# viswavi/speech-anonymization

Hardware: AMD Instinct MI355X
Metric: audio frames/sec (node), ConvAE+gender-adv train step (higher is better)
Workload: dtype bf16x3; 1 GPU; ConvAE recon0.1+sex0.9 adversarial train step (L1 recon + NLL), shape M: 32 utt/GPU x 161120 samples (T=1008 frames), Fbank x2 + norm + fwd + bwd + clip + Adam + Noam; batch_per_gpu=32, frames_per_utt=1008, parallelism=dp1

## Files before the change

### include/sa_hip.h

```cpp
#ifndef SA_HIP_H
#define SA_HIP_H
#ifdef __cplusplus
extern "C" {
#endif

#define SA_F32 0
#define SA_BF16 1
#define SA_BF16X3 2
#define SA_BF16X1F 3
#define SA_FP8 4
#define SA_F64 5
#define SA_MAX_TAPS 5
#define SA_COMM_ID_BYTES 128

typedef struct SaTaps {
  int ntaps[2];
  int off[2][SA_MAX_TAPS];
  int widx[2][SA_MAX_TAPS];
} SaTaps;

typedef struct SaConvArgs {
  const void* x;
  const void* wp;
  const float* bias;
  void* y;
  const float* s1; const float* t1;
  const float* s2; const float* t2;
  int swish;
  int relu;
  float* stats;
  int B, Lin, Lout, ntiles;
  int rowmin, nrows, wlo_off;
  SaTaps taps;
  int ep_mode, ep_xp_is_act, ep_bstride;
  const void* ep_x; const void* ep_g2;
  const float* ep_s1; const float* ep_t1; const float* ep_mean; const float* ep_rstd;
  void* a_out;
  const void* nb_x; const float* nb_c1; const float* nb_c2; const float* nb_c3;
  int nb_bstride, nb_relu_mask; float* nb_colsum;
  const float* ep_g2k1; const float* ep_g2k2; const float* ep_g2k3;
  float* pro_stats;
  const float* wscale;
  int tile_rows; int pad2_;
} SaConvArgs;

int sa_conv_gemm(int dtype, int cin, int cout, int sa, int u, const SaConvArgs* a, void* stream);
int sa_abi_sizeof(int which);
int sa_conv_gemm_ntiles(int cin, int cout, int u, int Lout);
int sa_conv_gemm_ntiles_tm(int tile_rows, int u, int Lout);
int sa_conv_gemm_set_tile_rows(int rows);
int sa_conv_gemm_set_impl(int impl);
int sa_conv_gemm_route(int dtype, int cin, int cout, int sa, int u, const SaConvArgs* a);

int sa_pack_weights(int dtype, const float* src, void* dst, int ntaps, int K, int N, int sk, int sn,
                    int st, void* stream);

typedef struct SaPackDesc {
  const float* src; void* dst;
  int dtype, ntaps, K, N, sk, sn, st, pad_;
  float* scale;
} SaPackDesc;
int sa_pack_weights_multi(const SaPackDesc* descs, int n, int blocks_per_image, void* stream);
int sa_pack_scales_multi(const SaPackDesc* descs, int n, void* stream);

typedef struct SaWgradArgs {
  const void* x;
  const void* dy;
  float* slabs;
  const float* s1; const float* t1; const float* s2; const float* t2; int swish;
  int B, Lin, Ldy, Mrows, chunk, nchunk;
  int ntaps; int off[SA_MAX_TAPS]; int ph[SA_MAX_TAPS];
  int x_pre;
  int dy_pre;
} SaWgradArgs;

int sa_wgrad(int dtype, int cin, int cout, int sa, int u, const SaWgradArgs* a, void* stream);
int sa_wgrad_kw(int cin, int cout);
int sa_wgrad_reduce(const float* slabs, float* dst, int nslab, int ntaps, int cin, int cout, int sk,
                    int sn, int st, int accumulate, void* stream);
#define SA_WRED_MAX 8
typedef struct SaWredDesc {
  const float* slabs; float* dst;
  int nslab, ntaps, cin, cout, sk, sn, st, accumulate, vec, pad_;
} SaWredDesc;
typedef struct SaWredMulti { int n, pad_; SaWredDesc d[SA_WRED_MAX]; } SaWredMulti;
int sa_wgrad_reduce_multi(const SaWredMulti* m, void* stream);

int sa_conv1toC(int dtype, const float* x, const float* w, const float* bias, void* y, int B, int L,
                int flip, float* stats, const void* ep_x, const float* ep_s1, const float* ep_t1,
                const float* ep_mean, const float* ep_rstd, void* stream);
int sa_conv1toC_ntiles(int L);
int sa_convCto1(int dtype, const void* x, const float* w, const float* bias, float* y, int B, int L,
                const float* s1, const float* t1, int swish, int flip, void* stream);
int sa_wgrad1C(int dtype, const float* u, const void* v, float* slabs, int B, int L, int chunk,
               int flip, const float* s1, const float* t1, int swish, void* stream);
int sa_wgrad1C_nchunk(int L, int chunk);
int sa_bwd1C(int dtype, const float* u, const void* v, const float* w, void* g, float* stats, float* slabs,
             int B, int L, int chunk, int flip, const float* s1, const float* t1, const float* mean,
             const float* rstd, void* stream);
int sa_sum_slabs(const float* slabs, float* dst, int nslab, int n, int accumulate, void* stream);

typedef struct SaEwArgs {
  const void* g; const void* g2; const void* x; void* out;
  const float* s1; const float* t1;
  const float* mean; const float* rstd;
  const float* c1; const float* c2; const float* c3;
  int actbwd, xp_is_act, relu_mask, bstride;
  float* stats;
  int B, L, ntiles;
} SaEwArgs;

int sa_ew_stats(int dtype, int C, const SaEwArgs* a, void* stream);
int sa_ew_apply(int dtype, int C, const SaEwArgs* a, void* stream);
int sa_ew_ntiles(int L);
int sa_sum_partials(const float* slabs, double* dst, int nbatch, int nslab, int n, void* stream);
int sa_sum_rows_d(const double* src, double* dst, int R, int n, void* stream);
int sa_fin_in_fwd(const double* sums, int B, int C, int n, const float* gamma, const float* beta,
                  float eps, float* mean, float* rstd, float* scale, float* shift, void* stream);
int sa_fin_bn_fwd(const double* sums, int R, int C, double count, const float* gamma, const float* beta,
                  float eps, float momentum, float* run_mean, float* run_var, float* mean,
                  float* rstd, float* scale, float* shift, const double* count_dev, void* stream);
int sa_fin_bn_eval(int C, const float* gamma, const float* beta, float eps, const float* run_mean,
                   const float* run_var, float* mean, float* rstd, float* scale, float* shift,
                   void* stream);
int sa_fin_norm_bwd(const double* sums, const double* lsums, int R, int groups, int C, double n,
                    const float* gamma, const float* mean, const float* rstd, float sign, float* c1,
                    float* c2, float* c3, float* dgamma, float* dbeta, const double* n_dev,
                    void* stream);
int sa_fin_bias(const double* sums, int B, int C, int ncomp, float* db, void* stream);

#define SA_FLATS_MAX 4
typedef struct SaFlat { float* p; long long n; } SaFlat;
typedef struct SaFlats { int n, pad_; SaFlat f[SA_FLATS_MAX]; } SaFlats;
int sa_clip_grads(const SaFlats* f, float max_norm, float eps, double* partials, float* total_norm, void* stream);
#define SA_BIAS_MAX 8
typedef struct SaBiasDesc {
  const float* part; double* rows; float* db;
  int nbatch, nslab, C, ncomp;
} SaBiasDesc;
typedef struct SaBiasMulti { int n, pad_; SaBiasDesc d[SA_BIAS_MAX]; } SaBiasMulti;
int sa_bias_multi(const SaBiasMulti* m, void* stream);

int sa_pool_fwd(int dtype, const void* r, const float* scale, const float* shift, float* part, int B,
                int L, int nseg, void* stream);
int sa_pool_nseg(int B);
int sa_pool_gather(const float* part, int B, int nseg, int L, double* sums, void* stream);
int sa_pool_fin(const double* sums, int B, int n, const float* noise, float eps, float* pooled,
                float* mean, float* stdraw, void* stream);
int sa_pool_bwd(int dtype, const void* r, const float* scale, const float* shift,
                const float* dpooled, const float* mean, const float* stdraw, void* g, int B, int L,
                const float* bn_mean, const float* bn_rstd, float* stats, void* stream);
int sa_dense(const float* X, int lda, const float* ps, const float* pt, const float* W, int sbk,
             int sbn, const float* bias, float* Y, int ldy, int M, int N, int K, int relu,
             void* stream);
int sa_colsums(const float* X, const float* H, const float* hmean, const float* hrstd, int M, int N,
               double* sums, float* out0, float* out1, void* stream);
int sa_bn2d_bwd(const float* G, const float* H, const double* sums, double count, const float* gamma,
                const float* mean, const float* rstd, int relu_mask, int M, int N, float* dH,
                const double* count_dev, void* stream);
int sa_dense_wgrad(const float* dY, const float* X, const float* ps, const float* pt, int M, int N,
                   int K, float* dW, void* stream);
int sa_log_softmax(const float* X, float* Y, int M, int N, void* stream);
int sa_log_softmax_bwd(const float* dY, const float* Y, float* dX, int M, int N, void* stream);
int sa_loss_workspace_bytes(void);
int sa_recon_loss(const float* a, const float* b, long long n, int kind, float* grad, float* loss,
                  void* workspace, void* stream);
int sa_cls_losses(const float* logp, const long long* label, int B, int NC, float* out, float* dnll,
                  float* dconf, void* stream);
int sa_cosine_loss(const float* x1, const float* x2, int B, int S, int D, float* rowloss,
                   float* loss, float* dx1, void* stream);

int sa_head_fwd(const float* pooled, const float* w1, const float* b1, const float* g1, const float* be1,
                float* rm1, float* rv1, const float* w2, const float* b2, const float* g2, const float* be2,
                float* rm2, float* rv2, const float* w3, const float* b3, float* h1, float* f1, float* h2,
                float* f2, float* logp, int M, float eps, float momentum, void* stream);
int sa_head_bwd(const float* dlogp, const float* logp, const float* pooled, const float* h1, const float* f1,
                const float* h2, const float* f2, const float* w1, const float* g1, const float* w2,
                const float* g2, const float* w3, float* dw1, float* db1, float* dg1, float* dbe1, float* dw2,
                float* db2, float* dg2, float* dbe2, float* dw3, float* db3, float* dpooled, int M, void* stream);
int sa_head_max_rows(void);

int sa_tdnn_fwd(const float* x, const void* wp, const float* bias, const float* bn_s, const float* bn_t,
                float* y, int B, int T, int Cin, int Cout, int Npad, int K, int dil, float slope,
                unsigned char* mask, void* stream);
int sa_time_pool(const float* x, const float* lens, const float* noise, int B, int T, int C, float eps,
                 float* out, void* stream);
int sa_leaky_affine(const float* x, const float* s, const float* t, float slope, int M, int C, float* y,
                    void* stream);
int sa_tdnn_bwd_input(const float* dy, const unsigned char* mask, const float* bn_s, const void* wp,
                      float* dxe, int B, int T, int Cy, int Cred, int Cin, int Npad, int K, int dil,
                      float slope, void* stream);
int sa_tdnn_fold(const float* dxe, float* dx, int B, int T, int C, int pad, void* stream);
int sa_time_pool_bwd(const float* x, const float* lens, const float* g, const float* pooled, int B,
                     int T, int C, float eps, float* dx, void* stream);
int sa_leaky_affine_bwd(const float* dy, const float* x, const float* s, float slope, int M, int C,
                        float* dx, void* stream);
// ... 137 lines not shown
```

### speech-anonymization_amd/_lib.py

```python
import ctypes as C
import os

import torch

_HERE = os.path.dirname(os.path.abspath(__file__))
LIB_PATH = os.environ.get("SA_HIP_LIB") or os.path.join(_HERE, "libsa_hip.so")

F32, BF16, BF16X3, BF16X1F, FP8, F64 = 0, 1, 2, 3, 4, 5
MAX_TAPS = 5

c_fp = C.POINTER(C.c_float)
vp = C.c_void_p


class SaTaps(C.Structure):
    _fields_ = [("ntaps", C.c_int * 2), ("off", (C.c_int * MAX_TAPS) * 2),
                ("widx", (C.c_int * MAX_TAPS) * 2)]


class SaConvArgs(C.Structure):
    _fields_ = [("x", vp), ("wp", vp), ("bias", vp), ("y", vp),
                ("s1", vp), ("t1", vp), ("s2", vp), ("t2", vp),
                ("swish", C.c_int), ("relu", C.c_int), ("stats", vp),
                ("B", C.c_int), ("Lin", C.c_int), ("Lout", C.c_int), ("ntiles", C.c_int),
                ("rowmin", C.c_int), ("nrows", C.c_int), ("wlo_off", C.c_int), ("taps", SaTaps),
                ("ep_mode", C.c_int), ("ep_xp_is_act", C.c_int), ("ep_bstride", C.c_int),
                ("ep_x", vp), ("ep_g2", vp), ("ep_s1", vp), ("ep_t1", vp), ("ep_mean", vp), ("ep_rstd", vp),
                ("a_out", vp),
                ("nb_x", vp), ("nb_c1", vp), ("nb_c2", vp), ("nb_c3", vp),
                ("nb_bstride", C.c_int), ("nb_relu_mask", C.c_int), ("nb_colsum", vp),
                ("ep_g2k1", vp), ("ep_g2k2", vp), ("ep_g2k3", vp), ("pro_stats", vp), ("wscale", vp),
                ("tile_rows", C.c_int), ("pad2_", C.c_int)]


class SaPackDesc(C.Structure):
    _fields_ = [("src", vp), ("dst", vp), ("dtype", C.c_int), ("ntaps", C.c_int), ("K", C.c_int),
                ("N", C.c_int), ("sk", C.c_int), ("sn", C.c_int), ("st", C.c_int), ("pad_", C.c_int),
                ("scale", vp)]


class SaWgradArgs(C.Structure):
    _fields_ = [("x", vp), ("dy", vp), ("slabs", vp),
                ("s1", vp), ("t1", vp), ("s2", vp), ("t2", vp), ("swish", C.c_int),
                ("B", C.c_int), ("Lin", C.c_int), ("Ldy", C.c_int), ("Mrows", C.c_int),
                ("chunk", C.c_int), ("nchunk", C.c_int),
                ("ntaps", C.c_int), ("off", C.c_int * MAX_TAPS), ("ph", C.c_int * MAX_TAPS),
                ("x_pre", C.c_int), ("dy_pre", C.c_int)]


class SaEwArgs(C.Structure):
    _fields_ = [("g", vp), ("g2", vp), ("x", vp), ("out", vp),
                ("s1", vp), ("t1", vp), ("mean", vp), ("rstd", vp),
                ("c1", vp), ("c2", vp), ("c3", vp),
                ("actbwd", C.c_int), ("xp_is_act", C.c_int), ("relu_mask", C.c_int),
                ("bstride", C.c_int), ("stats", vp),
                ("B", C.c_int), ("L", C.c_int), ("ntiles", C.c_int)]


BIAS_MAX = 8


class SaBiasDesc(C.Structure):
    _fields_ = [("part", vp), ("rows", vp), ("db", vp),
                ("nbatch", C.c_int), ("nslab", C.c_int), ("C", C.c_int), ("ncomp", C.c_int)]


class SaBiasMulti(C.Structure):
    _fields_ = [("n", C.c_int), ("pad_", C.c_int), ("d", SaBiasDesc * BIAS_MAX)]


WRED_MAX = 8
FLATS_MAX = 4


class SaFlat(C.Structure):
    _fields_ = [("p", vp), ("n", C.c_longlong)]


class SaFlats(C.Structure):
    _fields_ = [("n", C.c_int), ("pad_", C.c_int), ("f", SaFlat * FLATS_MAX)]



class SaWredDesc(C.Structure):
    _fields_ = [("slabs", vp), ("dst", vp)] + [(k, C.c_int) for k in ("nslab", "ntaps", "cin", "cout", "sk", "sn", "st",
                                                                      "accumulate", "vec", "pad_")]


class SaWredMulti(C.Structure):
    _fields_ = [("n", C.c_int), ("pad_", C.c_int), ("d", SaWredDesc * WRED_MAX)]


SYMBOLS = [
    "sa_conv_gemm", "sa_abi_sizeof", "sa_conv_gemm_ntiles", "sa_conv_gemm_ntiles_tm", "sa_conv_gemm_set_tile_rows",
    "sa_conv_gemm_set_impl", "sa_conv_gemm_route", "sa_pack_weights", "sa_pack_weights_multi", "sa_pack_scales_multi", "sa_wgrad", "sa_wgrad_kw", "sa_wgrad_reduce",
    "sa_conv1toC", "sa_conv1toC_ntiles", "sa_convCto1", "sa_wgrad1C", "sa_wgrad1C_nchunk", "sa_bwd1C",
    "sa_sum_slabs", "sa_ew_stats", "sa_ew_apply", "sa_ew_ntiles",
    "sa_sum_partials", "sa_sum_rows_d", "sa_fin_in_fwd", "sa_fin_bn_fwd", "sa_fin_bn_eval", "sa_fin_norm_bwd", "sa_fin_bias",
    "sa_pool_fwd", "sa_pool_nseg", "sa_pool_gather", "sa_pool_fin", "sa_pool_bwd", "sa_dense", "sa_colsums",
    "sa_bn2d_bwd", "sa_dense_wgrad", "sa_log_softmax", "sa_log_softmax_bwd",
    "sa_loss_workspace_bytes", "sa_recon_loss", "sa_cls_losses", "sa_cosine_loss",
    "sa_tdnn_fwd", "sa_time_pool", "sa_leaky_affine", "sa_tdnn_bwd_input", "sa_tdnn_fold", "sa_time_pool_bwd",
    "sa_leaky_affine_bwd", "sa_cluster_mi", "sa_fbank", "sa_fbank_table_elems", "sa_fbank_ntiles", "sa_fbank_scratch_bytes", "sa_fbank_normalize", "sa_fbank_normalize_pair",
    "sa_comm_unique_id", "sa_comm_init", "sa_comm_world", "sa_comm_allreduce", "sa_comm_allreduce_inline", "sa_comm_join", "sa_comm_ncalls",
    "sa_comm_destroy", "sa_head_fwd", "sa_head_bwd", "sa_head_max_rows",
    "sa_add_layernorm_fwd", "sa_layernorm_bwd", "sa_reflect_pad_fwd", "sa_reflect_pad_bwd", "sa_ln_leaky_fwd", "sa_ln_leaky_bwd", "sa_bias_multi", "sa_asr_block0_fwd", "sa_asr_block0_bwd", "sa_wgrad_reduce_multi", "sa_clip_grads",
    "sa_xv_tdnn_fwd_train", "sa_xv_tdnn_ntiles", "sa_xv_colsums", "sa_xv_tdnn_wgrad", "sa_xv_wgrad_reduce",
    "sa_xv_tdnn_dgrad", "sa_xv_pool_affine", "sa_xv_pool_affine_bwd",
    "sa_fc_tiles", "sa_fc_groups", "sa_fc_nparam", "sa_fc_nhead", "sa_fc_max_rows", "sa_fc_enc_fwd", "sa_fc_bn_fin",
    "sa_fc_mid_fwd", "sa_fc_head_fwd", "sa_fc_head_bwd", "sa_fc_mid_bwd", "sa_fc_bn_bwd_fin", "sa_fc_enc_bwd",
    "sa_fc_wreduce", "sa_fc_recon_fwd",
    "sa_wav_augment_tile", "sa_wav_augment_max_chunks", "sa_wav_abs_sums", "sa_noise_scales", "sa_wav_augment",
    "sa_specaug_warp_sums", "sa_specaug_finalize", "sa_specaug_fill",
    "sa_gl_tile", "sa_mel_to_mag", "sa_gl_istft", "sa_gl_project",
    "sa_yin_dim", "sa_yin_f0", "sa_pitch_ratio", "sa_pitch_stretch_mag", "sa_pitch_resample",
    "sa_env_dim", "sa_env_warp",
    "sa_mcadams_dim", "sa_mcadams",
    "sa_stoi_dim", "sa_stoi",
    "sa_pv_dim", "sa_pv_synth",
]

_lib = None


class SaHipError(RuntimeError):
    pass


def load():
    global _lib
    if _lib is None:
        if not os.path.exists(LIB_PATH):
            raise SaHipError(
                f"{LIB_PATH} not found: build it with `python -c 'import __graft_entry__ as g; "
                "g.build()'` (hipcc --offload-arch=gfx950). There is no CPU fallback.")
        _lib = C.CDLL(LIB_PATH)
        for s in SYMBOLS:
            getattr(_lib, s).restype = C.c_int
        _lib.sa_pv_workspace_bytes.restype = C.c_longlong
        for i, rec in enumerate((SaConvArgs, SaWgradArgs, SaEwArgs, SaPackDesc, SaTaps, SaBiasMulti, SaWredMulti, SaFlats)):
            if _lib.sa_abi_sizeof(i) != C.sizeof(rec):
                raise SaHipError(f"{rec.__name__}: binding has {C.sizeof(rec)} bytes, {LIB_PATH} "
                                 f"{_lib.sa_abi_sizeof(i)} -- rebuild the library (stale build?)")
    return _lib


def stream():
    return C.c_void_p(torch._C._cuda_getCurrentRawStream(torch._C._cuda_getDevice()))


def ptr(t):
    if t is None:
        return None
    assert t.is_cuda and t.is_contiguous(), "HIP kernels take contiguous device tensors"
    return C.c_void_p(t.data_ptr())


def check(rc, what):
    if rc != 0:
        raise SaHipError(f"{what} failed with code {rc}")


def dt_code(dtype):
    if dtype == torch.float32:
        return F32
    if dtype == torch.bfloat16:
        return BF16
    raise SaHipError(f"unsupported activation dtype {dtype}")


_taps_cache = {}


def make_taps(phases):
    key = tuple(tuple(p) for p in phases)
    t = _taps_cache.get(key)
    if t is not None:
        return t
    t = _taps_cache[key] = SaTaps()
    for ph, lst in enumerate(phases):
        t.ntaps[ph] = len(lst)
        for i, (off, wi) in enumerate(lst):
            t.off[ph][i] = off
            t.widx[ph][i] = wi
    return t
# ... 1 lines not shown
```

### speech-anonymization_amd/convae.py

```python
import functools
import os

import torch
import torch.nn as nn

from . import distributed as sdist
from . import ops
from . import _lib as L
from ._lib import SaHipError


class _ParamOnly(nn.Module):

    def forward(self, x):
        raise SaHipError("parameter container only; use ConvAutoencoder.forward")


class GLU(_ParamOnly):
    pass


class StatisticsPooling(_ParamOnly):
    pass


class TDNNSexClassifier(nn.Module):
    def __init__(self, num_classes=2):
        super().__init__()
        self.tdnn = nn.Sequential(
            nn.Conv1d(128, 128, kernel_size=5, dilation=1), nn.ReLU(), nn.BatchNorm1d(128),
            nn.Conv1d(128, 128, kernel_size=3, dilation=2), nn.ReLU(), nn.BatchNorm1d(128),
            nn.Conv1d(128, 128, kernel_size=3, dilation=3), nn.ReLU(), nn.BatchNorm1d(128),
        )
        self.norm = nn.BatchNorm1d(128)
        self.stats_pooling = StatisticsPooling()
        self.classify = nn.Sequential(
            nn.Linear(256, 128), nn.ReLU(), nn.BatchNorm1d(128),
            nn.Linear(128, 64), nn.ReLU(), nn.BatchNorm1d(64),
            nn.Linear(64, num_classes),
        )

    def forward(self, x):
        raise SaHipError("parameter container only; use ConvAutoencoder.forward")


class ConvAutoencoder(nn.Module):
    def __init__(self, precision="bf16x3", pooling_noise=True, sync_bn=True, dtype=None,
                 cache_wgrad_operand=True):
        super().__init__()
        if dtype is not None:
            precision = {torch.float32: "f32", torch.bfloat16: "bf16"}[dtype]
        if precision not in ops.PRECISIONS:
            raise SaHipError(f"unknown precision {precision!r}")
        self.precision = precision
        self.encoder = nn.Sequential(
            nn.Conv1d(1, 32, 15, 1, 7), GLU(),
            nn.Conv1d(32, 64, 5, 2, 2), nn.InstanceNorm1d(64, affine=True), GLU(),
            nn.Conv1d(64, 64, 5, 1, 2), nn.InstanceNorm1d(64, affine=True), GLU(),
            nn.Conv1d(64, 128, 5, 2, 2), nn.InstanceNorm1d(128, affine=True), GLU(),
            nn.Conv1d(128, 128, 5, 1, 2), nn.InstanceNorm1d(128, affine=True), GLU(),
        )
        self.decoder = nn.Sequential(
            nn.Conv1d(128, 128, 5, 1, 2),
            nn.ConvTranspose1d(128, 64, 5, 2, 2, output_padding=1),
            nn.InstanceNorm1d(64, affine=True), GLU(),
            nn.Conv1d(64, 64, 5, 1, 2),
            nn.ConvTranspose1d(64, 32, 5, 2, 2, output_padding=1),
            nn.InstanceNorm1d(32, affine=True), GLU(),
            nn.Conv1d(32, 1, 15, 1, 7),
        )
        self.sex_classifier = TDNNSexClassifier(2)
        self.lay = ops.conv_layers(self, ("encoder", "sex_classifier.tdnn", "decoder"))
        self.pack_plan = [(ly.key, ly.kinds[i]) for i in (0, 1)
                          for ly in sorted(self.lay.values(), key=lambda ly: ly.transposed)]
        self.act_dtype, self.kcode = ops.PRECISIONS[precision]
        self.dgrad_kcode = ops.DGRAD_CODE[precision]
        self.cache_wgrad_operand = cache_wgrad_operand
        self.pooling_noise = pooling_noise
        self.sync_bn = sync_bn
        self.fused_head = os.environ.get("SA_FUSED_HEAD", "1") == "1"
        self.fused_bwd1c = os.environ.get("SA_FUSED_BWD1C", "1") == "1"
        self.dp_batch_sizes = None

    def forward(self, feats):
        names, params = self._named_params()
        return _ConvAEFn.apply(self, names, feats, *params)

    def _named_params(self):
        c = self.__dict__.get("_np_cache")
        if c is None or any(o[n] is not p for o, n, p in c[2]):
            names, params, owners = [], [], []
            for mname, mod in self.named_modules():
                for pname, p in mod._parameters.items():
                    if p is not None:
                        names.append(f"{mname}.{pname}" if mname else pname)
                        params.append(p)
                        owners.append((mod._parameters, pname, p))
            c = self.__dict__["_np_cache"] = (tuple(names), tuple(params), owners)
        return c[0], c[1]

    @torch.no_grad()
    def reconstruct(self, feats):
        if not torch.is_tensor(feats) or feats.dim() != 3:
            raise SaHipError("ConvAutoencoder expects feats [B, T, 80]")
        x0, B, T, Ltot = _input_rows(feats)
        P = dict(zip(*self._named_params()))
        cg, inorm = _launchers(self, P, _packed(self, P), B)
        y, _, _ = _encoder_launches(self, P, cg, inorm, x0, Ltot, False)
        return _decoder_launches(self, P, cg, inorm, y[5], Ltot)[-1].view(B, T, 80)

    def _side_stream(self, device):
        if getattr(self, "_side", None) is None and device.type == "cuda":
            self._side = torch.cuda.Stream(device=device)
        return getattr(self, "_side", None)

    def _bn_syncs(self):
        return self.sync_bn and sdist.dp_active()

    def _bn_allreduce(self, sums):
        if self._bn_syncs():
            sdist.all_reduce_now(sums)
            return sdist.world_size()
        return 1

    def _bn_global_counts(self, counts, device):
        if not self._bn_syncs():
            return None
        key = (tuple(counts), str(device))
        cache = self.__dict__.setdefault("_count_cache", {})
        local = cache.get(key)
        if local is None:
            if len(cache) > 64:
                cache.clear()
            local = cache[key] = torch.tensor(counts, dtype=torch.float64).to(device)
        g = local.clone()
        sdist.all_reduce_now(g)
        return g

    def _bn_rows(self):
        return not self._bn_syncs()

    def _bn_global(self, local_sums):
        if not self._bn_syncs():
            return local_sums, 1
        g = local_sums.clone()
        return g, self._bn_allreduce(g)

    def _head_plan(self, B):
        if not self._bn_syncs() or self.dp_batch_sizes is None:
            return None
        W, r = sdist.world_size(), sdist.rank()
        sizes = [B] * W if isinstance(self.dp_batch_sizes, str) else [int(b) for b in self.dp_batch_sizes]
        if self.dp_batch_sizes != "equal" and isinstance(self.dp_batch_sizes, str):
            raise SaHipError(f"dp_batch_sizes: 'equal', a list of per-rank batch sizes or None, not {self.dp_batch_sizes!r}")
        if len(sizes) != W or sizes[r] != B:
            raise SaHipError(f"dp_batch_sizes {sizes} does not describe rank {r} of {W} holding {B} utterances")
        return sum(sizes[:r]), sum(sizes), W

    @staticmethod
    def _gather_rows(x, plan):
        off, Bg, _ = plan
        g = torch.zeros(Bg, x.shape[1], device=x.device, dtype=x.dtype)
        g[off:off + x.shape[0]].copy_(x)
        sdist.all_reduce_now(g)
        return g


class _W:
    __slots__ = ("img", "code")

    def __init__(self, img, code):
        self.img, self.code = img, code


def _kcode(model, kind):
    return model.dgrad_kcode if kind.endswith("dgrad") else model.kcode


def _packed(model, P):
    items = [((k, kind), P[k], kind, _kcode(model, kind)) for k, kind in model.pack_plan]
    key = tuple(w.data_ptr() for _, w, _, _ in items) + tuple(c for _, _, _, c in items)
    pk = getattr(model, "_pack_cache", None)
    if pk is None or pk[0] != key:
        pk = (key, ops.PackedWeights(items, model.act_dtype))
        model._pack_cache = pk
    pk[1].refresh()
    return {tag: _W(img, code) for tag, (img, code) in pk[1].images.items()}


def _conv(x, w, *args, **kw):
    return ops.conv_gemm(x, w.img, *args, code=w.code, **kw)


class _PendingApply:
    __slots__ = ("g", "y", "c", "per_c", "relu", "bias_key", "wgrads")

    def __init__(self, g, y, c, per_c, relu, bias_key):
        self.g, self.y, self.c, self.per_c, self.relu, self.bias_key = g, y, c, per_c, relu, bias_key
        self.wgrads = []


def _noise(model, B, device):
    return ops.pooling_noise(model.pooling_noise, B, 128, device)


def _input_rows(feats):
    B, T, Fd = feats.shape
    Ltot = T * Fd
    if Fd != 80 or Ltot % 4:
        raise SaHipError("ConvAutoencoder expects feats [B, T, 80] with T*80 divisible by 4")
    if not feats.is_cuda:
        raise SaHipError("ConvAutoencoder runs on the GPU only (no CPU fallback)")
    return feats.detach().reshape(B, Ltot).contiguous().float(), B, T, Ltot


def _in_ep(y, nrm, g2=None):
    mean, rstd, scale, shift = nrm
    d = dict(mode=1, x=y, g2=g2, s1=scale, t1=shift, mean=mean, rstd=rstd)
    if isinstance(g2, _PendingApply):
        d.update(g2=g2.g, g2k=g2.c)
    return d


def _launchers(model, P, W, B, A=None):
    def cg(ly, x, **kw):
        if A is not None and P[ly.key].requires_grad:
            A[ly.key] = kw["a_out"] = torch.empty(x.shape, dtype=torch.bfloat16, device=x.device)
        return _conv(x, W[ly.key, ly.kinds[0]], P[ly.bias], *ly.fwd(x.shape[1]), **kw)

    def inorm(stats, n, prefix, C):
        sums = ops.sum_partials(stats, B)
        return ops.fin_in_fwd(sums, B, C, n, P[prefix + ".weight"], P[prefix + ".bias"])
    return cg, inorm


def _encoder_launches(model, P, cg, inorm, x0, Ltot, want_pro_stats):
    L2, L4, lay = Ltot // 2, Ltot // 4, model.lay
    y0 = ops.conv1toC(x0, P["encoder.0.weight"], P["encoder.0.bias"], model.act_dtype)
    y1, st = cg(lay["encoder.2"], y0, swish=True, want_stats=True)
    n1 = inorm(st, L2, "encoder.3", 64)
    y2, st = cg(lay["encoder.5"], y1, s1=n1[2], t1=n1[3], swish=True, want_stats=True)
    n2 = inorm(st, L2, "encoder.6", 64)
    y3, st = cg(lay["encoder.8"], y2, s1=n2[2], t1=n2[3], swish=True, want_stats=True)
    n3 = inorm(st, L4, "encoder.9", 128)
    y4, st = cg(lay["encoder.11"], y3, s1=n3[2], t1=n3[3], swish=True, want_stats=True)
    n4 = inorm(st, L4, "encoder.12", 128)
    y5 = cg(lay["decoder.0"], y4, s1=n4[2], t1=n4[3], swish=True, want_pro_stats=want_pro_stats)
    a4_stats = None
    if want_pro_stats:
        y5, a4_stats = y5
    return [y0, y1, y2, y3, y4, y5], [n1, n2, n3, n4], a4_stats


def _decoder_launches(model, P, cg, inorm, y5, Ltot):
    L2, lay = Ltot // 2, model.lay
    y6, st = cg(lay["decoder.1"], y5, want_stats=True)
    n6 = inorm(st, L2, "decoder.2", 64)
    y7 = cg(lay["decoder.4"], y6, s1=n6[2], t1=n6[3], swish=True)
    y8, st = cg(lay["decoder.5"], y7, want_stats=True)
    n8 = inorm(st, Ltot, "decoder.6", 32)
    recon = ops.convCto1(y8, P["decoder.8.weight"], P["decoder.8.bias"], n8[2], n8[3], True)
    return y6, n6, y7, y8, n8, recon


class _ConvAEFn(torch.autograd.Function):
    @staticmethod
    def forward(ctx, model, names, feats, *params):
        ctx.set_materialize_grads(False)
        P = dict(zip(names, params))
        train = model.training
        x0, B, T, Ltot = _input_rows(feats)
        L2, L4 = Ltot // 2, Ltot // 4
        S = {}
        W, lay = _packed(model, P), model.lay
        A = {}
        cache_a = (train and model.cache_wgrad_operand and any(ctx.needs_input_grad)
                   and ops.WGRAD_CODE[model.precision] in (L.BF16X1F, L.BF16) and model.kcode != L.FP8)

        cg, inorm = _launchers(model, P, W, B, A if cache_a else None)

        def bn_stats(stats, count, mod, prefix, C, ci):
            sums = ops.sum_partials(stats, 1, rows=model._bn_rows()) if train else None
            return bnorm(sums, count, mod, prefix, C, ci)

        def bnorm(sums, count, mod, prefix, C, ci, local=False):
            if not train:
                return ops.fin_bn_eval(C, P[prefix + ".weight"], P[prefix + ".bias"],
                                       mod.running_mean, mod.running_var)
            if not local:
                model._bn_allreduce(sums)
            out = ops.fin_bn_fwd(sums, C, count, P[prefix + ".weight"], P[prefix + ".bias"],
                                 mod.running_mean, mod.running_var, count_dev=None if local else cdev(ci))
            tracked.append(mod.num_batches_tracked)
            return out

        tracked = []
        enc, dec, cls = model.encoder, model.decoder, model.sex_classifier
        La, Lb, Lc = L4 - 4, L4 - 8, L4 - 14
        gc = model._bn_global_counts([B * L4, B * La, B * Lb, B * Lc, B, B], feats.device) if train else None
        cdev = lambda i: None if gc is None else gc[i:i + 1]
        (y0, y1, y2, y3, y4, y5), (n1, n2, n3, n4), a4_stats = _encoder_launches(model, P, cg, inorm, x0, Ltot, train)
        bn_n = bn_stats(a4_stats if train else None, B * L4, cls.norm, "sex_classifier.norm", 128, 0)
        r0, st = cg(lay["sex_classifier.tdnn.0"], y4, s1=n4[2], t1=n4[3], swish=True, s2=bn_n[2], t2=bn_n[3],
                    relu=True, want_stats=True)
        bn0 = bn_stats(st, B * La, cls.tdnn[2], "sex_classifier.tdnn.2", 128, 1)
        r1, st = cg(lay["sex_classifier.tdnn.3"], r0, s2=bn0[2], t2=bn0[3], relu=True, want_stats=True)
        bn1 = bn_stats(st, B * Lb, cls.tdnn[5], "sex_classifier.tdnn.5", 128, 2)
        r2, st = cg(lay["sex_classifier.tdnn.6"], r1, s2=bn1[2], t2=bn1[3], relu=True, want_stats=True)
        bn2 = bn_stats(st, B * Lc, cls.tdnn[8], "sex_classifier.tdnn.8", 128, 3)
        pooled, pmean, psd = ops.pool_fwd(r2, bn2[2], bn2[3], noise=_noise(model, B, feats.device))
        def head_fwd(X, n, local=False):
            H1 = ops.dense(X, P["sex_classifier.classify.0.weight"], P["sex_classifier.classify.0.bias"],
                           128, 256, relu=True)
            f1 = bnorm(ops.colsums(H1) if train else None, n, cls.classify[2], "sex_classifier.classify.2", 128, 4, local)
            H2 = ops.dense(H1, P["sex_classifier.classify.3.weight"], P["sex_classifier.classify.3.bias"],
                           64, 128, ps=f1[2], pt=f1[3], relu=True)
            f2 = bnorm(ops.colsums(H2) if train else None, n, cls.classify[5], "sex_classifier.classify.5", 64, 5, local)
            logits = ops.dense(H2, P["sex_classifier.classify.6.weight"], P["sex_classifier.classify.6.bias"],
                               2, 64, ps=f2[2], pt=f2[3])
            return H1, f1, H2, f2, ops.log_softmax(logits)

        plan = model._head_plan(B) if train else None
        head_in, Bh = (model._gather_rows(pooled, plan), plan[1]) if plan else (pooled, B)
        fused_head = (train and model.fused_head and (plan is not None or not model._bn_syncs())
                      and Bh <= ops.head_max_rows())
        clsP = {k[len("sex_classifier.classify."):]: v for k, v in P.items() if k.startswith("sex_classifier.classify.")}
        if fused_head:
            H1, f1, H2, f2, logp = ops.head_fwd(head_in, clsP, cls.classify[2], cls.classify[5])
            tracked += [cls.classify[2].num_batches_tracked, cls.classify[5].num_batches_tracked]
        else:
            H1, f1, H2, f2, logp = head_fwd(head_in, Bh, plan is not None)
        logp_all = logp
        if plan:
            logp = logp_all[plan[0]:plan[0] + B]
        y6, n6, y7, y8, n8, recon = _decoder_launches(model, P, cg, inorm, y5, Ltot)

        if tracked:
            torch._foreach_add_(tracked, 1)
        S.update(x0=x0, y=[y0, y1, y2, y3, y4, y5, y6, y7, y8], r=[r0, r1, r2],
                 n=[None, n1, n2, n3, n4, None, n6, None, n8], bn=[bn_n, bn0, bn1, bn2], f=[f1, f2],
                 pooled=head_in, pmean=pmean, psd=psd, H1=H1, H2=H2, logp=logp_all, head_plan=plan,
                 dims=(B, T, Ltot, L2, L4, La, Lb, Lc), train=train, W=W, A=A, gc=gc, fused_head=fused_head)
        ctx.S, ctx.model, ctx.names, ctx.params = S, model, names, params
        ctx.need_input_grad = feats.requires_grad
        return recon.view(B, T, 80), logp

    @staticmethod
    def backward(ctx, d_recon, d_logp):
        S, model, names = ctx.S, ctx.model, ctx.names
        if S is None:
            raise SaHipError("ConvAutoencoder backward called twice (saved tensors were released)")
        P = dict(zip(names, ctx.params))
        dt = model.act_dtype
        B, T, Ltot, L2, L4, La, Lb, Lc = S["dims"]
        if not S["train"]:
            raise SaHipError("backward through eval-mode BatchNorm is not implemented")
        y0, y1, y2, y3, y4, y5, y6, y7, y8 = S["y"]
        r0, r1, r2 = S["r"]
        n1, n2, n3, n4, n6, n8 = S["n"][1], S["n"][2], S["n"][3], S["n"][4], S["n"][6], S["n"][8]
        bn_n, bn0, bn1, bn2 = S["bn"]
        f1, f2 = S["f"]
        dev = y0.device
        G = {k: None for k in names}
        need = {k: p.requires_grad for k, p in P.items()}
        need_stage = {st: any(v for k, v in need.items() if k.startswith(st))
                      for st in sdist.StageBuckets.STAGES}
        run_encoder = need_stage["encoder"] or ctx.need_input_grad
        run_decoder = need_stage["decoder"] or run_encoder
        model._last_flats = None
        buckets = sdist.StageBuckets(list(P.items()), dev, model._side_stream(dev))
        newg = buckets.view

        def setg(key, val):
            G[key] = newg(key).copy_(val.reshape(P[key].shape))
        W, A, lay = S["W"], S["A"], model.lay
        gc = S["gc"]
        cdev = lambda i: None if gc is None else gc[i:i + 1]
        pending_wred = []
        wg = functools.partial(ops.wgrad, code=ops.WGRAD_CODE[model.precision], defer=pending_wred)
        fuse = bool(A) and model.dgrad_kcode in (L.BF16X3, L.BF16)

        def cg(ly, gin, **kw):
            p, dy = gin, gin.g if isinstance(gin, _PendingApply) else gin
            w, args = W[ly.key, ly.kinds[1]], (None,) + ly.dgrad(ly.lin(dy.shape[1]))
            if dy is gin:
                return _conv(dy, w, *args, **kw)
            dyc = torch.empty(p.g.shape, dtype=torch.bfloat16, device=p.g.device) if p.wgrads else None
            want_cs = p.bias_key is not None and need[p.bias_key]
            out = _conv(p.g, w, *args, a_out=dyc, nb=dict(x=p.y, c1=p.c[0], c2=p.c[1], c3=p.c[2],
                                                           per_c=p.per_c, relu_mask=p.relu,
                                                           want_colsum=want_cs), **kw)
            if want_cs:
                cs = out[-1]
                out = out[:-1] if len(out) > 2 else out[0]
                nb_, _, cc_ = cs.shape
                G[p.bias_key] = newg(p.bias_key)
                pending_bias.append((cs, nb_, cc_, 1, G[p.bias_key]))
            for f in p.wgrads:
                f(dyc)
            p.wgrads = []
            return out

        def bias_from(stats, key, C):
            if need[key]:
                G[key] = newg(key)
                pending_bias.append((stats, B, C, 2, G[key]))

        pending_bias = []

        def flush_pending():
            if pending_bias:
                ops.bias_multi(pending_bias)
                pending_bias.clear()
            if pending_wred:
                ops.wgrad_reduce_multi(pending_wred)
                pending_wred.clear()

        def in_finish(g, st, y, nrm, C, Ln, prefix, bias_key):
            mean, rstd = nrm[0], nrm[1]
            dg, db = newg(prefix + ".weight"), newg(prefix + ".bias")
            sums = ops.sum_partials(st, B)
            c1, c2, c3 = ops.fin_norm_bwd(sums, sums, B * C, C, Ln, P[prefix + ".weight"], mean, rstd,
                                          dgamma=dg, dbeta=db)
            G[prefix + ".weight"], G[prefix + ".bias"] = dg, db
            if fuse:
                return _PendingApply(g, y, (c1, c2, c3), False, False, bias_key)
            st2 = ops.ew("apply", g, y, C, out=g, c1=c1, c2=c2, c3=c3)
            bias_from(st2, bias_key, C)
            return g

        def bn_ep(r, bn, xp=None):
            d = dict(mode=2, x=r, mean=bn[0], rstd=bn[1], per_c=True)
            if xp:
                d.update(s1=xp[0], t1=xp[1], xp_is_act=True)
            return d

        def bn_finish(g, st, r, bn, Ln, prefix, bias_key, ci, xp=None):
            mean, rstd = bn[0], bn[1]
            kw = dict(s1=xp[0], t1=xp[1], xp_is_act=True) if xp else {}
            dg, db = newg(prefix + ".weight"), newg(prefix + ".bias")
            lsums = ops.sum_partials(st, 1, rows=model._bn_rows())
            gsums, _ = model._bn_global(lsums)
            c1, c2, c3 = ops.fin_norm_bwd(gsums, lsums, 128, 128, float(B * Ln), P[prefix + ".weight"],
                                          mean, rstd, sign=-1.0 if xp else 1.0, dgamma=dg, dbeta=db,
                                          n_dev=cdev(ci))
            G[prefix + ".weight"], G[prefix + ".bias"] = dg, db
            if fuse:
                return _PendingApply(g, r, (c1, c2, c3), True, not xp, bias_key)
            st2 = ops.ew("apply", g, r, 128, out=g, c1=c1, c2=c2, c3=c3, relu_mask=not xp, per_c=True,
                         want_stats=bias_key is not None, **kw)
            if bias_key:
                bias_from(st2, bias_key, 128)
            return g

        def conv_wgrad(ly, x, dy, **pro):
            key = ly.key
            if not need[key]:
                return
            if isinstance(dy, _PendingApply):
                dy.wgrads.append(lambda dyc: conv_wgrad(ly, x, dyc, dy_pre=True))
                return
            if key in A:
                x, pro = A[key], dict(x_pre=True, dy_pre=bool(pro.get("dy_pre")))
            *geo, strides = ly.wgrad(x.shape[1])
            G[key] = wg(x, dy, *geo, newg(key), strides, **pro)

        recon_unused = d_recon is None
        if recon_unused:
            for k in need:
                if k.startswith("decoder"):
                    need[k] = False
            need_stage["decoder"] = False
        if d_logp is None:
            d_logp = torch.zeros(B, 2, device=dev)

        def finish(d_feats=None):
            flush_pending()
            buckets.join()
            ctx.S = None
            model._last_flats = [buckets.flat[st] for st in sdist.StageBuckets.STAGES if need_stage[st]]
            grads = tuple(G[k] if need[k] else None for k in names)
            G.clear()
            buckets.views.clear()
            return (None, None, d_feats) + grads

        def head_bwd():
            c = "sex_classifier.classify."
            plan = S.get("head_plan")
            dlp, Bh = d_logp.contiguous().float(), B
            if plan:
                dlp, Bh = model._gather_rows(dlp, plan), plan[1]
            dP = head_bwd_rows(c, dlp, Bh, plan is not None)
            if plan:
                hg = [G[k] for k in names if k.startswith(c) and k in G]
                if plan[2] > 1 and hg:
                    torch._foreach_mul_(hg, 1.0 / plan[2])
                dP = dP[plan[0]:plan[0] + B]
            return dP

        def head_bwd_rows(c, dlp, n, local):
            if S.get("fused_head"):
                short = ("0.weight", "0.bias", "2.weight", "2.bias", "3.weight", "3.bias", "5.weight", "5.bias",
                         "6.weight", "6.bias")
                views = {}
                for k in short:
                    if need[c + k]:
                        views[k] = G[c + k] = newg(c + k)
                clsP = {k: P[c + k] for k in short}
                return ops.head_bwd(dlp, S["logp"], S["pooled"], S["H1"], f1, S["H2"], f2, clsP, views)
            glob = (lambda l: l) if local else (lambda l: model._bn_global(l)[0])
            cd = (lambda i: None) if local else cdev
            dLG = ops.log_softmax_bwd(dlp, S["logp"])
            H1, H2 = S["H1"], S["H2"]
            G[c + "6.weight"] = ops.dense_wgrad(dLG, H2, newg(c + "6.weight"), ps=f2[2], pt=f2[3])
            G[c + "6.bias"] = newg(c + "6.bias"); ops.colsums(dLG, out0=G[c + "6.bias"])
            dN2 = ops.dense(dLG, P[c + "6.weight"], None, 64, 2, transpose_w=True)
            G[c + "5.weight"], G[c + "5.bias"] = newg(c + "5.weight"), newg(c + "5.bias")
            l2 = ops.colsums(dN2, H2, f2[0], f2[1], out0=G[c + "5.bias"], out1=G[c + "5.weight"])
            dH2 = ops.bn2d_bwd(dN2, H2, glob(l2), n, P[c + "5.weight"], f2[0], f2[1], True, count_dev=cd(5))
            G[c + "3.weight"] = ops.dense_wgrad(dH2, H1, newg(c + "3.weight"), ps=f1[2], pt=f1[3])
            G[c + "3.bias"] = newg(c + "3.bias"); ops.colsums(dH2, out0=G[c + "3.bias"])
            dN1 = ops.dense(dH2, P[c + "3.weight"], None, 128, 64, transpose_w=True)
            G[c + "2.weight"], G[c + "2.bias"] = newg(c + "2.weight"), newg(c + "2.bias")
            l1 = ops.colsums(dN1, H1, f1[0], f1[1], out0=G[c + "2.bias"], out1=G[c + "2.weight"])
            dH1 = ops.bn2d_bwd(dN1, H1, glob(l1), n, P[c + "2.weight"], f1[0], f1[1], True, count_dev=cd(4))
            G[c + "0.weight"] = ops.dense_wgrad(dH1, S["pooled"], newg(c + "0.weight"))
            G[c + "0.bias"] = newg(c + "0.bias"); ops.colsums(dH1, out0=G[c + "0.bias"])
            return ops.dense(dH1, P[c + "0.weight"], None, 256, 128, transpose_w=True)

        def tdnn_bwd(dP):
            t = "sex_classifier.tdnn."
            g, st = ops.pool_bwd(r2, bn2[2], bn2[3], dP, S["pmean"], S["psd"], bn=(bn2[0], bn2[1]))
            g = bn_finish(g, st, r2, bn2, Lc, t + "8", t + "6.bias", 3)
            conv_wgrad(lay[t + "6"], r1, g, s2=bn1[2], t2=bn1[3])
            g, st = cg(lay[t + "6"], g, want_stats=True, ep=bn_ep(r1, bn1))
            g = bn_finish(g, st, r1, bn1, Lb, t + "5", t + "3.bias", 2)
            conv_wgrad(lay[t + "3"], r0, g, s2=bn0[2], t2=bn0[3])
            g, st = cg(lay[t + "3"], g, want_stats=True, ep=bn_ep(r0, bn0))
            g = bn_finish(g, st, r0, bn0, La, t + "2", t + "0.bias", 1)
            conv_wgrad(lay[t + "0"], y4, g, s1=n4[2], t1=n4[3], swish=True, s2=bn_n[2], t2=bn_n[3])
            xp4 = (n4[2], n4[3])
            g, st = cg(lay[t + "0"], g, want_stats=True, ep=bn_ep(y4, bn_n, xp4))
            da = bn_finish(g, st, y4, bn_n, L4, "sex_classifier.norm", None, 0, xp=xp4)
            flush_pending()
            if need_stage["sex_classifier"]:
                buckets.reduce_stage("sex_classifier")
            return da

        def decoder_bwd():
            d_rec = torch.zeros(B, T, 80, device=dev) if recon_unused else d_recon
            g_rec = d_rec.reshape(B, Ltot).contiguous().float()
            if need["decoder.8.bias"]:
                setg("decoder.8.bias", ops.sum_partials(g_rec.view(4 * B, Ltot // 4), 1, n=Ltot // 4).sum())
            if need["decoder.8.weight"] and model.fused_bwd1c:
                g, st, G["decoder.8.weight"] = ops.bwd1C(g_rec, y8, P["decoder.8.weight"], newg("decoder.8.weight"),
                                                         n8[2], n8[3], n8[0], n8[1])
            else:
                if need["decoder.8.weight"]:
                    G["decoder.8.weight"] = ops.wgrad1C(g_rec, y8, newg("decoder.8.weight"), flip=True,
                                                        s1=n8[2], t1=n8[3], swish=True)
                g, st = ops.conv1toC(g_rec, P["decoder.8.weight"], None, dt, flip=True, want_stats=True,
                                     ep=dict(x=y8, s1=n8[2], t1=n8[3], mean=n8[0], rstd=n8[1]))
            g = in_finish(g, st, y8, n8, 32, Ltot, "decoder.6", "decoder.5.bias")
            conv_wgrad(lay["decoder.5"], y7, g)
            g, st = cg(lay["decoder.5"], g, want_stats=True)
            bias_from(st, "decoder.4.bias", 64)
            conv_wgrad(lay["decoder.4"], y6, g, s1=n6[2], t1=n6[3], swish=True)
            g, st = cg(lay["decoder.4"], g, want_stats=True, ep=_in_ep(y6, n6))
            g = in_finish(g, st, y6, n6, 64, L2, "decoder.2", "decoder.1.bias")
            conv_wgrad(lay["decoder.1"], y5, g)
            g, st = cg(lay["decoder.1"], g, want_stats=True)
            bias_from(st, "decoder.0.bias", 128)
            conv_wgrad(lay["decoder.0"], y4, g, s1=n4[2], t1=n4[3], swish=True)
            flush_pending()
            if need_stage["decoder"]:
                buckets.reduce_stage("decoder")
            return g

        da4_cls = tdnn_bwd(head_bwd())
        if not run_decoder:
            return finish()
        g = decoder_bwd()
        if not run_encoder:
            return finish()

        g, st = cg(lay["decoder.0"], g, want_stats=True, ep=_in_ep(y4, n4, g2=da4_cls))
        for conv, norm, y, nrm, x, nx in (("encoder.11", "encoder.12", y4, n4, y3, n3),
                                          ("encoder.8", "encoder.9", y3, n3, y2, n2),
                                          ("encoder.5", "encoder.6", y2, n2, y1, n1),
                                          ("encoder.2", "encoder.3", y1, n1, y0, None)):
            ly = lay[conv]
            g = in_finish(g, st, y, nrm, ly.cout, y.shape[1], norm, ly.bias)
            conv_wgrad(ly, x, g, swish=True, **(dict(s1=nx[2], t1=nx[3]) if nx else {}))
            g, st = cg(ly, g, want_stats=True, ep=_in_ep(x, nx) if nx else dict(mode=1, x=x))
        bias_from(st, "encoder.0.bias", 32)
        if need["encoder.0.weight"]:
            G["encoder.0.weight"] = ops.wgrad1C(S["x0"], g, newg("encoder.0.weight"))
        d_feats = None
        if ctx.need_input_grad:
            d_feats = ops.convCto1(g, P["encoder.0.weight"], None, flip=True).view(B, T, 80)
        flush_pending()
        if need_stage["encoder"]:
            buckets.reduce_stage("encoder")
        return finish(d_feats)
```

### speech-anonymization_amd/csrc/sa_conv_gemm.hip

```cpp
#include <type_traits>
#include "sa_common.h"

#include "sa_conv_cfg.h"

template <typename T, int CIN, int COUT, int SA, int U, int TM, bool PRO2>
__global__ __launch_bounds__(256, 2) void sa_conv_gemm_kernel(SaConvArgs a, int red_off, int col_off) {
  typedef ConvCfg<T, CIN, COUT, SA, U, TM> C;
  typedef Pol<T> P;
  typedef typename P::store_t S;
  typedef typename P::lds_t LT;
  typedef typename P::Frag Frag;
  typedef Tr<S> tr;
  constexpr int VEC = C::VEC, OVEC = C::OVEC;
  extern __shared__ __attribute__((aligned(16))) unsigned char smem[];
  LT* As = reinterpret_cast<LT*>(smem);
  S* Os = reinterpret_cast<S*>(smem);
  float* red = reinterpret_cast<float*>(smem + red_off);
  const int plane = a.nrows * C::APITCH;

  const int tid = threadIdx.x, lane = tid & 63, wave = tid >> 6;
  const int tile = blockIdx.x, b = blockIdx.y;
  const int m0 = tile * C::BMB;

  {
    const int c = tid % C::CHI, r0 = tid / C::CHI;
    float s1[VEC], t1[VEC], s2[VEC], t2[VEC];
#pragma unroll
    for (int j = 0; j < VEC; ++j) {
      s1[j] = a.s1 ? a.s1[(size_t)b * CIN + c * VEC + j] : 1.0f;
      t1[j] = a.t1 ? a.t1[(size_t)b * CIN + c * VEC + j] : 0.0f;
      s2[j] = a.s2 ? a.s2[c * VEC + j] : 1.0f;
      t2[j] = a.t2 ? a.t2[c * VEC + j] : 0.0f;
    }
    const bool has1 = a.s1 != nullptr, has2 = a.s2 != nullptr, sw = a.swish != 0;
    const S* xb = reinterpret_cast<const S*>(a.x) + (size_t)b * a.Lin * CIN + c * VEC;
    const int gbase = m0 * SA + a.rowmin;
    const int own_lo = m0 * SA;
    int own_hi = tile == a.ntiles - 1 ? a.Lin : (m0 + C::BMB) * SA;
    if (own_hi > a.Lin) own_hi = a.Lin;
    constexpr int NIT = ((C::BMB - 1) * SA + 1 + SA_MAX_HALO + C::RPPI - 1) / C::RPPI;
    uint4 raw[NIT];
#pragma unroll
    for (int i = 0; i < NIT; ++i) {
      const int r = r0 + i * C::RPPI, g = gbase + r;
      raw[i] = make_uint4(0, 0, 0, 0);
      if (r < a.nrows && g >= 0 && g < a.Lin) raw[i] = *reinterpret_cast<const uint4*>(xb + (size_t)g * CIN);
    }
    uint4 raw2[PRO2 ? NIT : 1];
    float k1[VEC], k2[VEC], k3[VEC], csum[VEC];
    if constexpr (PRO2) {
      const S* x2 = reinterpret_cast<const S*>(a.nb_x) + (size_t)b * a.Lin * CIN + c * VEC;
#pragma unroll
      for (int i = 0; i < NIT; ++i) {
        const int r = r0 + i * C::RPPI, g = gbase + r;
        raw2[i] = make_uint4(0, 0, 0, 0);
        if (r < a.nrows && g >= 0 && g < a.Lin) raw2[i] = *reinterpret_cast<const uint4*>(x2 + (size_t)g * CIN);
      }
#pragma unroll
      for (int j = 0; j < VEC; ++j) {
        const size_t q = (size_t)b * a.nb_bstride + c * VEC + j;
        k1[j] = a.nb_c1[q]; k2[j] = a.nb_c2[q]; k3[j] = a.nb_c3[q]; csum[j] = 0.0f;
      }
    }
    auto stage_rows = [&](auto xform) {
#pragma unroll
      for (int i = 0; i < NIT; ++i) {
        const int r = r0 + i * C::RPPI, g = gbase + r;
        if (r < a.nrows) {
          float f[VEC];
          tr::unpack(raw[i], f);
          if (g >= 0 && g < a.Lin) xform(f, i, g);
          LT* dst = As + (size_t)r * C::APITCH + c * VEC;
          if constexpr (P::NPL == 2) {
            uint2 hi, lo;
            sa_split4(f, hi, lo);
            *reinterpret_cast<uint2*>(dst) = hi;
            *reinterpret_cast<uint2*>(dst + plane) = lo;
          } else if constexpr (sizeof(LT) == 1) {
            *reinterpret_cast<uint2*>(dst) = sa_pack_fp8x8(f);
          } else if constexpr (sizeof(LT) == 2 && sizeof(S) == 4) {
            *reinterpret_cast<uint2*>(dst) = sa_pack_bf16x4(f);
          } else if constexpr (sizeof(LT) == 2) {
            *reinterpret_cast<uint4*>(dst) = tr::pack(f);
          } else {
            float* d = reinterpret_cast<float*>(dst);
            d[0] = f[0]; d[1] = f[1]; d[2] = f[2]; d[3] = f[3];
          }
        }
      }
    };
    if constexpr (PRO2) {
      stage_rows([&](float* f, int i, int g) {
        float y[VEC];
        tr::unpack(raw2[i], y);
        const bool own = g >= own_lo && g < own_hi;
#pragma unroll
        for (int j = 0; j < VEC; ++j) {
          float v = fmaf(k1[j], f[j], fmaf(k2[j], y[j], k3[j]));
          if (a.nb_relu_mask && !(y[j] > 0.0f)) v = 0.0f;
          f[j] = v;
          if (own) csum[j] += v;
        }
      });
      if (a.nb_colsum) {
        float* colred = reinterpret_cast<float*>(smem + col_off);
#pragma unroll
        for (int j = 0; j < VEC; ++j) {
          float v = csum[j];
          for (int off = C::CHI; off < 64; off <<= 1) v += __shfl_xor(v, off, 64);
          if (lane < C::CHI) colred[wave * CIN + (lane % C::CHI) * VEC + j] = v;
        }
      }
    } else if (!has1 && !has2 && !sw) {
      stage_rows([](float*, int, int) {});
    } else if (has1 && sw && !has2 && a.pro_stats) {
      float ps[VEC], pq[VEC];
#pragma unroll
      for (int j = 0; j < VEC; ++j) { ps[j] = 0.0f; pq[j] = 0.0f; }
      stage_rows([&](float* f, int, int g) {
        const bool own = g >= own_lo && g < own_hi;
#pragma unroll
        for (int j = 0; j < VEC; ++j) {
          const float v = sa_swish(fmaf(f[j], s1[j], t1[j]));
          f[j] = v;
          if (own) { ps[j] += v; pq[j] = fmaf(v, v, pq[j]); }
        }
      });
      float* colred = reinterpret_cast<float*>(smem + col_off);
#pragma unroll
      for (int j = 0; j < VEC; ++j) {
        float v = ps[j], w = pq[j];
        for (int off = C::CHI; off < 64; off <<= 1) { v += __shfl_xor(v, off, 64); w += __shfl_xor(w, off, 64); }
        if (lane < C::CHI) {
          colred[(wave * CIN + (lane % C::CHI) * VEC + j) * 2 + 0] = v;
          colred[(wave * CIN + (lane % C::CHI) * VEC + j) * 2 + 1] = w;
        }
      }
    } else if (has1 && sw && !has2) {
      stage_rows([&](float* f, int, int) {
#pragma unroll
        for (int j = 0; j < VEC; ++j) f[j] = sa_swish(fmaf(f[j], s1[j], t1[j]));
      });
    } else {
      stage_rows([&](float* f, int, int) {
#pragma unroll
        for (int j = 0; j < VEC; ++j) {
          float v = f[j];
          if (has1) v = fmaf(v, s1[j], t1[j]);
          if (sw) v = sa_swish(v);
          if (has2) v = fmaf(v, s2[j], t2[j]);
          f[j] = v;
        }
      });
    }
  }
  __syncthreads();
  if (!PRO2 && a.pro_stats && tid < CIN) {
    const float* colred = reinterpret_cast<const float*>(smem + col_off);
    float* d = a.pro_stats + (((size_t)b * a.ntiles + tile) * CIN + tid) * 2;
#pragma unroll
    for (int q = 0; q < 2; ++q)
      d[q] = (colred[tid * 2 + q] + colred[(CIN + tid) * 2 + q]) +
             (colred[(2 * CIN + tid) * 2 + q] + colred[(3 * CIN + tid) * 2 + q]);
  }
  if constexpr (PRO2) {
    if (a.nb_colsum && tid < CIN) {
      const float* colred = reinterpret_cast<const float*>(smem + col_off);
      a.nb_colsum[((size_t)b * a.ntiles + tile) * CIN + tid] =
          (colred[tid] + colred[CIN + tid]) + (colred[2 * CIN + tid] + colred[3 * CIN + tid]);
    }
  }
  if constexpr (sizeof(LT) == 2) {
    if (a.a_out) {
      constexpr int CH16 = CIN / 8;
      const int own_lo = m0 * SA;
      int own_hi = tile == a.ntiles - 1 ? a.Lin : (m0 + C::BMB) * SA;
      if (own_hi > a.Lin) own_hi = a.Lin;
      const int rlo = own_lo - (m0 * SA + a.rowmin);
      bf16_t* ao = reinterpret_cast<bf16_t*>(a.a_out) + ((size_t)b * a.Lin + own_lo) * CIN;
      for (int e = tid; e < (own_hi - own_lo) * CH16; e += 256) {
        const int r = e / CH16, c = e % CH16;
        *reinterpret_cast<uint4*>(ao + (size_t)r * CIN + c * 8) =
            *reinterpret_cast<const uint4*>(As + (size_t)(rlo + r) * C::APITCH + c * 8);
      }
    }
  }

  const int wn = wave % C::WN, wm = wave / C::WN;
  f32x16 acc[C::VPW][C::MT];
#pragma unroll
  for (int v = 0; v < C::VPW; ++v)
#pragma unroll
    for (int mt = 0; mt < C::MT; ++mt)
#pragma unroll
      for (int i = 0; i < 16; ++i) acc[v][mt][i] = 0.0f;

  constexpr int KUP = P::NPL == 2 ? 2 : 8;
  constexpr int KU = C::KSTEPS < KUP ? C::KSTEPS : KUP;
  constexpr int GPT = C::KSTEPS / KU;
  static_assert(C::KSTEPS % KU == 0, "k-steps per tap must be a multiple of the prefetch group");
  const Frag* wp = reinterpret_cast<const Frag*>(a.wp);
#pragma unroll
  for (int v = 0; v < C::VPW; ++v) {
    const int vt = wn + v * C::WN;
    const int ph = vt / C::NT, nt = vt % C::NT;
    const int G = a.taps.ntaps[ph] * GPT;
    const LT* abase = As + (size_t)((wm * C::MT * 32 + (lane & 31)) * SA - a.rowmin) * C::APITCH
                      + (lane >> 5) * (C::KS / 2);
    auto load_group = [&](Frag (&dst)[P::NPL][KU], int g) {
      const int ti = g / GPT, kg = g % GPT;
      const Frag* wt = wp + (((size_t)a.taps.widx[ph][ti] * C::KSTEPS + kg * KU) * C::NT + nt) * 64 + lane;
#pragma unroll
      for (int ku = 0; ku < KU; ++ku) {
        dst[0][ku] = wt[(size_t)ku * C::NT * 64];
        if constexpr (P::NPL == 2) dst[1][ku] = wt[(size_t)a.wlo_off + (size_t)ku * C::NT * 64];
      }
    };
    auto compute_group = [&](const Frag (&bq)[P::NPL][KU], int g) {
      const int ti = g / GPT, kg = g % GPT;
      const LT* arow = abase + (size_t)a.taps.off[ph][ti] * C::APITCH + kg * KU * C::KS;
      Frag ah[2][C::MT], al[2][C::MT];
      auto load_a = [&](int slot, int ku) {
#pragma unroll
        for (int mt = 0; mt < C::MT; ++mt) {
          const LT* ap = arow + (size_t)mt * 32 * SA * C::APITCH + ku * C::KS;
          ah[slot][mt] = *reinterpret_cast<const Frag*>(ap);
          if constexpr (P::NPL == 2) al[slot][mt] = *reinterpret_cast<const Frag*>(ap + plane);
        }
      };
      load_a(0, 0);
#pragma unroll
      for (int ku = 0; ku < KU; ++ku) {
        if (ku + 1 < KU) load_a((ku + 1) & 1, ku + 1);
#pragma unroll
        for (int mt = 0; mt < C::MT; ++mt) {
          if constexpr (P::NPL == 2) {
            acc[v][mt] = __builtin_amdgcn_mfma_f32_32x32x16_bf16(al[ku & 1][mt], bq[0][ku], acc[v][mt], 0, 0, 0);
            acc[v][mt] = __builtin_amdgcn_mfma_f32_32x32x16_bf16(ah[ku & 1][mt], bq[1][ku], acc[v][mt], 0, 0, 0);
            acc[v][mt] = __builtin_amdgcn_mfma_f32_32x32x16_bf16(ah[ku & 1][mt], bq[0][ku], acc[v][mt], 0, 0, 0);
          } else {
            acc[v][mt] = Tr<LT>::mfma(ah[ku & 1][mt], bq[0][ku], acc[v][mt]);
          }
        }
      }
    };
    Frag b0[P::NPL][KU], b1[P::NPL][KU];
    load_group(b0, 0);
    for (int g = 0; g < G; g += 2) {
      if (g + 1 < G) load_group(b1, g + 1);
      compute_group(b0, g);
      if (g + 1 < G) {
        if (g + 2 < G) load_group(b0, g + 2);
        compute_group(b1, g + 1);
      }
    }
  }
  constexpr int NOT = TM / C::RPPO;
  const int ec = tid % C::CHO, er0 = tid / C::CHO;
  __syncthreads();

#pragma unroll
  for (int v = 0; v < C::VPW; ++v) {
    const int vt = wn + v * C::WN;
    const int ph = vt / C::NT, nt = vt % C::NT;
    const int col = nt * 32 + (lane & 31);
    const float bv = a.bias ? a.bias[col] : 0.0f;
    float winv = 1.0f;
    if constexpr (sizeof(LT) == 1) winv = a.wscale ? 1.0f / a.wscale[0] : 1.0f;
#pragma unroll
    for (int mt = 0; mt < C::MT; ++mt) {
#pragma unroll
      for (int i = 0; i < 16; ++i) {
        const int m = wm * C::MT * 32 + mt * 32 + sa_acc_row(i, lane);
        float val = sizeof(LT) == 1 ? fmaf(acc[v][mt][i], winv, bv) : acc[v][mt][i] + bv;
        if (a.relu) val = fmaxf(val, 0.0f);
        Os[(size_t)(m * U + ph) * C::OPITCH + col] = tr::from_f(val);
      }
    }
  }
  __syncthreads();
  {
    const int c = ec, r0 = er0;
    float ssum[OVEC], ssq[OVEC], es1[OVEC], et1[OVEC], emu[OVEC], ers[OVEC];
#pragma unroll
    for (int j = 0; j < OVEC; ++j) {
      ssum[j] = 0.0f; ssq[j] = 0.0f;
      es1[j] = (a.ep_mode && a.ep_s1) ? a.ep_s1[(size_t)b * COUT + c * OVEC + j] : 1.0f;
      et1[j] = (a.ep_mode && a.ep_t1) ? a.ep_t1[(size_t)b * COUT + c * OVEC + j] : 0.0f;
      emu[j] = (a.ep_mode && a.ep_mean) ? a.ep_mean[(size_t)b * a.ep_bstride + c * OVEC + j] : 0.0f;
      ers[j] = (a.ep_mode && a.ep_rstd) ? a.ep_rstd[(size_t)b * a.ep_bstride + c * OVEC + j] : 1.0f;
    }
    const bool g2k = a.ep_mode && a.ep_g2 && a.ep_g2k1;
    float gk1[OVEC], gk2[OVEC], gk3[OVEC];
#pragma unroll
    for (int j = 0; j < OVEC; ++j) {
      gk1[j] = g2k ? a.ep_g2k1[c * OVEC + j] : 1.0f;
      gk2[j] = g2k ? a.ep_g2k2[c * OVEC + j] : 0.0f;
      gk3[j] = g2k ? a.ep_g2k3[c * OVEC + j] : 0.0f;
    }
    S* yb = reinterpret_cast<S*>(a.y) + (size_t)b * a.Lout * COUT + c * OVEC;
    const S* xe = a.ep_mode ? reinterpret_cast<const S*>(a.ep_x) + (size_t)b * a.Lout * COUT + c * OVEC : nullptr;
    const S* ge = (a.ep_mode && a.ep_g2) ? reinterpret_cast<const S*>(a.ep_g2) + (size_t)b * a.Lout * COUT + c * OVEC : nullptr;
    const int o0 = m0 * U;
    auto ep_rows = [&](uint4 u, const uint4& epx, const uint4& epg, int o) {
      float g[OVEC], x[OVEC], g2[OVEC], xn[OVEC];
      tr::unpack(u, g); tr::unpack(epx, x); tr::unpack(epg, g2);
#pragma unroll
      for (int j = 0; j < OVEC; ++j) {
        const float z = fmaf(x[j], es1[j], et1[j]);
        if (g2k) g2[j] = fmaf(gk1[j], g2[j], fmaf(gk2[j], sa_swish(z), gk3[j]));
        float gg = g[j] + g2[j];
        if (a.ep_mode == 1) gg *= sa_swish_grad(z);
        const float xv = a.ep_xp_is_act ? sa_swish(z) : x[j];
        xn[j] = (xv - emu[j]) * ers[j];
        g[j] = gg;
      }
      u = tr::pack(g);
      *reinterpret_cast<uint4*>(yb + (size_t)o * COUT) = u;
      if (a.stats) {
        tr::unpack(u, g);
#pragma unroll
        for (int j = 0; j < OVEC; ++j) { ssum[j] += g[j]; ssq[j] = fmaf(g[j], xn[j], ssq[j]); }
      }
    };
    if (a.ep_mode && o0 + TM <= a.Lout) {
      auto run = [&](auto has_g2_c) {
        constexpr bool HG = decltype(has_g2_c)::value;
        constexpr int D = NOT < 2 ? NOT : 2;
        uint4 px[D], pg[D];
#pragma unroll
        for (int d = 0; d < D; ++d) {
          px[d] = *reinterpret_cast<const uint4*>(xe + (size_t)(o0 + r0 + d * C::RPPO) * COUT);
          pg[d] = make_uint4(0, 0, 0, 0);
          if constexpr (HG) pg[d] = *reinterpret_cast<const uint4*>(ge + (size_t)(o0 + r0 + d * C::RPPO) * COUT);
        }
#pragma unroll
        for (int i = 0; i < NOT; ++i) {
          const int r = r0 + i * C::RPPO, o = o0 + r;
          const uint4 epx = px[i % D], epg = pg[i % D];
          if (i + D < NOT) {
            px[i % D] = *reinterpret_cast<const uint4*>(xe + (size_t)(o + D * C::RPPO) * COUT);
            if constexpr (HG) pg[i % D] = *reinterpret_cast<const uint4*>(ge + (size_t)(o + D * C::RPPO) * COUT);
          }
          const uint4 u = *reinterpret_cast<const uint4*>(Os + (size_t)r * C::OPITCH + c * OVEC);
          ep_rows(u, epx, epg, o);
        }
      };
      if (ge) run(std::true_type{}); else run(std::false_type{});
    } else {
#pragma unroll
    for (int i = 0; i < NOT; ++i) {
      const int r = r0 + i * C::RPPO, o = o0 + r;
      if (o < a.Lout) {
        uint4 u = *reinterpret_cast<const uint4*>(Os + (size_t)r * C::OPITCH + c * OVEC);
        if (a.ep_mode) {
          const uint4 epx = *reinterpret_cast<const uint4*>(xe + (size_t)o * COUT);
          const uint4 epg = ge ? *reinterpret_cast<const uint4*>(ge + (size_t)o * COUT) : make_uint4(0, 0, 0, 0);
          ep_rows(u, epx, epg, o);
        } else {
          *reinterpret_cast<uint4*>(yb + (size_t)o * COUT) = u;
          if (a.stats) {
            float f[OVEC];
            tr::unpack(u, f);
#pragma unroll
            for (int j = 0; j < OVEC; ++j) { ssum[j] += f[j]; ssq[j] = fmaf(f[j], f[j], ssq[j]); }
          }
        }
      }
    }
    }
    if (a.stats) {
      __syncthreads();
#pragma unroll
      for (int j = 0; j < OVEC; ++j) {
        red[((size_t)r0 * COUT + c * OVEC + j) * 2 + 0] = ssum[j];
        red[((size_t)r0 * COUT + c * OVEC + j) * 2 + 1] = ssq[j];
      }
    }
  }
  if (a.stats) {
    __syncthreads();
    if (tid < COUT) {
      float s = 0.0f, q = 0.0f;
      for (int r = 0; r < C::RPPO; ++r) {
        s += red[((size_t)r * COUT + tid) * 2 + 0];
        q += red[((size_t)r * COUT + tid) * 2 + 1];
      }
      float* dst = a.stats + (((size_t)b * a.ntiles + tile) * COUT + tid) * 2;
      dst[0] = s; dst[1] = q;
    }
  }
}

template <typename T, int CIN, int COUT, int SA, int U, int TM, bool PRO2 = false>
static int launch_cfg(const SaConvArgs& a, hipStream_t st) {
  typedef ConvCfg<T, CIN, COUT, SA, U, TM> C;
  SaConvArgs args = a;
  args.ntiles = sa_div_up(sa_div_up(a.Lout, U), C::BMB);
  int omin = 1 << 30, omax = -(1 << 30);
  for (int ph = 0; ph < U; ++ph)
    for (int t = 0; t < a.taps.ntaps[ph]; ++t) {
      omin = a.taps.off[ph][t] < omin ? a.taps.off[ph][t] : omin;
      omax = a.taps.off[ph][t] > omax ? a.taps.off[ph][t] : omax;
    }
  if (omin > omax || omax - omin > SA_MAX_HALO) return -22;
  int wmax = 0;
  for (int ph = 0; ph < U; ++ph)
    for (int t = 0; t < a.taps.ntaps[ph]; ++t) wmax = a.taps.widx[ph][t] > wmax ? a.taps.widx[ph][t] : wmax;
  args.rowmin = omin;
  args.nrows = (C::BMB - 1) * SA + (omax - omin) + 1;
  args.wlo_off = (wmax + 1) * C::KSTEPS * C::NT * 64;
  if ((a.a_out || a.nb_colsum || a.pro_stats) &&
      (omin > 0 || (C::BMB - 1) * SA + omax < C::BMB * SA - 1 ||
       (args.ntiles - 1) * C::BMB * SA + omin + args.nrows < a.Lin))
    return -22;
  if (a.a_out && sizeof(typename C::LT) != 2) return -22;
  if (PRO2 && (!a.nb_c1 || !a.nb_c2 || !a.nb_c3)) return -22;
  if (a.pro_stats && (PRO2 || !a.s1 || !a.swish || a.s2)) return -22;
  const size_t tile_lds = C::lds_bytes(args.nrows);
  const size_t lds = tile_lds + (PRO2 ? 4 * CIN * sizeof(float) : a.pro_stats ? 8 * CIN * sizeof(float) : 0);
  if (lds > 160 * 1024) return -12;
  auto kern = sa_conv_gemm_kernel<T, CIN, COUT, SA, U, TM, PRO2>;
  static bool attr_set = false;
  if (!attr_set) {
    hipError_t e = hipFuncSetAttribute(reinterpret_cast<const void*>(kern),
                                       hipFuncAttributeMaxDynamicSharedMemorySize, 160 * 1024);
    if (e != hipSuccess) return -(int)e;
    attr_set = true;
  }
  dim3 grid(args.ntiles, a.B);
  hipLaunchKernelGGL(kern, grid, dim3(256), lds, st, args, 0, (int)tile_lds);
  hipError_t e = hipGetLastError();
  return e == hipSuccess ? 0 : -(int)e;
}

static int g_tile_rows = 0;
extern "C" int sa_conv_gemm_set_tile_rows(int rows) {
  if (rows != 0 && rows != 64 && rows != 128) return -22;
  g_tile_rows = rows;
  return 0;
}
static int tile_rows(int cin, int cout, int u) {
  if (cin == 64 && cout == 32 && u == 2) return 128;
  if (g_tile_rows) return g_tile_rows;
  if ((cin == 64 && cout == 64) || (cin == 128 && cout == 64 && u == 2)) return 128;
  return 64;
}

extern "C" int sa_conv_gemm_ntiles(int cin, int cout, int u, int Lout) {
  const int tm = tile_rows(cin, cout, u);
  return sa_div_up(sa_div_up(Lout, u), tm / u);
}

bool sa_conv_ws_covers(int dtype, int cin, int cout, int sa, int u, const SaConvArgs* a);
int sa_conv_ws_dispatch(int cin, int cout, const SaConvArgs* a, hipStream_t st);
int sa_conv_ws_tile_rows(int cout);
int sa_conv_ws_rows_per_tile(int cout);
bool sa_conv_wsd_covers(int dtype, int cin, int cout, int sa, int u, const SaConvArgs* a);
int sa_conv_wsd_dispatch(int cin, int cout, const SaConvArgs* a, hipStream_t st);
static int g_use_ws = 1;
extern "C" int sa_conv_gemm_set_impl(int impl) {
  if (impl != 0 && impl != 2) return -22;
  g_use_ws = impl == 2;
  return 0;
}

extern "C" int sa_conv_gemm_ntiles_tm(int tile_rows, int u, int Lout) {
  if ((tile_rows != 64 && tile_rows != 128) || u < 1 || Lout < 1) return -22;
  return sa_div_up(sa_div_up(Lout, u), tile_rows / u);
}

template <typename T, int CI, int CO, int S, int UU, bool PRO2 = false>
static int launch_tm(const SaConvArgs& a, hipStream_t st) {
  if constexpr (CI == 64 && CO == 32 && UU == 2) {
    return launch_cfg<T, CI, CO, S, UU, 128, PRO2>(a, st);
  } else {
    const int tm = (a.tile_rows == 64 || a.tile_rows == 128) ? a.tile_rows : tile_rows(CI, CO, UU);
    return tm == 64 ? launch_cfg<T, CI, CO, S, UU, 64, PRO2>(a, st)
                    : launch_cfg<T, CI, CO, S, UU, 128, PRO2>(a, st);
  }
}

#define SA_CONV_CASE(CI, CO, S, UU)                                              \
  if (cin == CI && cout == CO && sa == S && u == UU) {                           \
    if (a->nb_x)                                                                 \
      return dtype == SA_BF16X3 ? launch_tm<bf16x3_t, CI, CO, S, UU, true>(*a, st) \
             : dtype == SA_BF16 ? launch_tm<bf16_t, CI, CO, S, UU, true>(*a, st) : -22; \
    if (dtype == SA_FP8) return (a->wscale && !a->ep_mode) ? launch_tm<fp8_t, CI, CO, S, UU>(*a, st) : -22; \
    return dtype == SA_BF16 ? launch_tm<bf16_t, CI, CO, S, UU>(*a, st)           \
           : dtype == SA_BF16X3 ? launch_tm<bf16x3_t, CI, CO, S, UU>(*a, st)     \
           : dtype == SA_BF16X1F ? launch_tm<bf16x1f_t, CI, CO, S, UU>(*a, st)   \
                                : launch_tm<float, CI, CO, S, UU>(*a, st);       \
  }

extern "C" int sa_abi_sizeof(int which) {
  switch (which) {
    case 0: return (int)sizeof(SaConvArgs);
    case 1: return (int)sizeof(SaWgradArgs);
    case 2: return (int)sizeof(SaEwArgs);
    case 3: return (int)sizeof(SaPackDesc);
    case 4: return (int)sizeof(SaTaps);
    case 5: return (int)sizeof(SaBiasMulti);
    case 6: return (int)sizeof(SaWredMulti);
    case 7: return (int)sizeof(SaFlats);
    default: return -22;
  }
}

static int conv_route(int dtype, int cin, int cout, int sa, int u, const SaConvArgs* a) {
  if (g_use_ws && sa_conv_ws_covers(dtype, cin, cout, sa, u, a) &&
      tile_rows(cin, cout, u) == sa_conv_ws_tile_rows(cout) &&
      (long)a->B * sa_div_up(a->Lout, sa_conv_ws_rows_per_tile(cout)) >= 1536)
    return 2;
  if (g_use_ws && sa_conv_wsd_covers(dtype, cin, cout, sa, u, a) && tile_rows(cin, cout, u) == 64 &&
      (long)a->B * sa_div_up(a->Lout, 64) >= 1536)
    return 3;
  return 0;
}
extern "C" int sa_conv_gemm_route(int dtype, int cin, int cout, int sa, int u, const SaConvArgs* a) {
  if (!a || a->B <= 0 || a->Lout <= 0) return -22;
  return conv_route(dtype, cin, cout, sa, u, a);
}

extern "C" int sa_conv_gemm(int dtype, int cin, int cout, int sa, int u, const SaConvArgs* a,
                            void* stream) {
  hipStream_t st = reinterpret_cast<hipStream_t>(stream);
  if (!a || !a->x || !a->wp || !a->y || a->B <= 0 || a->Lin <= 0 || a->Lout <= 0) return -22;
  if (a->ep_mode < 0 || a->ep_mode > 2 || (a->ep_mode && !a->ep_x)) return -22;
  const int route = conv_route(dtype, cin, cout, sa, u, a);
  if (route == 2) return sa_conv_ws_dispatch(cin, cout, a, st);
  if (route == 3) return sa_conv_wsd_dispatch(cin, cout, a, st);
  SA_CONV_CASE(32, 64, 2, 1)
  SA_CONV_CASE(64, 64, 1, 1)
  SA_CONV_CASE(64, 128, 2, 1)
  SA_CONV_CASE(128, 128, 1, 1)
  SA_CONV_CASE(128, 64, 1, 2)
  SA_CONV_CASE(64, 32, 1, 2)
  return -38;
}
```

### speech-anonymization_amd/csrc/sa_conv_ws.hip

```cpp
#include <type_traits>
#include "sa_conv_cfg.h"

#ifdef SA_WS_STAMPS
__device__ unsigned long long sa_ws_dbg[64 * 8];
#define WS_STAMP(it, i) do { if (lane_ == 0 && wave_ == 0 && blockIdx.x == 7 && (it) < 64) { \
  unsigned long long t_; asm volatile("s_memtime %0\n\ts_waitcnt lgkmcnt(0)" : "=s"(t_) :: "memory"); \
  sa_ws_dbg[(it) * 8 + (i)] = t_; } } while (0)
extern "C" int sa_ws_dbg_read(unsigned long long* out) {
  return -(int)hipMemcpyFromSymbol(out, HIP_SYMBOL(sa_ws_dbg), sizeof(sa_ws_dbg));
}
#else
#define WS_STAMP(it, i)
#endif

#include "sa_conv_ws_common.h"

namespace {

template <int MODE, int NT, int HALO, int CC = 128, int CO = CC, int SA = 1, int UU = 1>
__global__ __launch_bounds__(256) __attribute__((amdgpu_waves_per_eu(1, 1)))
void sa_conv_ws_kernel(SaConvArgs a, int total_tiles) {
  typedef WsGeo<CC, NT, HALO, CO, SA, UU> G;
  constexpr int WS_CO = G::CO, WS_SA = G::SA, WS_BM = G::BM;
  static_assert(UU == 1 || MODE == 0, "transposed layers: plain rows");
// ... 479 lines not shown
          if constexpr (k >= 2 && k < 6) piece_split(j, k - 2);
          if constexpr (k == 9) piece_cache(Tn, false, j);
          if constexpr (k == 10) dma_piece(Tnn, false, j);
        }
      };
      ws_static_for<0, WS_NTAPS * WS_KSTEPS>([&](auto s_c) {
        constexpr int s = decltype(s_c)::value;
        constexpr int tp = s / WS_KSTEPS, k = s % WS_KSTEPS, sl = s & 1;
        constexpr bool more = s + 1 < WS_NTAPS * WS_KSTEPS;
        __builtin_amdgcn_sched_barrier(0);
#define WS_MFMA1(M, A, BC, B) \
        asm volatile("v_mfma_f32_32x32x16_bf16 %0, %1, %2, %0" : "+v"(acc[M]) : "v"(A), BC(B))
#define WS_AL(M) if constexpr (more) { __builtin_amdgcn_sched_barrier(0); load_al(s + 1, M); load_ah(s + 1, M); }
#define WS_AH(M)
#define WS_SLOT(I) __builtin_amdgcn_sched_barrier(0); filler(std::integral_constant<int, 6 * s + (I)>{}); __builtin_amdgcn_sched_barrier(0)
        if constexpr (s == 0) {
          asm volatile("v_mfma_f32_32x32x16_bf16 %0, %1, %2, 0" : "=&v"(acc[0]) : "v"(al[0]), "a"(Bh[0][0]));
          WS_AL(0); WS_SLOT(0);
          asm volatile("v_mfma_f32_32x32x16_bf16 %0, %1, %2, 0" : "=&v"(acc[1]) : "v"(al[1]), "a"(Bh[0][0]));
          WS_AL(1); WS_SLOT(1);
        } else if constexpr (s < WS_NAGPR_FRAGS) {
          WS_MFMA1(0, al[0], "a", Bh[tp][k]); WS_AL(0); WS_SLOT(0);
          WS_MFMA1(1, al[1], "a", Bh[tp][k]); WS_AL(1); WS_SLOT(1);
        } else {
          WS_MFMA1(0, al[0], "v", Bh[tp][k]); WS_AL(0); WS_SLOT(0);
          WS_MFMA1(1, al[1], "v", Bh[tp][k]); WS_AL(1); WS_SLOT(1);
        }
        if constexpr (s < WS_NAGPR_FRAGS) {
          WS_MFMA1(0, ah[sl][0], "a", Bl[tp][k]); WS_AH(0); WS_SLOT(2);
          WS_MFMA1(1, ah[sl][1], "a", Bl[tp][k]); WS_AH(1); WS_SLOT(3);
          WS_MFMA1(0, ah[sl][0], "a", Bh[tp][k]); WS_SLOT(4);
          WS_MFMA1(1, ah[sl][1], "a", Bh[tp][k]); WS_SLOT(5);
        } else {
          WS_MFMA1(0, ah[sl][0], "v", Bl[tp][k]); WS_AH(0); WS_SLOT(2);
          WS_MFMA1(1, ah[sl][1], "v", Bl[tp][k]); WS_AH(1); WS_SLOT(3);
          WS_MFMA1(0, ah[sl][0], "v", Bh[tp][k]); WS_SLOT(4);
          WS_MFMA1(1, ah[sl][1], "v", Bh[tp][k]); WS_SLOT(5);
        }
#undef WS_MFMA1
#undef WS_SLOT
#undef WS_AL
#undef WS_AH
      });
    };
    const bool fast = slotE && slotT && slotD;
    if (fast) {
      tile_body(std::true_type{});
      piece_write(WS_DPW - 1);
    } else {
      if (doE && !partialE) {
#pragma unroll
        for (int n = 0; n < 32; ++n) epi_value(Tp, false, n);
        epi_stats(Tp);
      }
      tile_body(std::false_type{});
    }
    WS_STAMP(it, 1);
    if (!fast) {
      asm volatile("s_waitcnt vmcnt(0)" ::: "memory");
#pragma unroll
      for (int j = 0; j < WS_DPW; ++j) {
        piece_read(j);
#pragma unroll
        for (int q = 0; q < 4; ++q) piece_elem(Tn, edgeT, j, q);
        piece_write(j);
        piece_cache(Tn, edgeT, j);
      }
      asm volatile("s_waitcnt lgkmcnt(0)" ::: "memory");
#pragma unroll
      for (int j = 0; j < WS_DPW; ++j) dma_piece(Tnn, edgeD, j);
    }
    colsum_put(it + 1);
    asm volatile("s_nop 15\n\ts_nop 15\n\ts_nop 15\n\ts_nop 15\n\ts_nop 15" : "+v"(acc[0]), "+v"(acc[1]));
#pragma unroll
    for (int m = 0; m < 2; ++m)
#pragma unroll
      for (int i = 0; i < 16; ++i) {
        float v;
        asm volatile("v_mov_b32 %0, %1" : "=v"(v) : "v"(acc[m][i]));
        accp[m][i] = v;
      }
    eval = epi_form(0);
    asm volatile("s_waitcnt lgkmcnt(0)" ::: "memory");
    __builtin_amdgcn_s_barrier();
    WS_STAMP(it, 2);
    stats_out();
    if (doT) colsum_out(t + 1, it + 1);
    Tp = Tc; Tc = Tn; Tn = Tnn;
  }
  {
    const bool partialE = Tp.tile > part_hi;
    ybase_e = const_cast<char*>(row_ptr(a.y, Tp.orow, WS_CO * 4));
    stbase_e = const_cast<char*>(row_ptr(a.stats, Tp.srow, WS_CO * 8));
    st_slab_ok = G::SLABS == 1 || Tp.tile * 2 + rh_ < a.ntiles * 2 - slab_short;
    if (!partialE) eval = epi_form(0);
#pragma unroll
    for (int n = 0; n < 32; ++n) epi_value(Tp, partialE, n);
    epi_stats(Tp);
    if constexpr (G::COMBINE == 2) {
      asm volatile("s_waitcnt lgkmcnt(0)" ::: "memory");
      __builtin_amdgcn_s_barrier();
      stats_out();
    }
  }
#undef WS_IDS
}

template <int MODE, int NT = 5, int HALO = 4, int CC = 128, int CO = CC, int SA = 1, int UU = 1>
int launch_ws(const SaConvArgs& a, hipStream_t st) {
  typedef WsGeo<CC, NT, HALO, CO, SA, UU> G;
  constexpr int WS_NTAPS = G::NTAPS, WS_HALO = G::HALO, WS_ROWS = G::ROWS, WS_RAW_BYTES = G::RAW_BYTES, WS_BUF_BYTES = G::BUF_BYTES,
                WS_C = G::C, WS_KSTEPS = G::KSTEPS;
  SaConvArgs args = a;
  args.ntiles = sa_div_up(sa_div_up(a.Lout, UU), G::BM);
  int omin = 1 << 30, omax = -(1 << 30), wmax = 0;
  for (int ph = 0; ph < UU; ++ph)
    for (int t = 0; t < (UU == 1 ? WS_NTAPS : a.taps.ntaps[ph]); ++t) {
      omin = a.taps.off[ph][t] < omin ? a.taps.off[ph][t] : omin;
      omax = a.taps.off[ph][t] > omax ? a.taps.off[ph][t] : omax;
      wmax = a.taps.widx[ph][t] > wmax ? a.taps.widx[ph][t] : wmax;
    }
  if (omax - omin != WS_HALO) return -22;
  args.rowmin = omin;
  args.nrows = WS_ROWS;
  args.wlo_off = (wmax + 1) * WS_KSTEPS * G::NWN * 64;
  if ((a.a_out || a.nb_colsum || a.pro_stats) &&
      (omin > 0 || omax < 0 || (args.ntiles - 1) * G::BM * SA + omin + WS_ROWS < a.Lin))
    return -22;
  if ((long)a.B * a.Lin >= (1L << 31) - 64 || (long)a.B * a.Lout >= (1L << 31) - 64) return -22;
  const size_t lds = 2 * WS_BUF_BYTES + WS_RAW_BYTES + (MODE == 3 ? 2 * 4 * WS_C * 8 : G::COMBINE == 2 ? 2 * 4 * 32 * 8 : 0);
  auto kern = sa_conv_ws_kernel<MODE, NT, HALO, CC, CO, SA, UU>;
  static bool attr_set = false;
  static int n_cu = 0;
  if (!attr_set) {
    hipError_t e = hipFuncSetAttribute(reinterpret_cast<const void*>(kern),
                                       hipFuncAttributeMaxDynamicSharedMemorySize, 160 * 1024);
    if (e != hipSuccess) return -(int)e;
    int dev = 0;
    hipDeviceProp_t prop;
    if (hipGetDevice(&dev) != hipSuccess || hipGetDeviceProperties(&prop, dev) != hipSuccess) return -19;
    n_cu = prop.multiProcessorCount;
    attr_set = true;
  }
  const int total = args.ntiles * a.B;
  const int nwg = total < n_cu ? total : n_cu;
  hipLaunchKernelGGL(kern, dim3(nwg), dim3(256), lds, st, args, total);
  hipError_t e = hipGetLastError();
  return e == hipSuccess ? 0 : -(int)e;
}

}

bool sa_conv_ws_covers(int dtype, int cin, int cout, int sa, int u, const SaConvArgs* a) {
  if (dtype == SA_BF16X3 && ((cin == 128 && cout == 64) || (cin == 64 && cout == 32)) && sa == 1 && u == 2) {
    if (a->taps.ntaps[0] > 3 || a->taps.ntaps[1] > 3 || a->taps.ntaps[0] < 1 || a->taps.ntaps[1] < 1) return false;
    int lo = 1 << 30, hi = -(1 << 30);
    for (int ph = 0; ph < 2; ++ph)
      for (int t = 0; t < a->taps.ntaps[ph]; ++t) {
        lo = a->taps.off[ph][t] < lo ? a->taps.off[ph][t] : lo;
        hi = a->taps.off[ph][t] > hi ? a->taps.off[ph][t] : hi;
      }
    if (hi - lo != 2 || lo > 0 || hi < 0) return false;
    if (a->tile_rows && a->tile_rows != 128) return false;
    return !a->s1 && !a->swish && !a->s2 && !a->t2 && !a->pro_stats && !a->nb_x && !a->ep_mode && !a->wscale && !a->relu;
  }
  const bool s2layer = cin == 64 && cout == 128 && sa == 2;
  if (dtype != SA_BF16X3 || u != 1 || !(s2layer || (cin == cout && sa == 1 && (cin == 128 || cin == 64)))) return false;
  const int nt = a->taps.ntaps[0];
  if (cin == 64 && (nt != 5 || a->s2 || a->t2 || a->pro_stats || a->nb_x)) return false;
  if ((nt != 5 && nt != 3) || a->wscale) return false;
  if (a->ep_mode) return false;
  int omin = 1 << 30, omax = -(1 << 30);
  for (int t = 0; t < nt; ++t) {
    omin = a->taps.off[0][t] < omin ? a->taps.off[0][t] : omin;
    omax = a->taps.off[0][t] > omax ? a->taps.off[0][t] : omax;
  }
  if (nt == 5 ? omax - omin != 4 : (omax - omin != 4 && omax - omin != 6)) return false;
  if ((a->a_out || a->nb_colsum || a->pro_stats) && (omin > 0 || (omin & 1))) return false;
  if (a->tile_rows && a->tile_rows != (cout == 64 ? 128 : 64)) return false;
  if (a->nb_x) return false;
  if (nt == 3)
    return !a->s1 && !a->swish && !a->pro_stats && (a->s2 || !a->t2);
  if ((a->s2 || a->t2) && (!a->s2 || !a->s1 || a->pro_stats)) return false;
  if (a->pro_stats && !a->s1) return false;
  if (a->s1) return a->t1 && a->swish;
  return !a->swish;
}

int sa_conv_ws_tile_rows(int cout) { return cout == 128 ? 64 : 128; }
int sa_conv_ws_rows_per_tile(int cout) { return cout == 128 ? 64 : cout == 64 ? 128 : 256; }

int sa_conv_ws_dispatch(int cin, int cout, const SaConvArgs* a, hipStream_t st) {
  if (cin == 128 && cout == 64) return launch_ws<0, 3, 2, 128, 64, 1, 2>(*a, st);
  if (cin == 64 && cout == 32) return launch_ws<0, 3, 2, 64, 32, 1, 2>(*a, st);
  if (cin == 64 && cout == 128) return a->s1 ? launch_ws<1, 5, 4, 64, 128, 2>(*a, st) : launch_ws<0, 5, 4, 64, 128, 2>(*a, st);
  if (cin == 64) return a->s1 ? launch_ws<1, 5, 4, 64>(*a, st) : launch_ws<0, 5, 4, 64>(*a, st);
  if (a->taps.ntaps[0] == 3) {
    int omin = 1 << 30, omax = -(1 << 30);
    for (int t = 0; t < 3; ++t) {
      omin = a->taps.off[0][t] < omin ? a->taps.off[0][t] : omin;
      omax = a->taps.off[0][t] > omax ? a->taps.off[0][t] : omax;
    }
    if (omax - omin == 4) return a->s2 ? launch_ws<5, 3, 4>(*a, st) : launch_ws<0, 3, 4>(*a, st);
    return a->s2 ? launch_ws<5, 3, 6>(*a, st) : launch_ws<0, 3, 6>(*a, st);
  }
  if (a->s1 && a->pro_stats) return launch_ws<3>(*a, st);
  if (a->s1 && a->s2) return launch_ws<4>(*a, st);
  if (a->s1) return launch_ws<1>(*a, st);
  return launch_ws<0>(*a, st);
}
```

### speech-anonymization_amd/csrc/sa_conv_wsd.hip

```cpp
#include "sa_conv_ws_common.h"

#ifdef SA_WSD_STAMPS
__device__ unsigned long long sa_wsd_dbg[64 * 16];
__device__ unsigned long long sa_wsd_wg[512 * 2];
#define WSD_WG_STAMP(i) do { if (lane_ == 0 && wave_ == 0 && blockIdx.x < 512) { \
  unsigned long long t_; asm volatile("s_memrealtime %0\n\ts_waitcnt lgkmcnt(0)" : "=s"(t_) :: "memory"); \
  sa_wsd_wg[blockIdx.x * 2 + (i)] = t_; } } while (0)
#define WSD_STAMP(it, i) do { if (lane_ == 0 && wave_ == 0 && blockIdx.x == 7 && (it) < 64) { \
  unsigned long long t_; asm volatile("s_memtime %0\n\ts_waitcnt lgkmcnt(0)" : "=s"(t_) :: "memory"); \
  sa_wsd_dbg[(it) * 16 + (i)] = t_; } } while (0)
#define WSD_STAMP_RT(it, i) do { if (lane_ == 0 && wave_ == 0 && blockIdx.x == 7 && (it) < 64) { \
  unsigned long long t_; asm volatile("s_memrealtime %0\n\ts_waitcnt lgkmcnt(0)" : "=s"(t_) :: "memory"); \
  sa_wsd_dbg[(it) * 16 + (i)] = t_; } } while (0)
extern "C" int sa_wsd_dbg_read(unsigned long long* out) {
  return -(int)hipMemcpyFromSymbol(out, HIP_SYMBOL(sa_wsd_dbg), sizeof(sa_wsd_dbg));
}
extern "C" int sa_wsd_wg_read(unsigned long long* out) {
  return -(int)hipMemcpyFromSymbol(out, HIP_SYMBOL(sa_wsd_wg), sizeof(sa_wsd_wg));
}
#else
#define WSD_STAMP(it, i)
#define WSD_STAMP_RT(it, i)
#define WSD_WG_STAMP(i)
#endif
// ... 612 lines not shown
            if constexpr (k < 3) piece_level(Tn, j, k);
            if constexpr (k == 3) piece_split(j, 0);
            if constexpr (k == 4) { piece_split(j, 1); piece_level(Tn, j, 3); }
            if constexpr (k == 5) piece_split(j, 2);
            if constexpr (k == Sch::KWH) { piece_write(j, 0); piece_split(j, 3); }
          } else {
            if constexpr (k == 0) { piece_level(Tn, j, 0); piece_split(j, 0); }
            if constexpr (k == 1) piece_split(j, 1);
            if constexpr (k == 2) piece_split(j, 2);
            if constexpr (k == Sch::KWH) { piece_write(j, 0); piece_split(j, 3); }
          }
          if constexpr (k == Sch::KR && p + 1 < np) piece_read(j + 1);
          if constexpr (k == Sch::KWL) piece_write(j, 1);
          if constexpr (k == Sch::KC) piece_cache(Tn, false, j);
          if constexpr (k == Sch::KD0) dma_piece(Tnn, false, j, 0);
          if constexpr (PRO2 && k == Sch::KD1) dma_piece(Tnn, false, j, 1);
        }
        if constexpr (PRO2 && sec == 1 && fs == Sch::T0 + Sch::NP1 * Sch::SUBS) colsum_put(it + 1);
        if constexpr (fs >= Sch::LB && fs < Sch::LB + 16) {
          epi_load(std::integral_constant<int, fs - Sch::LB>{}, xcur, gcur);
          if constexpr (fs - Sch::LB == 7) { WSD_STEP16(xcur); if constexpr (EP == 4) WSD_STEP16(gcur); }
        }
      };
      ws_static_for<0, 2 * Sch::NS>([&](auto S_c) {
        constexpr int S = decltype(S_c)::value, sec = S / Sch::NS, s = S % Sch::NS;
        constexpr int tp = s / WS_KSTEPS, k = s % WS_KSTEPS, sl = S & 1;
        constexpr bool more = S + 1 < 2 * Sch::NS;
        __builtin_amdgcn_sched_barrier(0);
#define WSD_MFMA(A, BC, B) asm volatile("v_mfma_f32_32x32x16_bf16 %0, %1, %2, %0" : "+v"(acc[sec]) : "v"(A), BC(B))
#define WSD_SLOT(I) __builtin_amdgcn_sched_barrier(0); \
        filler(std::integral_constant<int, sec>{}, std::integral_constant<int, 3 * s + (I)>{}); __builtin_amdgcn_sched_barrier(0)
#define WSD_MFMA_LIT(A, R) asm volatile("v_mfma_f32_32x32x16_bf16 %0, %1, a[" R "], %0" : "+v"(acc[sec]) : "v"(A))
        constexpr bool hand = s >= WS_NAGPR_FRAGS && s < WS_NAGPR_FRAGS + WS_NHAND;
        if constexpr (s == 0) {
          asm volatile("v_mfma_f32_32x32x16_bf16 %0, %1, %2, 0" : "=&v"(acc[sec]) : "v"(al), "a"(Bh[0][0]));
        } else if constexpr (s < WS_NAGPR_FRAGS) {
          WSD_MFMA(al, "a", Bh[tp][k]);
        } else if constexpr (hand) {
          if constexpr (s == 30) WSD_MFMA_LIT(al, "240:243"); else WSD_MFMA_LIT(al, "248:251");
        } else {
          WSD_MFMA(al, "v", Bh[tp][k]);
        }
        if constexpr (more) { __builtin_amdgcn_sched_barrier(0); load_a(S + 1); }
        WSD_SLOT(0);
        if constexpr (s < WS_NAGPR_FRAGS) {
          WSD_MFMA(ah[sl], "a", Bl[tp][k]); WSD_SLOT(1);
          WSD_MFMA(ah[sl], "a", Bh[tp][k]); WSD_SLOT(2);
        } else if constexpr (hand) {
          if constexpr (s == 30) { WSD_MFMA_LIT(ah[sl], "244:247"); WSD_SLOT(1); WSD_MFMA_LIT(ah[sl], "240:243"); WSD_SLOT(2); }
          else { WSD_MFMA_LIT(ah[sl], "252:255"); WSD_SLOT(1); WSD_MFMA_LIT(ah[sl], "248:251"); WSD_SLOT(2); }
        } else {
          WSD_MFMA(ah[sl], "v", Bl[tp][k]); WSD_SLOT(1);
          WSD_MFMA(ah[sl], "v", Bh[tp][k]); WSD_SLOT(2);
        }
#undef WSD_MFMA_LIT
#undef WSD_MFMA
#undef WSD_SLOT
      });
    };
    if (fast) {
      tile_body(std::true_type{});
      pend_issued = true;
      WSD_STAMP(it, 2);
    } else {
      tile_body(std::false_type{});
      asm volatile("s_nop 15\n\ts_nop 15\n\ts_nop 15\n\ts_nop 15" : "+v"(acc[0]), "+v"(acc[1]));
      epi_plain(std::integral_constant<int, 0>{}, Tc, yb_c, xb_c, gb_c);
      asm volatile("s_waitcnt vmcnt(0)" ::: "memory");
#pragma unroll
      for (int j = 0; j < WS_DPW; ++j) {
        piece_read(j);
#pragma unroll
        for (int q = 0; q < 4; ++q) piece_elem(Tn, edgeT, j, q);
        piece_write(j);
        piece_cache(Tn, edgeT, j);
      }
      asm volatile("s_waitcnt lgkmcnt(0)" ::: "memory");
#pragma unroll
      for (int j = 0; j < WS_DPW; ++j) dma_piece(Tnn, edgeD, j);
      pend_issued = false;
    }
    if (!fast) colsum_put(it + 1);
    WSD_STAMP(it, 3);
    asm volatile("s_waitcnt lgkmcnt(0)" ::: "memory");
    __builtin_amdgcn_s_barrier();
    WSD_STAMP(it, 4);
    cs_pending = t + 1 < last;
    Tp = Tc; Tc = Tn; Tn = Tnn;
  }
  {
    drain_vmem();
    asm volatile("s_nop 15\n\ts_nop 15\n\ts_nop 15\n\ts_nop 15" : "+v"(acc[0]), "+v"(acc[1]));
    stbase_p = const_cast<char*>(row_ptr(a.stats, last - 1, WS_C * 8));
    epi_plain(std::integral_constant<int, 1>{}, Tp, block8(a.y, Tp), block8(a.ep_x, Tp), EP == 4 ? block8(a.ep_g2, Tp) : nullptr);
    epi_stats();
  }
  WSD_STAMP(63, 3); WSD_STAMP_RT(63, 9); WSD_WG_STAMP(1);
#undef WS_IDS
#undef WSD_IMM
#undef WSD_Q
#undef WSD_STEP16
#undef WSD_XR0
}

template <int NT, int HALO, int PRO, int EP>
__global__ __launch_bounds__(256) __attribute__((amdgpu_waves_per_eu(1, 1))) __attribute__((amdgpu_num_vgpr(240)))
void sa_conv_wsd_kernel(SaConvArgs a, int total_tiles) {
  wsd_body<NT, HALO, PRO, EP>(a, total_tiles);
}

template <int NT, int HALO, int PRO, int EP>
int launch_wsd(const SaConvArgs& a, hipStream_t st) {
  typedef WsGeo<128, NT, HALO> G;
  SaConvArgs args = a;
  args.ntiles = sa_div_up(a.Lout, G::BM);
  int omin = 1 << 30, omax = -(1 << 30), wmax = 0;
  for (int t = 0; t < NT; ++t) {
    omin = a.taps.off[0][t] < omin ? a.taps.off[0][t] : omin;
    omax = a.taps.off[0][t] > omax ? a.taps.off[0][t] : omax;
    wmax = a.taps.widx[0][t] > wmax ? a.taps.widx[0][t] : wmax;
  }
  if (omax - omin != HALO) return -22;
  args.rowmin = omin;
  args.nrows = G::ROWS;
  args.wlo_off = (wmax + 1) * G::KSTEPS * 4 * 64;
  if ((a.a_out || a.nb_colsum) && (omin > 0 || omax < 0 || (args.ntiles - 1) * G::BM + omin + G::ROWS < a.Lin))
    return -22;
  if ((long)a.B * a.Lin >= (1L << 31) - 64 || (long)a.B * a.Lout >= (1L << 31) - 64) return -22;
  const size_t lds = 2 * G::BUF_BYTES + (PRO == 2 ? 2 : 1) * G::RAW_BYTES + (PRO == 2 ? 2 * 4 * 128 * 4 : 0);
  if (lds > 160 * 1024) return -12;
  auto kern = sa_conv_wsd_kernel<NT, HALO, PRO, EP>;
  static bool attr_set = false;
  static int n_cu = 0;
  if (!attr_set) {
    hipError_t e = hipFuncSetAttribute(reinterpret_cast<const void*>(kern),
                                       hipFuncAttributeMaxDynamicSharedMemorySize, 160 * 1024);
    if (e != hipSuccess) return -(int)e;
    int dev = 0;
    hipDeviceProp_t prop;
    if (hipGetDevice(&dev) != hipSuccess || hipGetDeviceProperties(&prop, dev) != hipSuccess) return -19;
    n_cu = prop.multiProcessorCount;
    attr_set = true;
  }
  const int total = args.ntiles * a.B;
  const int nwg = total < n_cu ? total : n_cu;
  hipLaunchKernelGGL(kern, dim3(nwg), dim3(256), lds, st, args, total);
  hipError_t e = hipGetLastError();
  return e == hipSuccess ? 0 : -(int)e;
}

int wsd_variant(int dtype, int cin, int cout, int sa, int u, const SaConvArgs* a) {
  if (dtype != SA_BF16X3 || cin != 128 || cout != 128 || sa != 1 || u != 1) return 0;
  if (a->ep_mode != 1 && a->ep_mode != 2) return 0;
  if (!a->ep_x || !a->ep_mean || !a->ep_rstd || !a->stats) return 0;
  if (a->s1 || a->t1 || a->s2 || a->t2 || a->swish || a->relu || a->pro_stats || a->wscale || a->bias) return 0;
  if (a->tile_rows && a->tile_rows != 64) return 0;
  const int nt = a->taps.ntaps[0];
  if (nt != 5 && nt != 3) return 0;
  int omin = 1 << 30, omax = -(1 << 30);
  for (int t = 0; t < nt; ++t) {
    omin = a->taps.off[0][t] < omin ? a->taps.off[0][t] : omin;
    omax = a->taps.off[0][t] > omax ? a->taps.off[0][t] : omax;
  }
  const int halo = omax - omin;
  if (nt == 5 ? halo != 4 : (halo != 4 && halo != 6)) return 0;
  if (omin > 0 || (omin & 1) || omax < 0) return 0;
  int pro, ep;
  if (a->nb_x) {
    if (!a->nb_c1 || !a->nb_c2 || !a->nb_c3) return 0;
    pro = 2;
  } else {
    if (a->a_out || a->nb_colsum) return 0;
    pro = 0;
  }
  if (a->ep_mode == 1) {
    if (!a->ep_s1 || !a->ep_t1 || a->ep_xp_is_act || a->ep_bstride != 128) return 0;
    if (a->ep_g2) { if (!a->ep_g2k1 || !a->ep_g2k2 || !a->ep_g2k3) return 0; ep = 4; } else ep = 1;
  } else {
    if (a->ep_g2 || a->ep_bstride != 0) return 0;
    if (a->ep_xp_is_act) { if (!a->ep_s1 || !a->ep_t1) return 0; ep = 3; } else { if (a->ep_s1 || a->ep_t1) return 0; ep = 2; }
  }
  if (pro == 2 && (a->nb_relu_mask != 0) != (ep != 1)) return 0;
  if (nt == 5 && pro == 2 && ep == 1) return 1;
  if (nt == 5 && pro == 2 && ep == 3) return 2;
  if (nt == 5 && pro == 0 && ep == 4) return 3;
  if (nt == 3 && halo == 4 && pro == 2 && ep == 2) return 4;
  if (nt == 3 && halo == 6 && pro == 2 && ep == 2) return 5;
  return 0;
}

}

bool sa_conv_wsd_covers(int dtype, int cin, int cout, int sa, int u, const SaConvArgs* a) {
  return wsd_variant(dtype, cin, cout, sa, u, a) != 0;
}

int sa_conv_wsd_dispatch(int cin, int cout, const SaConvArgs* a, hipStream_t st) {
  switch (wsd_variant(SA_BF16X3, cin, cout, 1, 1, a)) {
    case 1: return launch_wsd<5, 4, 2, 1>(*a, st);
    case 2: return launch_wsd<5, 4, 2, 3>(*a, st);
    case 3: return launch_wsd<5, 4, 0, 4>(*a, st);
    case 4: return launch_wsd<3, 4, 2, 2>(*a, st);
    case 5: return launch_wsd<3, 6, 2, 2>(*a, st);
    default: return -38;
  }
}
```

### speech-anonymization_amd/csrc/sa_small.hip

```cpp
#include "sa_common.h"

#define SA_K15 15
#define SA_C32 32

template <typename T>
__global__ __launch_bounds__(256) void sa_conv1toC_kernel(const float* __restrict__ x,
                                                          const float* __restrict__ w,
                                                          const float* __restrict__ bias,
                                                          T* __restrict__ y, int L, int flip,
                                                          float* __restrict__ stats, int ntiles,
                                                          const T* __restrict__ ep_x,
                                                          const float* __restrict__ ep_s1,
                                                          const float* __restrict__ ep_t1,
                                                          const float* __restrict__ ep_mean,
                                                          const float* __restrict__ ep_rstd) {
  constexpr int VEC = Tr<T>::VEC, CH = SA_C32 / VEC, PPP = 256 / CH, TILE = 512;
  __shared__ float xs[TILE + SA_K15 - 1];
  __shared__ __attribute__((aligned(16))) float ws[SA_K15][SA_C32];
  __shared__ float red[PPP][SA_C32][2];
  const int tid = threadIdx.x, b = blockIdx.y, l0 = blockIdx.x * TILE;
  for (int i = tid; i < TILE + SA_K15 - 1; i += 256) {
    const int g = l0 + i - 7;
    xs[i] = (g >= 0 && g < L) ? x[(size_t)b * L + g] : 0.0f;
  }
  for (int i = tid; i < SA_K15 * SA_C32; i += 256) {
    const int k = i / SA_C32, c = i % SA_C32;
    ws[k][c] = w[c * SA_K15 + (flip ? SA_K15 - 1 - k : k)];
  }
  __syncthreads();
  const int c = tid % CH, p0 = tid / CH;
  float bv[VEC], ssum[VEC], ssq[VEC];
#pragma unroll
  for (int j = 0; j < VEC; ++j) { bv[j] = bias ? bias[c * VEC + j] : 0.0f; ssum[j] = 0.f; ssq[j] = 0.f; }
  float es[VEC], et[VEC], em[VEC], er[VEC];
#pragma unroll
  for (int j = 0; j < VEC; ++j) {
    const size_t bc = (size_t)b * SA_C32 + c * VEC + j;
    es[j] = ep_x ? ep_s1[bc] : 1.0f; et[j] = ep_x ? ep_t1[bc] : 0.0f;
    em[j] = ep_x ? ep_mean[bc] : 0.0f; er[j] = ep_x ? ep_rstd[bc] : 0.0f;
  }
  for (int p = p0; p < TILE; p += PPP) {
    const int l = l0 + p;
    if (l >= L) break;
    float acc[VEC];
#pragma unroll
    for (int j = 0; j < VEC; ++j) acc[j] = bv[j];
#pragma unroll
    for (int k = 0; k < SA_K15; ++k) {
      const float xv = xs[p + k];
#pragma unroll
      for (int j = 0; j < VEC; ++j) acc[j] = fmaf(xv, ws[k][c * VEC + j], acc[j]);
    }
    float xn[VEC];
    if (ep_x) {
      float xv[VEC];
      Tr<T>::unpack(*reinterpret_cast<const uint4*>(ep_x + ((size_t)b * L + l) * SA_C32 + c * VEC), xv);
#pragma unroll
      for (int j = 0; j < VEC; ++j) {
        acc[j] *= sa_swish_grad(fmaf(xv[j], es[j], et[j]));
        xn[j] = (xv[j] - em[j]) * er[j];
      }
    }
    const uint4 u = Tr<T>::pack(acc);
    *reinterpret_cast<uint4*>(y + ((size_t)b * L + l) * SA_C32 + c * VEC) = u;
    if (stats) {
      float f[VEC];
      Tr<T>::unpack(u, f);
#pragma unroll
      for (int j = 0; j < VEC; ++j) { ssum[j] += f[j]; ssq[j] = fmaf(f[j], ep_x ? xn[j] : f[j], ssq[j]); }
    }
  }
  if (stats) {
#pragma unroll
    for (int j = 0; j < VEC; ++j) { red[p0][c * VEC + j][0] = ssum[j]; red[p0][c * VEC + j][1] = ssq[j]; }
    __syncthreads();
    if (tid < SA_C32) {
      float s = 0.f, q = 0.f;
      for (int r = 0; r < PPP; ++r) { s += red[r][tid][0]; q += red[r][tid][1]; }
      float* d = stats + (((size_t)b * ntiles + blockIdx.x) * SA_C32 + tid) * 2;
      d[0] = s; d[1] = q;
    }
  }
}

extern "C" int sa_conv1toC_ntiles(int L) { return sa_div_up(L, 512); }

extern "C" int sa_conv1toC(int dtype, const float* x, const float* w, const float* bias, void* y,
                           int B, int L, int flip, float* stats, const void* ep_x, const float* ep_s1,
                           const float* ep_t1, const float* ep_mean, const float* ep_rstd,
                           void* stream) {
  if (!x || !w || !y || B <= 0 || L <= 0) return -22;
  if (ep_x && (!ep_s1 || !ep_t1 || !ep_mean || !ep_rstd)) return -22;
  hipStream_t st = reinterpret_cast<hipStream_t>(stream);
  const int nt = sa_div_up(L, 512);
  dim3 grid(nt, B);
  if (dtype == SA_BF16)
    hipLaunchKernelGGL(sa_conv1toC_kernel<bf16_t>, grid, dim3(256), 0, st, x, w, bias,
                       reinterpret_cast<bf16_t*>(y), L, flip, stats, nt,
                       reinterpret_cast<const bf16_t*>(ep_x), ep_s1, ep_t1, ep_mean, ep_rstd);
  else
    hipLaunchKernelGGL(sa_conv1toC_kernel<float>, grid, dim3(256), 0, st, x, w, bias,
                       reinterpret_cast<float*>(y), L, flip, stats, nt,
                       reinterpret_cast<const float*>(ep_x), ep_s1, ep_t1, ep_mean, ep_rstd);
  hipError_t e = hipGetLastError();
  return e == hipSuccess ? 0 : -(int)e;
}

template <typename T>
__global__ __launch_bounds__(256) void sa_convCto1_kernel(const T* __restrict__ x,
                                                          const float* __restrict__ w,
                                                          const float* __restrict__ bias,
                                                          float* __restrict__ y, int L,
                                                          const float* __restrict__ s1,
                                                          const float* __restrict__ t1, int swish,
                                                          int flip) {
  constexpr int VEC = Tr<T>::VEC, CH = SA_C32 / VEC, RPP = 256 / CH, TILE = 128, PITCH = 36;
  constexpr int NPOS = TILE + SA_K15 - 1, NBLK = (NPOS + 15) / 16, TP = 17;
  constexpr int NIT = (NBLK * 16 + RPP - 1) / RPP;
  __shared__ __attribute__((aligned(16))) float xs[NBLK * 16 * PITCH];
  __shared__ float tp[NBLK * 16 * TP];
  const int tid = threadIdx.x, lane = tid & 63, wave = tid >> 6, b = blockIdx.y, l0 = blockIdx.x * TILE;
  {
    const int c = tid % CH, r0 = tid / CH;
    float sc[VEC], sh[VEC];
#pragma unroll
    for (int j = 0; j < VEC; ++j) {
      sc[j] = s1 ? s1[(size_t)b * SA_C32 + c * VEC + j] : 1.0f;
      sh[j] = t1 ? t1[(size_t)b * SA_C32 + c * VEC + j] : 0.0f;
    }
    uint4 raw[NIT];
#pragma unroll
    for (int i = 0; i < NIT; ++i) {
      const int r = r0 + i * RPP, g = l0 + r - 7;
      raw[i] = make_uint4(0, 0, 0, 0);
      if (r < NPOS && g >= 0 && g < L)
        raw[i] = *reinterpret_cast<const uint4*>(x + ((size_t)b * L + g) * SA_C32 + c * VEC);
    }
#pragma unroll
    for (int i = 0; i < NIT; ++i) {
      const int r = r0 + i * RPP, g = l0 + r - 7;
      if (r < NBLK * 16) {
        float f[VEC];
        Tr<T>::unpack(raw[i], f);
        const bool valid = r < NPOS && g >= 0 && g < L;
#pragma unroll
        for (int j = 0; j < VEC; ++j) {
          float v = fmaf(f[j], sc[j], sh[j]);
          v = swish ? sa_swish(v) : v;
          xs[r * PITCH + c * VEC + j] = valid ? v : 0.0f;
        }
      }
    }
  }
  const int n = lane & 15, kq = lane >> 4;
  float wb[8];
#pragma unroll
  for (int ks = 0; ks < 8; ++ks)
    wb[ks] = n < SA_K15 ? w[(ks * 4 + kq) * SA_K15 + (flip ? SA_K15 - 1 - n : n)] : 0.0f;
  __syncthreads();
  for (int blk = wave; blk < NBLK; blk += 4) {
    f32x4 acc = {0.f, 0.f, 0.f, 0.f};
    const float* ap = xs + (blk * 16 + n) * PITCH + kq;
#pragma unroll
    for (int ks = 0; ks < 8; ++ks) acc = __builtin_amdgcn_mfma_f32_16x16x4f32(ap[ks * 4], wb[ks], acc, 0, 0, 0);
#pragma unroll
    for (int i = 0; i < 4; ++i) tp[(blk * 16 + 4 * kq + i) * TP + n] = acc[i];
  }
  __syncthreads();
  const int l = l0 + tid;
  if (tid < TILE && l < L) {
    float acc = bias ? bias[0] : 0.0f;
#pragma unroll
    for (int k = 0; k < SA_K15; ++k) acc += tp[(tid + k) * TP + k];
    y[(size_t)b * L + l] = acc;
  }
}

extern "C" int sa_convCto1(int dtype, const void* x, const float* w, const float* bias, float* y,
                           int B, int L, const float* s1, const float* t1, int swish, int flip,
                           void* stream) {
  if (!x || !w || !y || B <= 0 || L <= 0) return -22;
  hipStream_t st = reinterpret_cast<hipStream_t>(stream);
  dim3 grid(sa_div_up(L, 128), B);
  if (dtype == SA_BF16)
    hipLaunchKernelGGL(sa_convCto1_kernel<bf16_t>, grid, dim3(256), 0, st,
                       reinterpret_cast<const bf16_t*>(x), w, bias, y, L, s1, t1, swish, flip);
  else
    hipLaunchKernelGGL(sa_convCto1_kernel<float>, grid, dim3(256), 0, st,
                       reinterpret_cast<const float*>(x), w, bias, y, L, s1, t1, swish, flip);
  hipError_t e = hipGetLastError();
  return e == hipSuccess ? 0 : -(int)e;
}

template <typename T>
__global__ __launch_bounds__(256) void sa_wgrad1C_kernel(const float* __restrict__ u,
                                                         const T* __restrict__ v,
                                                         float* __restrict__ slabs, int L,
                                                         int chunk, int flip,
                                                         const float* __restrict__ s1,
                                                         const float* __restrict__ t1, int swish) {
  constexpr int VEC = Tr<T>::VEC, CH = SA_C32 / VEC, RPP = 256 / CH, TILE = 256, PITCH = 33;
  __shared__ float us[TILE + SA_K15 - 1 + 1];
  __shared__ float vs[TILE * PITCH];
  const int tid = threadIdx.x, lane = tid & 63, wave = tid >> 6, b = blockIdx.y;
  const int lbeg = blockIdx.x * chunk;
// ... 289 lines not shown
```

### speech-anonymization_amd/ops.py

```python
import collections
import ctypes as C
import functools

import torch

from . import _lib as L

UP2 = [[(1, 0), (0, 2), (-1, 4)], [(1, 1), (0, 3)]]


def taps_conv(K, dil, pad):
    return [[(k * dil - pad, k) for k in range(K)]]


def taps_conv_dgrad_s1(K, dil, pad):
    return [[(pad - k * dil, k) for k in range(K)]]


def taps_convT_dgrad(K=5, pad=2):
    return [[(k - pad, k) for k in range(K)]]


CONVT_WG_TAPS = [(1, 0), (1, 1), (0, 0), (0, 1), (-1, 0)]

# ... 22 lines not shown
        return 2 * Lout if self.stride == 2 else Lout - 2 * self.pad + self.dil * (self.K - 1)

    @functools.lru_cache(maxsize=256)
    def fwd(self, Lin):
        if self.transposed:
            return self.cin, self.cout, 1, 2, UP2, 2 * Lin
        return self.cin, self.cout, self.stride, 1, taps_conv(self.K, self.dil, self.pad), self.lout(Lin)

    @functools.lru_cache(maxsize=256)
    def dgrad(self, Lin):
        if self.transposed:
            return self.cout, self.cin, 2, 1, taps_convT_dgrad(), Lin
        if self.stride == 2:
            return self.cout, self.cin, 1, 2, UP2, Lin
        return self.cout, self.cin, 1, 1, taps_conv_dgrad_s1(self.K, self.dil, self.pad), Lin

    @functools.lru_cache(maxsize=256)
    def wgrad(self, Lin):
        if self.transposed:
            return self.cin, self.cout, 1, 2, CONVT_WG_TAPS, Lin, (self.cout * self.K, self.K, 1)
        return (self.cin, self.cout, self.stride, 1, [(k * self.dil - self.pad, 0) for k in range(self.K)],
                self.lout(Lin), (self.K, self.cin * self.K, 1))


def conv_layers(model, roots):
    return {f"{r}.{n}": ConvGeom.of(f"{r}.{n}", m) for r in roots for n, m in model.get_submodule(r).named_children()
            if isinstance(m, (torch.nn.Conv1d, torch.nn.ConvTranspose1d)) and min(m.in_channels, m.out_channels) > 1}


def _f(t):
    return L.ptr(t)


class _Profile:

    def __init__(self):
        self.key, self.kinds = None, {}

    def enable(self, key):
        self.key, self.kinds = key, {}

    def start(self, key):
        if key != self.key:
            return None
        e = torch.cuda.Event(enable_timing=True)
        e.record()
        return e

    def stop(self, e0, nbytes, flops, alg_bytes=None, kind=""):
        e1 = torch.cuda.Event(enable_timing=True)
        e1.record()
        k = self.kinds.setdefault(kind, {"ev": [], "bytes": 0, "alg_bytes": 0, "flops": 0})
        k["ev"].append((e0, e1))
        k["bytes"] += nbytes
        k["alg_bytes"] += nbytes if alg_bytes is None else alg_bytes
        k["flops"] += flops

    def collect(self):
        torch.cuda.synchronize()
        out = []
        for kind, k in self.kinds.items():
            out.append({"kernel": kind or self.key, "family": self.key, "launches": len(k["ev"]),
                        "ms": sum(a.elapsed_time(b) for a, b in k["ev"]), "bytes": k["bytes"],
                        "alg_bytes": k["alg_bytes"], "flops": k["flops"]})
        out.sort(key=lambda r: -r["ms"])
        self.key, self.kinds = None, {}
        return out


PROFILE = _Profile()


PRECISIONS = {"f32": (torch.float32, L.F32), "bf16": (torch.bfloat16, L.BF16),
              "bf16x3": (torch.float32, L.BF16X3), "bf16x1f": (torch.float32, L.BF16X1F),
              "fp8": (torch.bfloat16, L.FP8)}
WGRAD_CODE = {"f32": L.F32, "bf16": L.BF16, "bf16x3": L.BF16X1F, "bf16x1f": L.BF16X1F, "fp8": L.BF16}
DGRAD_CODE = {"f32": L.F32, "bf16": L.BF16, "bf16x3": L.BF16X3, "bf16x1f": L.BF16X1F, "fp8": L.BF16}


def _pack_geometry(shape, kind):
    if kind in ("conv_fwd", "conv_dgrad"):
        Cout, Cin, Kw = shape
        if kind == "conv_fwd":
            return Kw, Cin, Cout, Kw, Cin * Kw
        return Kw, Cout, Cin, Cin * Kw, Kw
    Cin, Cout, Kw = shape
    if kind == "convT_fwd":
        return Kw, Cin, Cout, Cout * Kw, Kw
    return Kw, Cout, Cin, Kw, Cout * Kw


def _image_buffer(code, dtype, n, device):
    if code == L.FP8:
        return torch.empty(n + 4, dtype=torch.uint8, device=device)
    if code == L.BF16X3:
        return torch.empty(2 * n, dtype=torch.bfloat16, device=device)
    if code in (L.BF16X1F, L.BF16):
        return torch.empty(n, dtype=torch.bfloat16, device=device)
    return torch.empty(n, dtype=torch.float32, device=device)


def pack_weights(w, kind, dtype, code=None):
    lib = L.load()
    code = L.dt_code(dtype) if code is None else code
    Kw, K, N, sk, sn = _pack_geometry(w.shape, kind)
    out = _image_buffer(code, dtype, Kw * K * N, w.device)
    L.check(lib.sa_pack_weights(code, _f(w), _f(out), Kw, K, N, sk, sn, 1, L.stream()),
            "sa_pack_weights")
    return out


class PackedWeights:

    def __init__(self, items, dtype):
        self.images, descs = {}, (L.SaPackDesc * len(items))()
        dev = items[0][1].device
        for d, (tag, w, kind, code) in zip(descs, items):
            Kw, K, N, sk, sn = _pack_geometry(w.shape, kind)
            img = _image_buffer(code, dtype, Kw * K * N, dev)
            self.images[tag] = (img, code)
            d.src, d.dst, d.dtype = w.data_ptr(), img.data_ptr(), code
            d.ntaps, d.K, d.N, d.sk, d.sn, d.st = Kw, K, N, sk, sn, 1
            d.scale = img.data_ptr() + Kw * K * N if code == L.FP8 else None
            self.fp8 = getattr(self, "fp8", False) or code == L.FP8
        raw = torch.frombuffer(bytearray(bytes(descs)), dtype=torch.uint8)
        self.table = raw.to(dev)
        self.n = len(items)
        self.key = tuple(w.data_ptr() for _, w, _, _ in items)

    def refresh(self):
        if getattr(self, "fp8", False):
            L.check(L.load().sa_pack_scales_multi(_f(self.table), self.n, L.stream()), "sa_pack_scales_multi")
        L.check(L.load().sa_pack_weights_multi(_f(self.table), self.n, 64, L.stream()),
                "sa_pack_weights_multi")


@functools.lru_cache(maxsize=None)
def _conv_geometry(cin, cout, u, Lout):
    return L.load().sa_conv_gemm_ntiles(cin, cout, u, Lout)


def conv_impl(pingpong=False, tile_rows=0, ws=True):
    if pingpong:
        raise L.SaHipError("the ping-pong conv kernel was removed (it tied the one-tile kernel forward and lost "
                           "on the fused data gradients: DESIGN.md section 4); use ws=True or ws=False")
    lib = L.load()
    L.check(lib.sa_conv_gemm_set_impl(2 if ws else 0), "sa_conv_gemm_set_impl")
    L.check(lib.sa_conv_gemm_set_tile_rows(int(tile_rows)), "sa_conv_gemm_set_tile_rows")
    _conv_geometry.cache_clear()


def conv_gemm(x, wp, bias, cin, cout, sa, u, phases, Lout, s1=None, t1=None, s2=None, t2=None,
              swish=False, relu=False, want_stats=False, out=None, code=None, ep=None, a_out=None,
              nb=None, want_pro_stats=False):
    lib = L.load()
    B, Lin, _ = x.shape
    assert x.shape[2] == cin
    y = out if out is not None else torch.empty(B, Lout, cout, dtype=x.dtype, device=x.device)
    kc = L.dt_code(x.dtype) if code is None else code
    nt = _conv_geometry(cin, cout, u, Lout)
    stats = torch.empty(B, nt, cout, 2, dtype=torch.float32, device=x.device) if want_stats else None
    a = L.SaConvArgs()
    a.x, a.wp, a.bias, a.y = _f(x), _f(wp), _f(bias), _f(y)
    a.s1, a.t1, a.s2, a.t2 = _f(s1), _f(t1), _f(s2), _f(t2)
    a.swish, a.relu, a.stats = int(swish), int(relu), _f(stats)
    a.B, a.Lin, a.Lout = B, Lin, Lout
    a.taps = L.make_taps(phases)
    if kc == L.FP8:
        a.wscale = C.c_void_p(wp.data_ptr() + wp.numel() - 4)
    if a_out is not None:
        assert a_out.dtype == torch.bfloat16 and a_out.shape == x.shape
        a.a_out = _f(a_out)
    pro_stats = None
    if want_pro_stats:
        pro_stats = torch.empty(B, nt, cin, 2, dtype=torch.float32, device=x.device)
        a.pro_stats = _f(pro_stats)
    colsum = None
    if nb:
        assert nb["x"].shape == x.shape and nb["x"].dtype == x.dtype
        a.nb_x, a.nb_c1, a.nb_c2, a.nb_c3 = _f(nb["x"]), _f(nb["c1"]), _f(nb["c2"]), _f(nb["c3"])
        a.nb_bstride, a.nb_relu_mask = (0 if nb.get("per_c") else cin), int(bool(nb.get("relu_mask")))
        if nb.get("want_colsum"):
            colsum = torch.empty(B, nt, cin, dtype=torch.float32, device=x.device)
            a.nb_colsum = _f(colsum)
    if ep:
        a.ep_mode, a.ep_xp_is_act = int(ep["mode"]), int(bool(ep.get("xp_is_act")))
        a.ep_bstride = 0 if ep.get("per_c") else cout
        a.ep_x, a.ep_g2 = _f(ep["x"]), _f(ep.get("g2"))
        a.ep_s1, a.ep_t1 = _f(ep.get("s1")), _f(ep.get("t1"))
        a.ep_mean, a.ep_rstd = _f(ep.get("mean")), _f(ep.get("rstd"))
        if ep.get("g2k") is not None:
            a.ep_g2k1, a.ep_g2k2, a.ep_g2k3 = (_f(t) for t in ep["g2k"])
    e0 = PROFILE.start(f"conv_gemm({cin},{cout},{sa},{u})") if PROFILE.key else None
    L.check(lib.sa_conv_gemm(kc, cin, cout, sa, u, C.byref(a), L.stream()),
            f"sa_conv_gemm({cin},{cout},{sa},{u})")
    if e0 is not None:
        ntap = sum(len(p) for p in phases)
        esz = x.element_size()
        extra = (a_out.numel() * 2 if a_out is not None else 0)
        if ep:
            extra += y.numel() * esz * (2 if ep.get("g2") is not None else 1)
        if nb:
            extra += x.numel() * esz
        io = (x.numel() + y.numel()) * esz
        route = lib.sa_conv_gemm_route(kc, cin, cout, sa, u, C.byref(a))
        tname = {L.F32: "float", L.BF16: "bf16_t", L.BF16X3: "bf16x3_t", L.BF16X1F: "bf16x1f_t", L.FP8: "fp8_t"}[kc]
        ws_mode = (5 if s2 is not None else 0) if s1 is None else 3 if want_pro_stats else 4 if s2 is not None else 1
        kind = (f"sa_conv_wsd_kernel ({tname}, {cin}->{cout}; 5 instances)" if route == 3 else
                f"sa_conv_ws_kernel<{ws_mode},{ntap}> ({tname}, {cin}->{cout})" if route == 2 else
                f"sa_conv_gemm_kernel<{tname},{cin},{cout},{sa},{u}{',nb prologue' if nb else ''}>")
        PROFILE.stop(e0, io + ntap * cin * cout * esz + extra,
                     2 * B * (-(-Lout // u)) * ntap * cin * cout,
                     alg_bytes=io + (y.numel() * esz if ep else 0), kind=kind)
    out_t = (y, stats) if want_stats else (y,)
    if nb and nb.get("want_colsum"):
        out_t = out_t + (colsum,)
    if want_pro_stats:
        out_t = out_t + (pro_stats,)
    return out_t if len(out_t) > 1 else y


WGRAD_TARGET_WGS = {True: 256, False: 512}


def wgrad(x, dy, cin, cout, sa, u, taps, Mrows, dst, dst_strides, s1=None, t1=None, s2=None,
          t2=None, swish=False, accumulate=False, target_wgs=None, code=None, x_pre=False,
          dy_pre=False, defer=None):
    lib = L.load()
    B, Lin, _ = x.shape
    Ldy = dy.shape[1]
    if x_pre:
        assert x.dtype == torch.bfloat16 and code in (L.BF16X1F, L.BF16)
    nt = len(taps)
    kw = lib.sa_wgrad_kw(cin, cout)
    if target_wgs is None:
        target_wgs = WGRAD_TARGET_WGS[(cin // 32) * (cout // 32) >= 8]
    chunk = max(64, -(-Mrows * B // target_wgs))
    chunk = -(-chunk // 64) * 64
    nchunk = -(-Mrows // chunk)
    slabs = torch.empty(B * nchunk * kw * nt * cin * cout, dtype=torch.float32, device=x.device)
    a = L.SaWgradArgs()
    a.x, a.dy, a.slabs = _f(x), _f(dy), _f(slabs)
    a.s1, a.t1, a.s2, a.t2, a.swish = _f(s1), _f(t1), _f(s2), _f(t2), int(swish)
    a.B, a.Lin, a.Ldy, a.Mrows, a.chunk, a.nchunk, a.ntaps = B, Lin, Ldy, Mrows, chunk, nchunk, nt
    for i, (off, ph) in enumerate(taps):
        a.off[i], a.ph[i] = off, ph
    a.x_pre, a.dy_pre = int(x_pre), int(dy_pre)
    if dy_pre:
        assert x_pre and dy.dtype == torch.bfloat16
    L.check(lib.sa_wgrad((L.BF16X1F if dy_pre else L.dt_code(dy.dtype)) if code is None else code, cin, cout, sa, u,
                         C.byref(a), L.stream()),
            f"sa_wgrad({cin},{cout},{sa},{u})")
    sk, sn, st = dst_strides
    if defer is not None:
        defer.append((slabs, dst, B * nchunk * kw, nt, cin, cout, sk, sn, st, int(accumulate)))
        return dst
    L.check(lib.sa_wgrad_reduce(_f(slabs), _f(dst), B * nchunk * kw, nt, cin, cout, sk, sn, st,
                                int(accumulate), L.stream()), "sa_wgrad_reduce")
    return dst


def wgrad_reduce_multi(items):
    lib = L.load()
    for i0 in range(0, len(items), L.WRED_MAX):
        m = L.SaWredMulti()
        chunk = items[i0:i0 + L.WRED_MAX]
        m.n = len(chunk)
        for d, (slabs, dst, nslab, nt, cin, cout, sk, sn, st, acc) in zip(m.d, chunk):
            d.slabs, d.dst = slabs.data_ptr(), dst.data_ptr()
            d.nslab, d.ntaps, d.cin, d.cout, d.sk, d.sn, d.st, d.accumulate = nslab, nt, cin, cout, sk, sn, st, acc
        L.check(lib.sa_wgrad_reduce_multi(C.byref(m), L.stream()), "sa_wgrad_reduce_multi")


def conv1toC(x, w, bias, dtype, flip=False, want_stats=False, ep=None):
    lib = L.load()
    B, Ln = x.shape
    y = torch.empty(B, Ln, 32, dtype=dtype, device=x.device)
    nt = lib.sa_conv1toC_ntiles(Ln)
    stats = torch.empty(B, nt, 32, 2, dtype=torch.float32, device=x.device) if want_stats else None
    e = ep or {}
    L.check(lib.sa_conv1toC(L.dt_code(dtype), _f(x), _f(w), _f(bias), _f(y), B, Ln, int(flip),
                            _f(stats), _f(e.get("x")), _f(e.get("s1")), _f(e.get("t1")),
                            _f(e.get("mean")), _f(e.get("rstd")), L.stream()), "sa_conv1toC")
    return (y, stats) if want_stats else y


def convCto1(x, w, bias, s1=None, t1=None, swish=False, flip=False):
    lib = L.load()
    B, Ln, _ = x.shape
    y = torch.empty(B, Ln, dtype=torch.float32, device=x.device)
    L.check(lib.sa_convCto1(L.dt_code(x.dtype), _f(x), _f(w), _f(bias), _f(y), B, Ln, _f(s1), _f(t1),
                            int(swish), int(flip), L.stream()), "sa_convCto1")
    return y


def wgrad1C(u, v, dst, flip=False, s1=None, t1=None, swish=False, accumulate=False, chunk=2048):
    lib = L.load()
    B, Ln = u.shape
    nch = lib.sa_wgrad1C_nchunk(Ln, chunk)
    slabs = torch.empty(B * nch, 32 * 15, dtype=torch.float32, device=u.device)
    L.check(lib.sa_wgrad1C(L.dt_code(v.dtype), _f(u), _f(v), _f(slabs), B, Ln, chunk, int(flip),
                           _f(s1), _f(t1), int(swish), L.stream()), "sa_wgrad1C")
    L.check(lib.sa_sum_slabs(_f(slabs), _f(dst), B * nch, 32 * 15, int(accumulate), L.stream()),
            "sa_sum_slabs")
    return dst


def bwd1C(u, v, w, dst, s1, t1, mean, rstd, flip=True, accumulate=False, chunk=2048):
    lib = L.load()
    B, Ln = u.shape
    nch = lib.sa_wgrad1C_nchunk(Ln, chunk)
    g = torch.empty(B, Ln, 32, dtype=v.dtype, device=u.device)
    stats = torch.empty(B, lib.sa_conv1toC_ntiles(Ln), 32, 2, dtype=torch.float32, device=u.device)
    slabs = torch.empty(B * nch, 32 * 15, dtype=torch.float32, device=u.device)
    L.check(lib.sa_bwd1C(L.dt_code(v.dtype), _f(u), _f(v), _f(w), _f(g), _f(stats), _f(slabs), B, Ln, chunk,
                         int(flip), _f(s1), _f(t1), _f(mean), _f(rstd), L.stream()), "sa_bwd1C")
    L.check(lib.sa_sum_slabs(_f(slabs), _f(dst), B * nch, 32 * 15, int(accumulate), L.stream()),
            "sa_sum_slabs")
    return g, stats, dst


def sum_partials(part, nbatch, n=None, rows=False):
    lib = L.load()
    if n is None:
        n = part.shape[-2] * part.shape[-1]
    total = part.numel()
    nslab = total // (nbatch * n)
    if nbatch == 1 and nslab >= 512 and part.dim() == 4 and part.shape[0] > 1:
        R = part.shape[0]
        mid = torch.empty(R, n, dtype=torch.float64, device=part.device)
        L.check(lib.sa_sum_partials(_f(part), _f(mid), R, nslab // R, n, L.stream()), "sa_sum_partials")
        if rows:
            return mid
        out = torch.empty(1, n, dtype=torch.float64, device=part.device)
        L.check(lib.sa_sum_rows_d(_f(mid), _f(out), R, n, L.stream()), "sa_sum_rows_d")
        return out
    out = torch.empty(nbatch, n, dtype=torch.float64, device=part.device)
    L.check(lib.sa_sum_partials(_f(part), _f(out), nbatch, nslab, n, L.stream()), "sa_sum_partials")
    return out


def fin_in_fwd(sums, B, Cc, n, gamma, beta, eps=1e-5):
    lib = L.load()
    o = torch.empty(4, B, Cc, dtype=torch.float32, device=sums.device)
    L.check(lib.sa_fin_in_fwd(_f(sums), B, Cc, n, _f(gamma), _f(beta), C.c_float(eps), _f(o[0]),
                              _f(o[1]), _f(o[2]), _f(o[3]), L.stream()), "sa_fin_in_fwd")
    return o[0], o[1], o[2], o[3]


def fin_bn_fwd(sums, Cc, count, gamma, beta, run_mean=None, run_var=None, eps=1e-5, momentum=0.1,
               count_dev=None):
    lib = L.load()
    o = torch.empty(4, Cc, dtype=torch.float32, device=sums.device)
    L.check(lib.sa_fin_bn_fwd(_f(sums), sums.numel() // (2 * Cc), Cc, C.c_double(count), _f(gamma), _f(beta), C.c_float(eps),
                              C.c_float(momentum), _f(run_mean), _f(run_var), _f(o[0]), _f(o[1]),
                              _f(o[2]), _f(o[3]), _f(count_dev), L.stream()), "sa_fin_bn_fwd")
    return o[0], o[1], o[2], o[3]


def fin_bn_eval(Cc, gamma, beta, run_mean, run_var, eps=1e-5):
    lib = L.load()
    o = torch.empty(4, Cc, dtype=torch.float32, device=gamma.device)
# ... 671 lines not shown
```

Measured before the change: 3.956 million frames/s.

## Recompute encoder.0 conv inside the next conv GEMM instead of materialising it

```diff
diff --git a/include/sa_hip.h b/include/sa_hip.h
--- a/include/sa_hip.h
+++ b/include/sa_hip.h
@@ -42,6 +42,8 @@
   float* pro_stats;
   const float* wscale;
   int tile_rows; int pad2_;
+  const float* gen_x; const float* gen_w; const float* gen_b;
+  int gen_in; int gen_ep;
 } SaConvArgs;
 
 int sa_conv_gemm(int dtype, int cin, int cout, int sa, int u, const SaConvArgs* a, void* stream);
diff --git a/speech-anonymization_amd/_lib.py b/speech-anonymization_amd/_lib.py
--- a/speech-anonymization_amd/_lib.py
+++ b/speech-anonymization_amd/_lib.py
@@ -30,7 +30,8 @@
                 ("nb_x", vp), ("nb_c1", vp), ("nb_c2", vp), ("nb_c3", vp),
                 ("nb_bstride", C.c_int), ("nb_relu_mask", C.c_int), ("nb_colsum", vp),
                 ("ep_g2k1", vp), ("ep_g2k2", vp), ("ep_g2k3", vp), ("pro_stats", vp), ("wscale", vp),
-                ("tile_rows", C.c_int), ("pad2_", C.c_int)]
+                ("tile_rows", C.c_int), ("pad2_", C.c_int),
+                ("gen_x", vp), ("gen_w", vp), ("gen_b", vp), ("gen_in", C.c_int), ("gen_ep", C.c_int)]
 
 
 class SaPackDesc(C.Structure):
diff --git a/speech-anonymization_amd/convae.py b/speech-anonymization_amd/convae.py
--- a/speech-anonymization_amd/convae.py
+++ b/speech-anonymization_amd/convae.py
@@ -80,6 +80,7 @@
         self.sync_bn = sync_bn
         self.fused_head = os.environ.get("SA_FUSED_HEAD", "1") == "1"
         self.fused_bwd1c = os.environ.get("SA_FUSED_BWD1C", "1") == "1"
+        self.recompute_enc0 = os.environ.get("SA_RECOMPUTE_ENC0", "1") == "1"
         self.dp_batch_sizes = None
 
     def forward(self, feats):
@@ -106,7 +107,7 @@
         x0, B, T, Ltot = _input_rows(feats)
         P = dict(zip(*self._named_params()))
         cg, inorm = _launchers(self, P, _packed(self, P), B)
-        y, _, _ = _encoder_launches(self, P, cg, inorm, x0, Ltot, False)
+        y, _, _ = _encoder_launches(self, P, cg, inorm, x0, Ltot, False, _recompute_enc0(self, False, False))
         return _decoder_launches(self, P, cg, inorm, y[5], Ltot)[-1].view(B, T, 80)
 
     def _side_stream(self, device):
@@ -222,11 +223,17 @@
     return d
 
 
+def _recompute_enc0(model, needs_grad, cache_a):
+    return (model.recompute_enc0 and model.kcode in (L.BF16X3, L.F32) and
+            (not needs_grad or (cache_a and model.dgrad_kcode in (L.BF16X3, L.F32))))
+
+
 def _launchers(model, P, W, B, A=None):
     def cg(ly, x, **kw):
+        shape = x.shape if x is not None else kw["gen"]["x"].shape + (ly.cin,)
         if A is not None and P[ly.key].requires_grad:
-            A[ly.key] = kw["a_out"] = torch.empty(x.shape, dtype=torch.bfloat16, device=x.device)
-        return _conv(x, W[ly.key, ly.kinds[0]], P[ly.bias], *ly.fwd(x.shape[1]), **kw)
+            A[ly.key] = kw["a_out"] = torch.empty(shape, dtype=torch.bfloat16, device=P[ly.key].device)
+        return _conv(x, W[ly.key, ly.kinds[0]], P[ly.bias], *ly.fwd(shape[1]), **kw)
 
     def inorm(stats, n, prefix, C):
         sums = ops.sum_partials(stats, B)
@@ -234,10 +241,18 @@
     return cg, inorm
 
 
-def _encoder_launches(model, P, cg, inorm, x0, Ltot, want_pro_stats):
+def _enc0_gen(P, x0):
+    return dict(x=x0, w=P["encoder.0.weight"], b=P["encoder.0.bias"])
+
+
+def _encoder_launches(model, P, cg, inorm, x0, Ltot, want_pro_stats, gen0=False):
     L2, L4, lay = Ltot // 2, Ltot // 4, model.lay
-    y0 = ops.conv1toC(x0, P["encoder.0.weight"], P["encoder.0.bias"], model.act_dtype)
-    y1, st = cg(lay["encoder.2"], y0, swish=True, want_stats=True)
+    if gen0:
+        y0 = None
+        y1, st = cg(lay["encoder.2"], None, swish=True, want_stats=True, gen=_enc0_gen(P, x0))
+    else:
+        y0 = ops.conv1toC(x0, P["encoder.0.weight"], P["encoder.0.bias"], model.act_dtype)
+        y1, st = cg(lay["encoder.2"], y0, swish=True, want_stats=True)
     n1 = inorm(st, L2, "encoder.3", 64)
     y2, st = cg(lay["encoder.5"], y1, s1=n1[2], t1=n1[3], swish=True, want_stats=True)
     n2 = inorm(st, L2, "encoder.6", 64)
@@ -299,7 +314,9 @@
         La, Lb, Lc = L4 - 4, L4 - 8, L4 - 14
         gc = model._bn_global_counts([B * L4, B * La, B * Lb, B * Lc, B, B], feats.device) if train else None
         cdev = lambda i: None if gc is None else gc[i:i + 1]
-        (y0, y1, y2, y3, y4, y5), (n1, n2, n3, n4), a4_stats = _encoder_launches(model, P, cg, inorm, x0, Ltot, train)
+        gen0 = _recompute_enc0(model, train and any(ctx.needs_input_grad), cache_a)
+        (y0, y1, y2, y3, y4, y5), (n1, n2, n3, n4), a4_stats = _encoder_launches(model, P, cg, inorm, x0, Ltot, train,
+                                                                                 gen0)
         bn_n = bn_stats(a4_stats if train else None, B * L4, cls.norm, "sex_classifier.norm", 128, 0)
         r0, st = cg(lay["sex_classifier.tdnn.0"], y4, s1=n4[2], t1=n4[3], swish=True, s2=bn_n[2], t2=bn_n[3],
                     relu=True, want_stats=True)
@@ -360,7 +377,7 @@
         n1, n2, n3, n4, n6, n8 = S["n"][1], S["n"][2], S["n"][3], S["n"][4], S["n"][6], S["n"][8]
         bn_n, bn0, bn1, bn2 = S["bn"]
         f1, f2 = S["f"]
-        dev = y0.device
+        dev = y1.device
         G = {k: None for k in names}
         need = {k: p.requires_grad for k, p in P.items()}
         need_stage = {st: any(v for k, v in need.items() if k.startswith(st))
@@ -592,7 +609,8 @@
             ly = lay[conv]
             g = in_finish(g, st, y, nrm, ly.cout, y.shape[1], norm, ly.bias)
             conv_wgrad(ly, x, g, swish=True, **(dict(s1=nx[2], t1=nx[3]) if nx else {}))
-            g, st = cg(ly, g, want_stats=True, ep=_in_ep(x, nx) if nx else dict(mode=1, x=x))
+            g, st = cg(ly, g, want_stats=True, ep=_in_ep(x, nx) if nx else
+                       dict(mode=1, x=x) if x is not None else dict(mode=1, gen=_enc0_gen(P, S["x0"])))
         bias_from(st, "encoder.0.bias", 32)
         if need["encoder.0.weight"]:
             G["encoder.0.weight"] = ops.wgrad1C(S["x0"], g, newg("encoder.0.weight"))
diff --git a/speech-anonymization_amd/csrc/sa_conv_gemm.hip b/speech-anonymization_amd/csrc/sa_conv_gemm.hip
--- a/speech-anonymization_amd/csrc/sa_conv_gemm.hip
+++ b/speech-anonymization_amd/csrc/sa_conv_gemm.hip
@@ -2,397 +2,19 @@
 #include "sa_common.h"
 
 #include "sa_conv_cfg.h"
+#include "sa_enc0.h"
 
 template <typename T, int CIN, int COUT, int SA, int U, int TM, bool PRO2>
 __global__ __launch_bounds__(256, 2) void sa_conv_gemm_kernel(SaConvArgs a, int red_off, int col_off) {
-  typedef ConvCfg<T, CIN, COUT, SA, U, TM> C;
-  typedef Pol<T> P;
-  typedef typename P::store_t S;
-  typedef typename P::lds_t LT;
-  typedef typename P::Frag Frag;
-  typedef Tr<S> tr;
-  constexpr int VEC = C::VEC, OVEC = C::OVEC;
-  extern __shared__ __attribute__((aligned(16))) unsigned char smem[];
-  LT* As = reinterpret_cast<LT*>(smem);
-  S* Os = reinterpret_cast<S*>(smem);
-  float* red = reinterpret_cast<float*>(smem + red_off);
-  const int plane = a.nrows * C::APITCH;
-
-  const int tid = threadIdx.x, lane = tid & 63, wave = tid >> 6;
-  const int tile = blockIdx.x, b = blockIdx.y;
-  const int m0 = tile * C::BMB;
-
-  {
-    const int c = tid % C::CHI, r0 = tid / C::CHI;
-    float s1[VEC], t1[VEC], s2[VEC], t2[VEC];
-#pragma unroll
-    for (int j = 0; j < VEC; ++j) {
-      s1[j] = a.s1 ? a.s1[(size_t)b * CIN + c * VEC + j] : 1.0f;
-      t1[j] = a.t1 ? a.t1[(size_t)b * CIN + c * VEC + j] : 0.0f;
-      s2[j] = a.s2 ? a.s2[c * VEC + j] : 1.0f;
-      t2[j] = a.t2 ? a.t2[c * VEC + j] : 0.0f;
-    }
-    const bool has1 = a.s1 != nullptr, has2 = a.s2 != nullptr, sw = a.swish != 0;
-    const S* xb = reinterpret_cast<const S*>(a.x) + (size_t)b * a.Lin * CIN + c * VEC;
-    const int gbase = m0 * SA + a.rowmin;
-    const int own_lo = m0 * SA;
-    int own_hi = tile == a.ntiles - 1 ? a.Lin : (m0 + C::BMB) * SA;
-    if (own_hi > a.Lin) own_hi = a.Lin;
-    constexpr int NIT = ((C::BMB - 1) * SA + 1 + SA_MAX_HALO + C::RPPI - 1) / C::RPPI;
-    uint4 raw[NIT];
-#pragma unroll
-    for (int i = 0; i < NIT; ++i) {
-      const int r = r0 + i * C::RPPI, g = gbase + r;
-      raw[i] = make_uint4(0, 0, 0, 0);
-      if (r < a.nrows && g >= 0 && g < a.Lin) raw[i] = *reinterpret_cast<const uint4*>(xb + (size_t)g * CIN);
-    }
-    uint4 raw2[PRO2 ? NIT : 1];
-    float k1[VEC], k2[VEC], k3[VEC], csum[VEC];
-    if constexpr (PRO2) {
-      const S* x2 = reinterpret_cast<const S*>(a.nb_x) + (size_t)b * a.Lin * CIN + c * VEC;
-#pragma unroll
-      for (int i = 0; i < NIT; ++i) {
-        const int r = r0 + i * C::RPPI, g = gbase + r;
-        raw2[i] = make_uint4(0, 0, 0, 0);
-        if (r < a.nrows && g >= 0 && g < a.Lin) raw2[i] = *reinterpret_cast<const uint4*>(x2 + (size_t)g * CIN);
-      }
-#pragma unroll
-      for (int j = 0; j < VEC; ++j) {
-        const size_t q = (size_t)b * a.nb_bstride + c * VEC + j;
-        k1[j] = a.nb_c1[q]; k2[j] = a.nb_c2[q]; k3[j] = a.nb_c3[q]; csum[j] = 0.0f;
-      }
-    }
-    auto stage_rows = [&](auto xform) {
-#pragma unroll
-      for (int i = 0; i < NIT; ++i) {
-        const int r = r0 + i * C::RPPI, g = gbase + r;
-        if (r < a.nrows) {
-          float f[VEC];
-          tr::unpack(raw[i], f);
-          if (g >= 0 && g < a.Lin) xform(f, i, g);
-          LT* dst = As + (size_t)r * C::APITCH + c * VEC;
-          if constexpr (P::NPL == 2) {
-            uint2 hi, lo;
-            sa_split4(f, hi, lo);
-            *reinterpret_cast<uint2*>(dst) = hi;
-            *reinterpret_cast<uint2*>(dst + plane) = lo;
-          } else if constexpr (sizeof(LT) == 1) {
-            *reinterpret_cast<uint2*>(dst) = sa_pack_fp8x8(f);
-          } else if constexpr (sizeof(LT) == 2 && sizeof(S) == 4) {
-            *reinterpret_cast<uint2*>(dst) = sa_pack_bf16x4(f);
-          } else if constexpr (sizeof(LT) == 2) {
-            *reinterpret_cast<uint4*>(dst) = tr::pack(f);
-          } else {
-            float* d = reinterpret_cast<float*>(dst);
-            d[0] = f[0]; d[1] = f[1]; d[2] = f[2]; d[3] = f[3];
-          }
-        }
-      }
-    };
-    if constexpr (PRO2) {
-      stage_rows([&](float* f, int i, int g) {
-        float y[VEC];
-        tr::unpack(raw2[i], y);
-        const bool own = g >= own_lo && g < own_hi;
-#pragma unroll
-        for (int j = 0; j < VEC; ++j) {
-          float v = fmaf(k1[j], f[j], fmaf(k2[j], y[j], k3[j]));
-          if (a.nb_relu_mask && !(y[j] > 0.0f)) v = 0.0f;
-          f[j] = v;
-          if (own) csum[j] += v;
-        }
-      });
-      if (a.nb_colsum) {
-        float* colred = reinterpret_cast<float*>(smem + col_off);
-#pragma unroll
-        for (int j = 0; j < VEC; ++j) {
-          float v = csum[j];
-          for (int off = C::CHI; off < 64; off <<= 1) v += __shfl_xor(v, off, 64);
-          if (lane < C::CHI) colred[wave * CIN + (lane % C::CHI) * VEC + j] = v;
-        }
-      }
-    } else if (!has1 && !has2 && !sw) {
-      stage_rows([](float*, int, int) {});
-    } else if (has1 && sw && !has2 && a.pro_stats) {
-      float ps[VEC], pq[VEC];
-#pragma unroll
-      for (int j = 0; j < VEC; ++j) { ps[j] = 0.0f; pq[j] = 0.0f; }
-      stage_rows([&](float* f, int, int g) {
-        const bool own = g >= own_lo && g < own_hi;
-#pragma unroll
-        for (int j = 0; j < VEC; ++j) {
-          const float v = sa_swish(fmaf(f[j], s1[j], t1[j]));
-          f[j] = v;
-          if (own) { ps[j] += v; pq[j] = fmaf(v, v, pq[j]); }
-        }
-      });
-      float* colred = reinterpret_cast<float*>(smem + col_off);
-#pragma unroll
-      for (int j = 0; j < VEC; ++j) {
-        float v = ps[j], w = pq[j];
-        for (int off = C::CHI; off < 64; off <<= 1) { v += __shfl_xor(v, off, 64); w += __shfl_xor(w, off, 64); }
-        if (lane < C::CHI) {
-          colred[(wave * CIN + (lane % C::CHI) * VEC + j) * 2 + 0] = v;
-          colred[(wave * CIN + (lane % C::CHI) * VEC + j) * 2 + 1] = w;
-        }
-      }
-    } else if (has1 && sw && !has2) {
-      stage_rows([&](float* f, int, int) {
-#pragma unroll
-        for (int j = 0; j < VEC; ++j) f[j] = sa_swish(fmaf(f[j], s1[j], t1[j]));
-      });
-    } else {
-      stage_rows([&](float* f, int, int) {
-#pragma unroll
-        for (int j = 0; j < VEC; ++j) {
-          float v = f[j];
-          if (has1) v = fmaf(v, s1[j], t1[j]);
-          if (sw) v = sa_swish(v);
-          if (has2) v = fmaf(v, s2[j], t2[j]);
-          f[j] = v;
-        }
-      });
-    }
-  }
-  __syncthreads();
-  if (!PRO2 && a.pro_stats && tid < CIN) {
-    const float* colred = reinterpret_cast<const float*>(smem + col_off);
-    float* d = a.pro_stats + (((size_t)b * a.ntiles + tile) * CIN + tid) * 2;
-#pragma unroll
-    for (int q = 0; q < 2; ++q)
-      d[q] = (colred[tid * 2 + q] + colred[(CIN + tid) * 2 + q]) +
-             (colred[(2 * CIN + tid) * 2 + q] + colred[(3 * CIN + tid) * 2 + q]);
-  }
-  if constexpr (PRO2) {
-    if (a.nb_colsum && tid < CIN) {
-      const float* colred = reinterpret_cast<const float*>(smem + col_off);
-      a.nb_colsum[((size_t)b * a.ntiles + tile) * CIN + tid] =
-          (colred[tid] + colred[CIN + tid]) + (colred[2 * CIN + tid] + colred[3 * CIN + tid]);
-    }
-  }
-  if constexpr (sizeof(LT) == 2) {
-    if (a.a_out) {
-      constexpr int CH16 = CIN / 8;
-      const int own_lo = m0 * SA;
-      int own_hi = tile == a.ntiles - 1 ? a.Lin : (m0 + C::BMB) * SA;
-      if (own_hi > a.Lin) own_hi = a.Lin;
-      const int rlo = own_lo - (m0 * SA + a.rowmin);
-      bf16_t* ao = reinterpret_cast<bf16_t*>(a.a_out) + ((size_t)b * a.Lin + own_lo) * CIN;
-      for (int e = tid; e < (own_hi - own_lo) * CH16; e += 256) {
-        const int r = e / CH16, c = e % CH16;
-        *reinterpret_cast<uint4*>(ao + (size_t)r * CIN + c * 8) =
-            *reinterpret_cast<const uint4*>(As + (size_t)(rlo + r) * C::APITCH + c * 8);
-      }
-    }
-  }
-
-  const int wn = wave % C::WN, wm = wave / C::WN;
-  f32x16 acc[C::VPW][C::MT];
-#pragma unroll
-  for (int v = 0; v < C::VPW; ++v)
-#pragma unroll
-    for (int mt = 0; mt < C::MT; ++mt)
-#pragma unroll
-      for (int i = 0; i < 16; ++i) acc[v][mt][i] = 0.0f;
-
-  constexpr int KUP = P::NPL == 2 ? 2 : 8;
-  constexpr int KU = C::KSTEPS < KUP ? C::KSTEPS : KUP;
-  constexpr int GPT = C::KSTEPS / KU;
-  static_assert(C::KSTEPS % KU == 0, "k-steps per tap must be a multiple of the prefetch group");
-  const Frag* wp = reinterpret_cast<const Frag*>(a.wp);
-#pragma unroll
-  for (int v = 0; v < C::VPW; ++v) {
-    const int vt = wn + v * C::WN;
-    const int ph = vt / C::NT, nt = vt % C::NT;
-    const int G = a.taps.ntaps[ph] * GPT;
-    const LT* abase = As + (size_t)((wm * C::MT * 32 + (lane & 31)) * SA - a.rowmin) * C::APITCH
-                      + (lane >> 5) * (C::KS / 2);
-    auto load_group = [&](Frag (&dst)[P::NPL][KU], int g) {
-      const int ti = g / GPT, kg = g % GPT;
-      const Frag* wt = wp + (((size_t)a.taps.widx[ph][ti] * C::KSTEPS + kg * KU) * C::NT + nt) * 64 + lane;
-#pragma unroll
-      for (int ku = 0; ku < KU; ++ku) {
-        dst[0][ku] = wt[(size_t)ku * C::NT * 64];
-        if constexpr (P::NPL == 2) dst[1][ku] = wt[(size_t)a.wlo_off + (size_t)ku * C::NT * 64];
-      }
-    };
-    auto compute_group = [&](const Frag (&bq)[P::NPL][KU], int g) {
-      const int ti = g / GPT, kg = g % GPT;
-      const LT* arow = abase + (size_t)a.taps.off[ph][ti] * C::APITCH + kg * KU * C::KS;
-      Frag ah[2][C::MT], al[2][C::MT];
-      auto load_a = [&](int slot, int ku) {
-#pragma unroll
-        for (int mt = 0; mt < C::MT; ++mt) {
-          const LT* ap = arow + (size_t)mt * 32 * SA * C::APITCH + ku * C::KS;
-          ah[slot][mt] = *reinterpret_cast<const Frag*>(ap);
-          if constexpr (P::NPL == 2) al[slot][mt] = *reinterpret_cast<const Frag*>(ap + plane);
-        }
-      };
-      load_a(0, 0);
-#pragma unroll
-      for (int ku = 0; ku < KU; ++ku) {
-        if (ku + 1 < KU) load_a((ku + 1) & 1, ku + 1);
-#pragma unroll
-        for (int mt = 0; mt < C::MT; ++mt) {
-          if constexpr (P::NPL == 2) {
-            acc[v][mt] = __builtin_amdgcn_mfma_f32_32x32x16_bf16(al[ku & 1][mt], bq[0][ku], acc[v][mt], 0, 0, 0);
-            acc[v][mt] = __builtin_amdgcn_mfma_f32_32x32x16_bf16(ah[ku & 1][mt], bq[1][ku], acc[v][mt], 0, 0, 0);
-            acc[v][mt] = __builtin_amdgcn_mfma_f32_32x32x16_bf16(ah[ku & 1][mt], bq[0][ku], acc[v][mt], 0, 0, 0);
-          } else {
-            acc[v][mt] = Tr<LT>::mfma(ah[ku & 1][mt], bq[0][ku], acc[v][mt]);
-          }
-        }
-      }
-    };
-    Frag b0[P::NPL][KU], b1[P::NPL][KU];
-    load_group(b0, 0);
-    for (int g = 0; g < G; g += 2) {
-      if (g + 1 < G) load_group(b1, g + 1);
-      compute_group(b0, g);
-      if (g + 1 < G) {
-        if (g + 2 < G) load_group(b0, g + 2);
-        compute_group(b1, g + 1);
-      }
-    }
-  }
-  constexpr int NOT = TM / C::RPPO;
-  const int ec = tid % C::CHO, er0 = tid / C::CHO;
-  __syncthreads();
-
-#pragma unroll
-  for (int v = 0; v < C::VPW; ++v) {
-    const int vt = wn + v * C::WN;
-    const int ph = vt / C::NT, nt = vt % C::NT;
-    const int col = nt * 32 + (lane & 31);
-    const float bv = a.bias ? a.bias[col] : 0.0f;
-    float winv = 1.0f;
-    if constexpr (sizeof(LT) == 1) winv = a.wscale ? 1.0f / a.wscale[0] : 1.0f;
-#pragma unroll
-    for (int mt = 0; mt < C::MT; ++mt) {
-#pragma unroll
-      for (int i = 0; i < 16; ++i) {
-        const int m = wm * C::MT * 32 + mt * 32 + sa_acc_row(i, lane);
-        float val = sizeof(LT) == 1 ? fmaf(acc[v][mt][i], winv, bv) : acc[v][mt][i] + bv;
-        if (a.relu) val = fmaxf(val, 0.0f);
-        Os[(size_t)(m * U + ph) * C::OPITCH + col] = tr::from_f(val);
-      }
-    }
-  }
-  __syncthreads();
-  {
-    const int c = ec, r0 = er0;
-    float ssum[OVEC], ssq[OVEC], es1[OVEC], et1[OVEC], emu[OVEC], ers[OVEC];
-#pragma unroll
-    for (int j = 0; j < OVEC; ++j) {
-      ssum[j] = 0.0f; ssq[j] = 0.0f;
-      es1[j] = (a.ep_mode && a.ep_s1) ? a.ep_s1[(size_t)b * COUT + c * OVEC + j] : 1.0f;
-      et1[j] = (a.ep_mode && a.ep_t1) ? a.ep_t1[(size_t)b * COUT + c * OVEC + j] : 0.0f;
-      emu[j] = (a.ep_mode && a.ep_mean) ? a.ep_mean[(size_t)b * a.ep_bstride + c * OVEC + j] : 0.0f;
-      ers[j] = (a.ep_mode && a.ep_rstd) ? a.ep_rstd[(size_t)b * a.ep_bstride + c * OVEC + j] : 1.0f;
-    }
-    const bool g2k = a.ep_mode && a.ep_g2 && a.ep_g2k1;
-    float gk1[OVEC], gk2[OVEC], gk3[OVEC];
-#pragma unroll
-    for (int j = 0; j < OVEC; ++j) {
-      gk1[j] = g2k ? a.ep_g2k1[c * OVEC + j] : 1.0f;
-      gk2[j] = g2k ? a.ep_g2k2[c * OVEC + j] : 0.0f;
-      gk3[j] = g2k ? a.ep_g2k3[c * OVEC + j] : 0.0f;
-    }
-    S* yb = reinterpret_cast<S*>(a.y) + (size_t)b * a.Lout * COUT + c * OVEC;
-    const S* xe = a.ep_mode ? reinterpret_cast<const S*>(a.ep_x) + (size_t)b * a.Lout * COUT + c * OVEC : nullptr;
-    const S* ge = (a.ep_mode && a.ep_g2) ? reinterpret_cast<const S*>(a.ep_g2) + (size_t)b * a.Lout * COUT + c * OVEC : nullptr;
-    const int o0 = m0 * U;
-    auto ep_rows = [&](uint4 u, const uint4& epx, const uint4& epg, int o) {
-      float g[OVEC], x[OVEC], g2[OVEC], xn[OVEC];
-      tr::unpack(u, g); tr::unpack(epx, x); tr::unpack(epg, g2);
-#pragma unroll
-      for (int j = 0; j < OVEC; ++j) {
-        const float z = fmaf(x[j], es1[j], et1[j]);
-        if (g2k) g2[j] = fmaf(gk1[j], g2[j], fmaf(gk2[j], sa_swish(z), gk3[j]));
-        float gg = g[j] + g2[j];
-        if (a.ep_mode == 1) gg *= sa_swish_grad(z);
-        const float xv = a.ep_xp_is_act ? sa_swish(z) : x[j];
-        xn[j] = (xv - emu[j]) * ers[j];
-        g[j] = gg;
-      }
-      u = tr::pack(g);
-      *reinterpret_cast<uint4*>(yb + (size_t)o * COUT) = u;
-      if (a.stats) {
-        tr::unpack(u, g);
-#pragma unroll
-        for (int j = 0; j < OVEC; ++j) { ssum[j] += g[j]; ssq[j] = fmaf(g[j], xn[j], ssq[j]); }
-      }
-    };
-    if (a.ep_mode && o0 + TM <= a.Lout) {
-      auto run = [&](auto has_g2_c) {
-        constexpr bool HG = decltype(has_g2_c)::value;
-        constexpr int D = NOT < 2 ? NOT : 2;
-        uint4 px[D], pg[D];
-#pragma unroll
-        for (int d = 0; d < D; ++d) {
-          px[d] = *reinterpret_cast<const uint4*>(xe + (size_t)(o0 + r0 + d * C::RPPO) * COUT);
-          pg[d] = make_uint4(0, 0, 0, 0);
-          if constexpr (HG) pg[d] = *reinterpret_cast<const uint4*>(ge + (size_t)(o0 + r0 + d * C::RPPO) * COUT);
-        }
-#pragma unroll
-        for (int i = 0; i < NOT; ++i) {
-          const int r = r0 + i * C::RPPO, o = o0 + r;
-          const uint4 epx = px[i % D], epg = pg[i % D];
-          if (i + D < NOT) {
-            px[i % D] = *reinterpret_cast<const uint4*>(xe + (size_t)(o + D * C::RPPO) * COUT);
-            if constexpr (HG) pg[i % D] = *reinterpret_cast<const uint4*>(ge + (size_t)(o + D * C::RPPO) * COUT);
-          }
-          const uint4 u = *reinterpret_cast<const uint4*>(Os + (size_t)r * C::OPITCH + c * OVEC);
-          ep_rows(u, epx, epg, o);
-        }
-      };
-      if (ge) run(std::true_type{}); else run(std::false_type{});
-    } else {
-#pragma unroll
-    for (int i = 0; i < NOT; ++i) {
-      const int r = r0 + i * C::RPPO, o = o0 + r;
-      if (o < a.Lout) {
-        uint4 u = *reinterpret_cast<const uint4*>(Os + (size_t)r * C::OPITCH + c * OVEC);
-        if (a.ep_mode) {
-          const uint4 epx = *reinterpret_cast<const uint4*>(xe + (size_t)o * COUT);
-          const uint4 epg = ge ? *reinterpret_cast<const uint4*>(ge + (size_t)o * COUT) : make_uint4(0, 0, 0, 0);
-          ep_rows(u, epx, epg, o);
-        } else {
-          *reinterpret_cast<uint4*>(yb + (size_t)o * COUT) = u;
-          if (a.stats) {
-            float f[OVEC];
-            tr::unpack(u, f);
-#pragma unroll
-            for (int j = 0; j < OVEC; ++j) { ssum[j] += f[j]; ssq[j] = fmaf(f[j], f[j], ssq[j]); }
-          }
-        }
-      }
-    }
-    }
-    if (a.stats) {
-      __syncthreads();
-#pragma unroll
-      for (int j = 0; j < OVEC; ++j) {
-        red[((size_t)r0 * COUT + c * OVEC + j) * 2 + 0] = ssum[j];
-        red[((size_t)r0 * COUT + c * OVEC + j) * 2 + 1] = ssq[j];
-      }
-    }
-  }
-  if (a.stats) {
-    __syncthreads();
-    if (tid < COUT) {
-      float s = 0.0f, q = 0.0f;
-      for (int r = 0; r < C::RPPO; ++r) {
-        s += red[((size_t)r * COUT + tid) * 2 + 0];
-        q += red[((size_t)r * COUT + tid) * 2 + 1];
-      }
-      float* dst = a.stats + (((size_t)b * a.ntiles + tile) * COUT + tid) * 2;
-      dst[0] = s; dst[1] = q;
-    }
-  }
+  constexpr int GEN = 0;
+#include "sa_conv_gemm_body.inc"
+}
+template <typename T, int CIN, int COUT, int SA, int U, int TM, bool PRO2, int GEN>
+__global__ __launch_bounds__(256, 2) void sa_conv_gemm_gen_kernel(SaConvArgs a, int red_off, int col_off) {
+#include "sa_conv_gemm_body.inc"
 }
 
-template <typename T, int CIN, int COUT, int SA, int U, int TM, bool PRO2 = false>
+template <typename T, int CIN, int COUT, int SA, int U, int TM, bool PRO2 = false, int GEN = 0>
 static int launch_cfg(const SaConvArgs& a, hipStream_t st) {
   typedef ConvCfg<T, CIN, COUT, SA, U, TM> C;
   SaConvArgs args = a;
@@ -418,9 +40,16 @@
   if (PRO2 && (!a.nb_c1 || !a.nb_c2 || !a.nb_c3)) return -22;
   if (a.pro_stats && (PRO2 || !a.s1 || !a.swish || a.s2)) return -22;
   const size_t tile_lds = C::lds_bytes(args.nrows);
-  const size_t lds = tile_lds + (PRO2 ? 4 * CIN * sizeof(float) : a.pro_stats ? 8 * CIN * sizeof(float) : 0);
+  size_t lds = tile_lds + (PRO2 ? 4 * CIN * sizeof(float) : a.pro_stats ? 8 * CIN * sizeof(float) : 0);
+  if (GEN) {
+    constexpr int NIT = ((C::BMB - 1) * SA + 1 + SA_MAX_HALO + C::RPPI - 1) / C::RPPI;
+    const int nx = (GEN == 1 ? NIT * C::RPPI : TM) + SA_ENC0_K - 1;
+    lds = tile_lds + (PRO2 ? 4 : 8) * CIN * sizeof(float) + SA_ENC0_LDS_FLOATS(nx) * sizeof(float);
+  }
   if (lds > 160 * 1024) return -12;
-  auto kern = sa_conv_gemm_kernel<T, CIN, COUT, SA, U, TM, PRO2>;
+  void (*kern)(SaConvArgs, int, int);
+  if constexpr (GEN != 0) kern = sa_conv_gemm_gen_kernel<T, CIN, COUT, SA, U, TM, PRO2, GEN>;
+  else kern = sa_conv_gemm_kernel<T, CIN, COUT, SA, U, TM, PRO2>;
   static bool attr_set = false;
   if (!attr_set) {
     hipError_t e = hipFuncSetAttribute(reinterpret_cast<const void*>(kern),
@@ -525,11 +154,31 @@
 extern "C" int sa_conv_gemm(int dtype, int cin, int cout, int sa, int u, const SaConvArgs* a,
                             void* stream) {
   hipStream_t st = reinterpret_cast<hipStream_t>(stream);
-  if (!a || !a->x || !a->wp || !a->y || a->B <= 0 || a->Lin <= 0 || a->Lout <= 0) return -22;
-  if (a->ep_mode < 0 || a->ep_mode > 2 || (a->ep_mode && !a->ep_x)) return -22;
+  if (!a || (!a->x && !a->gen_in) || !a->wp || !a->y || a->B <= 0 || a->Lin <= 0 || a->Lout <= 0) return -22;
+  if (a->ep_mode < 0 || a->ep_mode > 2 || (a->ep_mode && !a->ep_x && !a->gen_ep)) return -22;
   const int route = conv_route(dtype, cin, cout, sa, u, a);
   if (route == 2) return sa_conv_ws_dispatch(cin, cout, a, st);
   if (route == 3) return sa_conv_wsd_dispatch(cin, cout, a, st);
+  if (a->gen_in || a->gen_ep) {
+    if (!a->gen_x || !a->gen_w || (a->gen_in && a->gen_ep)) return -22;
+    if (dtype != SA_BF16X3 && dtype != SA_F32) return -22;
+    if (a->gen_in && (cin != 32 || a->nb_x)) return -22;
+    if (a->gen_ep && (cout != 32 || a->ep_mode != 1)) return -22;
+    if (a->gen_in && cout == 64 && sa == 2 && u == 1) {
+      const int tm = (a->tile_rows == 64 || a->tile_rows == 128) ? a->tile_rows : tile_rows(cin, cout, u);
+      if (dtype == SA_BF16X3)
+        return tm == 64 ? launch_cfg<bf16x3_t, 32, 64, 2, 1, 64, false, 1>(*a, st)
+                        : launch_cfg<bf16x3_t, 32, 64, 2, 1, 128, false, 1>(*a, st);
+      return tm == 64 ? launch_cfg<float, 32, 64, 2, 1, 64, false, 1>(*a, st)
+                      : launch_cfg<float, 32, 64, 2, 1, 128, false, 1>(*a, st);
+    }
+    if (a->gen_ep && cin == 64 && sa == 1 && u == 2) {
+      if (a->nb_x) return dtype == SA_BF16X3 ? launch_cfg<bf16x3_t, 64, 32, 1, 2, 128, true, 2>(*a, st) : -22;
+      return dtype == SA_BF16X3 ? launch_cfg<bf16x3_t, 64, 32, 1, 2, 128, false, 2>(*a, st)
+                                : launch_cfg<float, 64, 32, 1, 2, 128, false, 2>(*a, st);
+    }
+    return -38;
+  }
   SA_CONV_CASE(32, 64, 2, 1)
   SA_CONV_CASE(64, 64, 1, 1)
   SA_CONV_CASE(64, 128, 2, 1)
diff --git a/speech-anonymization_amd/csrc/sa_conv_gemm_body.inc b/speech-anonymization_amd/csrc/sa_conv_gemm_body.inc
--- /dev/null
+++ b/speech-anonymization_amd/csrc/sa_conv_gemm_body.inc
@@ -0,0 +1,419 @@
+  typedef ConvCfg<T, CIN, COUT, SA, U, TM> C;
+  typedef Pol<T> P;
+  typedef typename P::store_t S;
+  typedef typename P::lds_t LT;
+  typedef typename P::Frag Frag;
+  typedef Tr<S> tr;
+  constexpr int VEC = C::VEC, OVEC = C::OVEC;
+  extern __shared__ __attribute__((aligned(16))) unsigned char smem[];
+  LT* As = reinterpret_cast<LT*>(smem);
+  S* Os = reinterpret_cast<S*>(smem);
+  float* red = reinterpret_cast<float*>(smem + red_off);
+  const int plane = a.nrows * C::APITCH;
+
+  const int tid = threadIdx.x, lane = tid & 63, wave = tid >> 6;
+  const int tile = blockIdx.x, b = blockIdx.y;
+  const int m0 = tile * C::BMB;
+  static_assert(GEN == 0 || (sizeof(S) == 4 && (GEN == 1 ? CIN : COUT) == SA_ENC0_C && !(GEN == 1 && PRO2)),
+                "generated rows: fp32 storage, 32 channels");
+  float* gens = reinterpret_cast<float*>(smem + col_off + (PRO2 ? 4 : 8) * CIN * sizeof(float));
+  SaEnc0Regs genr;
+  if constexpr (GEN == 2)
+    genr = sa_enc0_load(a.gen_x, a.gen_w, a.gen_b, b, a.Lout, m0 * U - SA_ENC0_PAD, TM + SA_ENC0_K - 1, tid);
+
+  {
+    const int c = tid % C::CHI, r0 = tid / C::CHI;
+    float s1[VEC], t1[VEC], s2[VEC], t2[VEC];
+#pragma unroll
+    for (int j = 0; j < VEC; ++j) {
+      s1[j] = a.s1 ? a.s1[(size_t)b * CIN + c * VEC + j] : 1.0f;
+      t1[j] = a.t1 ? a.t1[(size_t)b * CIN + c * VEC + j] : 0.0f;
+      s2[j] = a.s2 ? a.s2[c * VEC + j] : 1.0f;
+      t2[j] = a.t2 ? a.t2[c * VEC + j] : 0.0f;
+    }
+    const bool has1 = a.s1 != nullptr, has2 = a.s2 != nullptr, sw = a.swish != 0;
+    const S* xb = reinterpret_cast<const S*>(a.x) + (size_t)b * a.Lin * CIN + c * VEC;
+    const int gbase = m0 * SA + a.rowmin;
+    const int own_lo = m0 * SA;
+    int own_hi = tile == a.ntiles - 1 ? a.Lin : (m0 + C::BMB) * SA;
+    if (own_hi > a.Lin) own_hi = a.Lin;
+    constexpr int NIT = ((C::BMB - 1) * SA + 1 + SA_MAX_HALO + C::RPPI - 1) / C::RPPI;
+    uint4 raw[NIT];
+    if constexpr (GEN == 1) {
+      constexpr int NX = NIT * C::RPPI + SA_ENC0_K - 1;
+      static_assert(NX <= 512, "sa_enc0_load stages at most 512 samples");
+      sa_enc0_stage(gens, sa_enc0_load(a.gen_x, a.gen_w, a.gen_b, b, a.Lin, gbase - SA_ENC0_PAD, NX, tid), NX, tid);
+      __syncthreads();
+      float bv[VEC];
+#pragma unroll
+      for (int j = 0; j < VEC; ++j) bv[j] = gens[SA_ENC0_K * SA_ENC0_C + c * VEC + j];
+      sa_enc0_chunks<S, NIT>(gens + SA_ENC0_LDS_FLOATS(0) + r0, C::RPPI, gens + c * VEC, bv, raw);
+#pragma unroll
+      for (int i = 0; i < NIT; ++i) {
+        const int r = r0 + i * C::RPPI, g = gbase + r;
+        if (!(r < a.nrows && g >= 0 && g < a.Lin)) raw[i] = make_uint4(0, 0, 0, 0);
+      }
+    } else {
+#pragma unroll
+      for (int i = 0; i < NIT; ++i) {
+        const int r = r0 + i * C::RPPI, g = gbase + r;
+        raw[i] = make_uint4(0, 0, 0, 0);
+        if (r < a.nrows && g >= 0 && g < a.Lin) raw[i] = *reinterpret_cast<const uint4*>(xb + (size_t)g * CIN);
+      }
+    }
+    uint4 raw2[PRO2 ? NIT : 1];
+    float k1[VEC], k2[VEC], k3[VEC], csum[VEC];
+    if constexpr (PRO2) {
+      const S* x2 = reinterpret_cast<const S*>(a.nb_x) + (size_t)b * a.Lin * CIN + c * VEC;
+#pragma unroll
+      for (int i = 0; i < NIT; ++i) {
+        const int r = r0 + i * C::RPPI, g = gbase + r;
+        raw2[i] = make_uint4(0, 0, 0, 0);
+        if (r < a.nrows && g >= 0 && g < a.Lin) raw2[i] = *reinterpret_cast<const uint4*>(x2 + (size_t)g * CIN);
+      }
+#pragma unroll
+      for (int j = 0; j < VEC; ++j) {
+        const size_t q = (size_t)b * a.nb_bstride + c * VEC + j;
+        k1[j] = a.nb_c1[q]; k2[j] = a.nb_c2[q]; k3[j] = a.nb_c3[q]; csum[j] = 0.0f;
+      }
+    }
+    if constexpr (GEN == 2) sa_enc0_stage(gens, genr, TM + SA_ENC0_K - 1, tid);
+    auto stage_rows = [&](auto xform) {
+#pragma unroll
+      for (int i = 0; i < NIT; ++i) {
+        const int r = r0 + i * C::RPPI, g = gbase + r;
+        if (r < a.nrows) {
+          float f[VEC];
+          tr::unpack(raw[i], f);
+          if (g >= 0 && g < a.Lin) xform(f, i, g);
+          LT* dst = As + (size_t)r * C::APITCH + c * VEC;
+          if constexpr (P::NPL == 2) {
+            uint2 hi, lo;
+            sa_split4(f, hi, lo);
+            *reinterpret_cast<uint2*>(dst) = hi;
+            *reinterpret_cast<uint2*>(dst + plane) = lo;
+          } else if constexpr (sizeof(LT) == 1) {
+            *reinterpret_cast<uint2*>(dst) = sa_pack_fp8x8(f);
+          } else if constexpr (sizeof(LT) == 2 && sizeof(S) == 4) {
+            *reinterpret_cast<uint2*>(dst) = sa_pack_bf16x4(f);
+          } else if constexpr (sizeof(LT) == 2) {
+            *reinterpret_cast<uint4*>(dst) = tr::pack(f);
+          } else {
+            float* d = reinterpret_cast<float*>(dst);
+            d[0] = f[0]; d[1] = f[1]; d[2] = f[2]; d[3] = f[3];
+          }
+        }
+      }
+    };
+    if constexpr (PRO2) {
+      stage_rows([&](float* f, int i, int g) {
+        float y[VEC];
+        tr::unpack(raw2[i], y);
+        const bool own = g >= own_lo && g < own_hi;
+#pragma unroll
+        for (int j = 0; j < VEC; ++j) {
+          float v = fmaf(k1[j], f[j], fmaf(k2[j], y[j], k3[j]));
+          if (a.nb_relu_mask && !(y[j] > 0.0f)) v = 0.0f;
+          f[j] = v;
+          if (own) csum[j] += v;
+        }
+      });
+      if (a.nb_colsum) {
+        float* colred = reinterpret_cast<float*>(smem + col_off);
+#pragma unroll
+        for (int j = 0; j < VEC; ++j) {
+          float v = csum[j];
+          for (int off = C::CHI; off < 64; off <<= 1) v += __shfl_xor(v, off, 64);
+          if (lane < C::CHI) colred[wave * CIN + (lane % C::CHI) * VEC + j] = v;
+        }
+      }
+    } else if (!has1 && !has2 && !sw) {
+      stage_rows([](float*, int, int) {});
+    } else if (has1 && sw && !has2 && a.pro_stats) {
+      float ps[VEC], pq[VEC];
+#pragma unroll
+      for (int j = 0; j < VEC; ++j) { ps[j] = 0.0f; pq[j] = 0.0f; }
+      stage_rows([&](float* f, int, int g) {
+        const bool own = g >= own_lo && g < own_hi;
+#pragma unroll
+        for (int j = 0; j < VEC; ++j) {
+          const float v = sa_swish(fmaf(f[j], s1[j], t1[j]));
+          f[j] = v;
+          if (own) { ps[j] += v; pq[j] = fmaf(v, v, pq[j]); }
+        }
+      });
+      float* colred = reinterpret_cast<float*>(smem + col_off);
+#pragma unroll
+      for (int j = 0; j < VEC; ++j) {
+        float v = ps[j], w = pq[j];
+        for (int off = C::CHI; off < 64; off <<= 1) { v += __shfl_xor(v, off, 64); w += __shfl_xor(w, off, 64); }
+        if (lane < C::CHI) {
+          colred[(wave * CIN + (lane % C::CHI) * VEC + j) * 2 + 0] = v;
+          colred[(wave * CIN + (lane % C::CHI) * VEC + j) * 2 + 1] = w;
+        }
+      }
+    } else if (has1 && sw && !has2) {
+      stage_rows([&](float* f, int, int) {
+#pragma unroll
+        for (int j = 0; j < VEC; ++j) f[j] = sa_swish(fmaf(f[j], s1[j], t1[j]));
+      });
+    } else {
+      stage_rows([&](float* f, int, int) {
+#pragma unroll
+        for (int j = 0; j < VEC; ++j) {
+          float v = f[j];
+          if (has1) v = fmaf(v, s1[j], t1[j]);
+          if (sw) v = sa_swish(v);
+          if (has2) v = fmaf(v, s2[j], t2[j]);
+          f[j] = v;
+        }
+      });
+    }
+  }
+  __syncthreads();
+  if (!PRO2 && a.pro_stats && tid < CIN) {
+    const float* colred = reinterpret_cast<const float*>(smem + col_off);
+    float* d = a.pro_stats + (((size_t)b * a.ntiles + tile) * CIN + tid) * 2;
+#pragma unroll
+    for (int q = 0; q < 2; ++q)
+      d[q] = (colred[tid * 2 + q] + colred[(CIN + tid) * 2 + q]) +
+             (colred[(2 * CIN + tid) * 2 + q] + colred[(3 * CIN + tid) * 2 + q]);
+  }
+  if constexpr (PRO2) {
+    if (a.nb_colsum && tid < CIN) {
+      const float* colred = reinterpret_cast<const float*>(smem + col_off);
+      a.nb_colsum[((size_t)b * a.ntiles + tile) * CIN + tid] =
+          (colred[tid] + colred[CIN + tid]) + (colred[2 * CIN + tid] + colred[3 * CIN + tid]);
+    }
+  }
+  if constexpr (sizeof(LT) == 2) {
+    if (a.a_out) {
+      constexpr int CH16 = CIN / 8;
+      const int own_lo = m0 * SA;
+      int own_hi = tile == a.ntiles - 1 ? a.Lin : (m0 + C::BMB) * SA;
+      if (own_hi > a.Lin) own_hi = a.Lin;
+      const int rlo = own_lo - (m0 * SA + a.rowmin);
+      bf16_t* ao = reinterpret_cast<bf16_t*>(a.a_out) + ((size_t)b * a.Lin + own_lo) * CIN;
+      for (int e = tid; e < (own_hi - own_lo) * CH16; e += 256) {
+        const int r = e / CH16, c = e % CH16;
+        *reinterpret_cast<uint4*>(ao + (size_t)r * CIN + c * 8) =
+            *reinterpret_cast<const uint4*>(As + (size_t)(rlo + r) * C::APITCH + c * 8);
+      }
+    }
+  }
+
+  const int wn = wave % C::WN, wm = wave / C::WN;
+  f32x16 acc[C::VPW][C::MT];
+#pragma unroll
+  for (int v = 0; v < C::VPW; ++v)
+#pragma unroll
+    for (int mt = 0; mt < C::MT; ++mt)
+#pragma unroll
+      for (int i = 0; i < 16; ++i) acc[v][mt][i] = 0.0f;
+
+  constexpr int KUP = P::NPL == 2 ? 2 : 8;
+  constexpr int KU = C::KSTEPS < KUP ? C::KSTEPS : KUP;
+  constexpr int GPT = C::KSTEPS / KU;
+  static_assert(C::KSTEPS % KU == 0, "k-steps per tap must be a multiple of the prefetch group");
+  const Frag* wp = reinterpret_cast<const Frag*>(a.wp);
+#pragma unroll
+  for (int v = 0; v < C::VPW; ++v) {
+    const int vt = wn + v * C::WN;
+    const int ph = vt / C::NT, nt = vt % C::NT;
+    const int G = a.taps.ntaps[ph] * GPT;
+    const LT* abase = As + (size_t)((wm * C::MT * 32 + (lane & 31)) * SA - a.rowmin) * C::APITCH
+                      + (lane >> 5) * (C::KS / 2);
+    auto load_group = [&](Frag (&dst)[P::NPL][KU], int g) {
+      const int ti = g / GPT, kg = g % GPT;
+      const Frag* wt = wp + (((size_t)a.taps.widx[ph][ti] * C::KSTEPS + kg * KU) * C::NT + nt) * 64 + lane;
+#pragma unroll
+      for (int ku = 0; ku < KU; ++ku) {
+        dst[0][ku] = wt[(size_t)ku * C::NT * 64];
+        if constexpr (P::NPL == 2) dst[1][ku] = wt[(size_t)a.wlo_off + (size_t)ku * C::NT * 64];
+      }
+    };
+    auto compute_group = [&](const Frag (&bq)[P::NPL][KU], int g) {
+      const int ti = g / GPT, kg = g % GPT;
+      const LT* arow = abase + (size_t)a.taps.off[ph][ti] * C::APITCH + kg * KU * C::KS;
+      Frag ah[2][C::MT], al[2][C::MT];
+      auto load_a = [&](int slot, int ku) {
+#pragma unroll
+        for (int mt = 0; mt < C::MT; ++mt) {
+          const LT* ap = arow + (size_t)mt * 32 * SA * C::APITCH + ku * C::KS;
+          ah[slot][mt] = *reinterpret_cast<const Frag*>(ap);
+          if constexpr (P::NPL == 2) al[slot][mt] = *reinterpret_cast<const Frag*>(ap + plane);
+        }
+      };
+      load_a(0, 0);
+#pragma unroll
+      for (int ku = 0; ku < KU; ++ku) {
+        if (ku + 1 < KU) load_a((ku + 1) & 1, ku + 1);
+#pragma unroll
+        for (int mt = 0; mt < C::MT; ++mt) {
+          if constexpr (P::NPL == 2) {
+            acc[v][mt] = __builtin_amdgcn_mfma_f32_32x32x16_bf16(al[ku & 1][mt], bq[0][ku], acc[v][mt], 0, 0, 0);
+            acc[v][mt] = __builtin_amdgcn_mfma_f32_32x32x16_bf16(ah[ku & 1][mt], bq[1][ku], acc[v][mt], 0, 0, 0);
+            acc[v][mt] = __builtin_amdgcn_mfma_f32_32x32x16_bf16(ah[ku & 1][mt], bq[0][ku], acc[v][mt], 0, 0, 0);
+          } else {
+            acc[v][mt] = Tr<LT>::mfma(ah[ku & 1][mt], bq[0][ku], acc[v][mt]);
+          }
+        }
+      }
+    };
+    Frag b0[P::NPL][KU], b1[P::NPL][KU];
+    load_group(b0, 0);
+    for (int g = 0; g < G; g += 2) {
+      if (g + 1 < G) load_group(b1, g + 1);
+      compute_group(b0, g);
+      if (g + 1 < G) {
+        if (g + 2 < G) load_group(b0, g + 2);
+        compute_group(b1, g + 1);
+      }
+    }
+  }
+  constexpr int NOT = TM / C::RPPO;
+  const int ec = tid % C::CHO, er0 = tid / C::CHO;
+  __syncthreads();
+
+#pragma unroll
+  for (int v = 0; v < C::VPW; ++v) {
+    const int vt = wn + v * C::WN;
+    const int ph = vt / C::NT, nt = vt % C::NT;
+    const int col = nt * 32 + (lane & 31);
+    const float bv = a.bias ? a.bias[col] : 0.0f;
+    float winv = 1.0f;
+    if constexpr (sizeof(LT) == 1) winv = a.wscale ? 1.0f / a.wscale[0] : 1.0f;
+#pragma unroll
+    for (int mt = 0; mt < C::MT; ++mt) {
+#pragma unroll
+      for (int i = 0; i < 16; ++i) {
+        const int m = wm * C::MT * 32 + mt * 32 + sa_acc_row(i, lane);
+        float val = sizeof(LT) == 1 ? fmaf(acc[v][mt][i], winv, bv) : acc[v][mt][i] + bv;
+        if (a.relu) val = fmaxf(val, 0.0f);
+        Os[(size_t)(m * U + ph) * C::OPITCH + col] = tr::from_f(val);
+      }
+    }
+  }
+  __syncthreads();
+  {
+    const int c = ec, r0 = er0;
+    float ssum[OVEC], ssq[OVEC], es1[OVEC], et1[OVEC], emu[OVEC], ers[OVEC];
+#pragma unroll
+    for (int j = 0; j < OVEC; ++j) {
+      ssum[j] = 0.0f; ssq[j] = 0.0f;
+      es1[j] = (a.ep_mode && a.ep_s1) ? a.ep_s1[(size_t)b * COUT + c * OVEC + j] : 1.0f;
+      et1[j] = (a.ep_mode && a.ep_t1) ? a.ep_t1[(size_t)b * COUT + c * OVEC + j] : 0.0f;
+      emu[j] = (a.ep_mode && a.ep_mean) ? a.ep_mean[(size_t)b * a.ep_bstride + c * OVEC + j] : 0.0f;
+      ers[j] = (a.ep_mode && a.ep_rstd) ? a.ep_rstd[(size_t)b * a.ep_bstride + c * OVEC + j] : 1.0f;
+    }
+    const bool g2k = a.ep_mode && a.ep_g2 && a.ep_g2k1;
+    float gk1[OVEC], gk2[OVEC], gk3[OVEC];
+#pragma unroll
+    for (int j = 0; j < OVEC; ++j) {
+      gk1[j] = g2k ? a.ep_g2k1[c * OVEC + j] : 1.0f;
+      gk2[j] = g2k ? a.ep_g2k2[c * OVEC + j] : 0.0f;
+      gk3[j] = g2k ? a.ep_g2k3[c * OVEC + j] : 0.0f;
+    }
+    S* yb = reinterpret_cast<S*>(a.y) + (size_t)b * a.Lout * COUT + c * OVEC;
+    const S* xe = a.ep_mode ? reinterpret_cast<const S*>(a.ep_x) + (size_t)b * a.Lout * COUT + c * OVEC : nullptr;
+    const S* ge = (a.ep_mode && a.ep_g2) ? reinterpret_cast<const S*>(a.ep_g2) + (size_t)b * a.Lout * COUT + c * OVEC : nullptr;
+    const int o0 = m0 * U;
+    uint4 gx[GEN == 2 ? NOT : 1];
+    if constexpr (GEN == 2) {
+      static_assert(NOT * C::RPPO == TM, "one source window per tile");
+      float bv[OVEC];
+#pragma unroll
+      for (int j = 0; j < OVEC; ++j) bv[j] = gens[SA_ENC0_K * SA_ENC0_C + c * OVEC + j];
+      sa_enc0_chunks<S, NOT>(gens + SA_ENC0_LDS_FLOATS(0) + r0, C::RPPO, gens + c * OVEC, bv, gx);
+    }
+    auto ep_rows = [&](uint4 u, const uint4& epx, const uint4& epg, int o) {
+      float g[OVEC], x[OVEC], g2[OVEC], xn[OVEC];
+      tr::unpack(u, g); tr::unpack(epx, x); tr::unpack(epg, g2);
+#pragma unroll
+      for (int j = 0; j < OVEC; ++j) {
+        const float z = fmaf(x[j], es1[j], et1[j]);
+        if (g2k) g2[j] = fmaf(gk1[j], g2[j], fmaf(gk2[j], sa_swish(z), gk3[j]));
+        float gg = g[j] + g2[j];
+        if (a.ep_mode == 1) gg *= sa_swish_grad(z);
+        const float xv = a.ep_xp_is_act ? sa_swish(z) : x[j];
+        xn[j] = (xv - emu[j]) * ers[j];
+        g[j] = gg;
+      }
+      u = tr::pack(g);
+      *reinterpret_cast<uint4*>(yb + (size_t)o * COUT) = u;
+      if (a.stats) {
+        tr::unpack(u, g);
+#pragma unroll
+        for (int j = 0; j < OVEC; ++j) { ssum[j] += g[j]; ssq[j] = fmaf(g[j], xn[j], ssq[j]); }
+      }
+    };
+    if (a.ep_mode && o0 + TM <= a.Lout) {
+      auto run = [&](auto has_g2_c) {
+        constexpr bool HG = decltype(has_g2_c)::value;
+        constexpr int D = NOT < 2 ? NOT : 2;
+        uint4 px[D], pg[D];
+#pragma unroll
+        for (int d = 0; d < D; ++d) {
+          if constexpr (GEN != 2) px[d] = *reinterpret_cast<const uint4*>(xe + (size_t)(o0 + r0 + d * C::RPPO) * COUT);
+          pg[d] = make_uint4(0, 0, 0, 0);
+          if constexpr (HG) pg[d] = *reinterpret_cast<const uint4*>(ge + (size_t)(o0 + r0 + d * C::RPPO) * COUT);
+        }
+#pragma unroll
+        for (int i = 0; i < NOT; ++i) {
+          const int r = r0 + i * C::RPPO, o = o0 + r;
+          uint4 epx;
+          if constexpr (GEN == 2) epx = gx[i]; else epx = px[i % D];
+          const uint4 epg = pg[i % D];
+          if (i + D < NOT) {
+            if constexpr (GEN != 2) px[i % D] = *reinterpret_cast<const uint4*>(xe + (size_t)(o + D * C::RPPO) * COUT);
+            if constexpr (HG) pg[i % D] = *reinterpret_cast<const uint4*>(ge + (size_t)(o + D * C::RPPO) * COUT);
+          }
+          const uint4 u = *reinterpret_cast<const uint4*>(Os + (size_t)r * C::OPITCH + c * OVEC);
+          ep_rows(u, epx, epg, o);
+        }
+      };
+      if (ge) run(std::true_type{}); else run(std::false_type{});
+    } else {
+#pragma unroll
+    for (int i = 0; i < NOT; ++i) {
+      const int r = r0 + i * C::RPPO, o = o0 + r;
+      if (o < a.Lout) {
+        uint4 u = *reinterpret_cast<const uint4*>(Os + (size_t)r * C::OPITCH + c * OVEC);
+        if (a.ep_mode) {
+          uint4 epx;
+          if constexpr (GEN == 2) epx = gx[i]; else epx = *reinterpret_cast<const uint4*>(xe + (size_t)o * COUT);
+          const uint4 epg = ge ? *reinterpret_cast<const uint4*>(ge + (size_t)o * COUT) : make_uint4(0, 0, 0, 0);
+          ep_rows(u, epx, epg, o);
+        } else {
+          *reinterpret_cast<uint4*>(yb + (size_t)o * COUT) = u;
+          if (a.stats) {
+            float f[OVEC];
+            tr::unpack(u, f);
+#pragma unroll
+            for (int j = 0; j < OVEC; ++j) { ssum[j] += f[j]; ssq[j] = fmaf(f[j], f[j], ssq[j]); }
+          }
+        }
+      }
+    }
+    }
+    if (a.stats) {
+      __syncthreads();
+#pragma unroll
+      for (int j = 0; j < OVEC; ++j) {
+        red[((size_t)r0 * COUT + c * OVEC + j) * 2 + 0] = ssum[j];
+        red[((size_t)r0 * COUT + c * OVEC + j) * 2 + 1] = ssq[j];
+      }
+    }
+  }
+  if (a.stats) {
+    __syncthreads();
+    if (tid < COUT) {
+      float s = 0.0f, q = 0.0f;
+      for (int r = 0; r < C::RPPO; ++r) {
+        s += red[((size_t)r * COUT + tid) * 2 + 0];
+        q += red[((size_t)r * COUT + tid) * 2 + 1];
+      }
+      float* dst = a.stats + (((size_t)b * a.ntiles + tile) * COUT + tid) * 2;
+      dst[0] = s; dst[1] = q;
+    }
+  }
diff --git a/speech-anonymization_amd/csrc/sa_conv_ws.hip b/speech-anonymization_amd/csrc/sa_conv_ws.hip
--- a/speech-anonymization_amd/csrc/sa_conv_ws.hip
+++ b/speech-anonymization_amd/csrc/sa_conv_ws.hip
@@ -655,6 +655,7 @@
 }
 
 bool sa_conv_ws_covers(int dtype, int cin, int cout, int sa, int u, const SaConvArgs* a) {
+  if (a->gen_in || a->gen_ep) return false;
   if (dtype == SA_BF16X3 && ((cin == 128 && cout == 64) || (cin == 64 && cout == 32)) && sa == 1 && u == 2) {
     if (a->taps.ntaps[0] > 3 || a->taps.ntaps[1] > 3 || a->taps.ntaps[0] < 1 || a->taps.ntaps[1] < 1) return false;
     int lo = 1 << 30, hi = -(1 << 30);
diff --git a/speech-anonymization_amd/csrc/sa_conv_wsd.hip b/speech-anonymization_amd/csrc/sa_conv_wsd.hip
--- a/speech-anonymization_amd/csrc/sa_conv_wsd.hip
+++ b/speech-anonymization_amd/csrc/sa_conv_wsd.hip
@@ -788,6 +788,7 @@
 int wsd_variant(int dtype, int cin, int cout, int sa, int u, const SaConvArgs* a) {
   if (dtype != SA_BF16X3 || cin != 128 || cout != 128 || sa != 1 || u != 1) return 0;
   if (a->ep_mode != 1 && a->ep_mode != 2) return 0;
+  if (a->gen_in || a->gen_ep) return 0;
   if (!a->ep_x || !a->ep_mean || !a->ep_rstd || !a->stats) return 0;
   if (a->s1 || a->t1 || a->s2 || a->t2 || a->swish || a->relu || a->pro_stats || a->wscale || a->bias) return 0;
   if (a->tile_rows && a->tile_rows != 64) return 0;
diff --git a/speech-anonymization_amd/csrc/sa_enc0.h b/speech-anonymization_amd/csrc/sa_enc0.h
--- /dev/null
+++ b/speech-anonymization_amd/csrc/sa_enc0.h
@@ -0,0 +1,62 @@
+#pragma once
+#include "sa_common.h"
+
+#define SA_ENC0_K 15
+#define SA_ENC0_C 32
+#define SA_ENC0_PAD 7
+
+template <int VEC, int N>
+__device__ static inline void sa_enc0_acc(const float* xs, int stride, const float* ws, const float* bv,
+                                          float (&acc)[N][VEC]) {
+#pragma unroll
+  for (int i = 0; i < N; ++i)
+#pragma unroll
+    for (int j = 0; j < VEC; ++j) acc[i][j] = bv[j];
+#pragma unroll
+  for (int k = 0; k < SA_ENC0_K; ++k) {
+    float wv[VEC];
+#pragma unroll
+    for (int j = 0; j < VEC; ++j) wv[j] = ws[k * SA_ENC0_C + j];
+#pragma unroll
+    for (int i = 0; i < N; ++i) {
+      const float xv = xs[i * stride + k];
+#pragma unroll
+      for (int j = 0; j < VEC; ++j) acc[i][j] = fmaf(xv, wv[j], acc[i][j]);
+    }
+  }
+}
+template <typename T, int N>
+__device__ static inline void sa_enc0_chunks(const float* xs, int stride, const float* ws, const float* bv,
+                                             uint4 (&out)[N]) {
+  float acc[N][Tr<T>::VEC];
+  sa_enc0_acc<Tr<T>::VEC, N>(xs, stride, ws, bv, acc);
+#pragma unroll
+  for (int i = 0; i < N; ++i) out[i] = Tr<T>::pack(acc[i]);
+}
+
+#define SA_ENC0_LDS_FLOATS(n) (SA_ENC0_K * SA_ENC0_C + SA_ENC0_C + (n))
+struct SaEnc0Regs { float w[2]; float x[2]; };
+__device__ static inline SaEnc0Regs sa_enc0_load(const float* __restrict__ x, const float* __restrict__ w,
+                                                 const float* __restrict__ bias, int b, int L, int g0, int n,
+                                                 int tid) {
+  SaEnc0Regs r;
+#pragma unroll
+  for (int q = 0; q < 2; ++q) {
+    const int i = tid + q * 256;
+    const int k = i / SA_ENC0_C, c = i % SA_ENC0_C;
+    r.w[q] = i < SA_ENC0_K * SA_ENC0_C ? w[c * SA_ENC0_K + k] : (bias ? bias[c] : 0.0f);
+  }
+#pragma unroll
+  for (int q = 0; q < 2; ++q) {
+    const int i = tid + q * 256, g = g0 + i;
+    r.x[q] = (i < n && g >= 0 && g < L) ? x[(size_t)b * L + g] : 0.0f;
+  }
+  return r;
+}
+__device__ static inline void sa_enc0_stage(float* dst, const SaEnc0Regs& r, int n, int tid) {
+  dst[tid] = r.w[0];
+  dst[tid + 256] = r.w[1];
+#pragma unroll
+  for (int q = 0; q < 2; ++q)
+    if (tid + q * 256 < n) dst[SA_ENC0_K * SA_ENC0_C + SA_ENC0_C + tid + q * 256] = r.x[q];
+}
diff --git a/speech-anonymization_amd/csrc/sa_small.hip b/speech-anonymization_amd/csrc/sa_small.hip
--- a/speech-anonymization_amd/csrc/sa_small.hip
+++ b/speech-anonymization_amd/csrc/sa_small.hip
@@ -1,7 +1,8 @@
 #include "sa_common.h"
-
-#define SA_K15 15
-#define SA_C32 32
+#include "sa_enc0.h"
+
+#define SA_K15 SA_ENC0_K
+#define SA_C32 SA_ENC0_C
 
 template <typename T>
 __global__ __launch_bounds__(256) void sa_conv1toC_kernel(const float* __restrict__ x,
@@ -42,15 +43,9 @@
   for (int p = p0; p < TILE; p += PPP) {
     const int l = l0 + p;
     if (l >= L) break;
-    float acc[VEC];
-#pragma unroll
-    for (int j = 0; j < VEC; ++j) acc[j] = bv[j];
-#pragma unroll
-    for (int k = 0; k < SA_K15; ++k) {
-      const float xv = xs[p + k];
-#pragma unroll
-      for (int j = 0; j < VEC; ++j) acc[j] = fmaf(xv, ws[k][c * VEC + j], acc[j]);
-    }
+    float acc1[1][VEC];
+    sa_enc0_acc<VEC, 1>(xs + p, 0, &ws[0][c * VEC], bv, acc1);
+    float (&acc)[VEC] = acc1[0];
     float xn[VEC];
     if (ep_x) {
       float xv[VEC];
diff --git a/speech-anonymization_amd/ops.py b/speech-anonymization_amd/ops.py
--- a/speech-anonymization_amd/ops.py
+++ b/speech-anonymization_amd/ops.py
@@ -198,14 +198,20 @@
 
 def conv_gemm(x, wp, bias, cin, cout, sa, u, phases, Lout, s1=None, t1=None, s2=None, t2=None,
               swish=False, relu=False, want_stats=False, out=None, code=None, ep=None, a_out=None,
-              nb=None, want_pro_stats=False):
-    lib = L.load()
-    B, Lin, _ = x.shape
-    assert x.shape[2] == cin
-    y = out if out is not None else torch.empty(B, Lout, cout, dtype=x.dtype, device=x.device)
-    kc = L.dt_code(x.dtype) if code is None else code
+              nb=None, want_pro_stats=False, gen=None):
+    lib = L.load()
+    if gen is not None:
+        assert x is None
+        B, Lin = gen["x"].shape
+        dev, adt = gen["x"].device, torch.float32
+    else:
+        B, Lin, _ = x.shape
+        assert x.shape[2] == cin
+        dev, adt = x.device, x.dtype
+    y = out if out is not None else torch.empty(B, Lout, cout, dtype=adt, device=dev)
+    kc = L.dt_code(adt) if code is None else code
     nt = _conv_geometry(cin, cout, u, Lout)
-    stats = torch.empty(B, nt, cout, 2, dtype=torch.float32, device=x.device) if want_stats else None
+    stats = torch.empty(B, nt, cout, 2, dtype=torch.float32, device=dev) if want_stats else None
     a = L.SaConvArgs()
     a.x, a.wp, a.bias, a.y = _f(x), _f(wp), _f(bias), _f(y)
     a.s1, a.t1, a.s2, a.t2 = _f(s1), _f(t1), _f(s2), _f(t2)
@@ -215,24 +221,36 @@
     if kc == L.FP8:
         a.wscale = C.c_void_p(wp.data_ptr() + wp.numel() - 4)
     if a_out is not None:
-        assert a_out.dtype == torch.bfloat16 and a_out.shape == x.shape
+        assert a_out.dtype == torch.bfloat16 and a_out.shape == (B, Lin, cin)
         a.a_out = _f(a_out)
+
+    def set_gen(g, Lg):
+        assert g["x"].dtype == torch.float32 and g["x"].shape == (B, Lg) and g["w"].numel() == 32 * 15
+        assert g["w"].dtype == torch.float32 and (g.get("b") is None or g["b"].numel() == 32)
+        a.gen_x, a.gen_w, a.gen_b = _f(g["x"]), _f(g["w"]), _f(g.get("b"))
+    if gen is not None:
+        set_gen(gen, Lin)
+        a.gen_in = 1
     pro_stats = None
     if want_pro_stats:
-        pro_stats = torch.empty(B, nt, cin, 2, dtype=torch.float32, device=x.device)
+        pro_stats = torch.empty(B, nt, cin, 2, dtype=torch.float32, device=dev)
         a.pro_stats = _f(pro_stats)
     colsum = None
     if nb:
-        assert nb["x"].shape == x.shape and nb["x"].dtype == x.dtype
+        assert nb["x"].shape == (B, Lin, cin) and nb["x"].dtype == adt
         a.nb_x, a.nb_c1, a.nb_c2, a.nb_c3 = _f(nb["x"]), _f(nb["c1"]), _f(nb["c2"]), _f(nb["c3"])
         a.nb_bstride, a.nb_relu_mask = (0 if nb.get("per_c") else cin), int(bool(nb.get("relu_mask")))
         if nb.get("want_colsum"):
-            colsum = torch.empty(B, nt, cin, dtype=torch.float32, device=x.device)
+            colsum = torch.empty(B, nt, cin, dtype=torch.float32, device=dev)
             a.nb_colsum = _f(colsum)
     if ep:
         a.ep_mode, a.ep_xp_is_act = int(ep["mode"]), int(bool(ep.get("xp_is_act")))
         a.ep_bstride = 0 if ep.get("per_c") else cout
-        a.ep_x, a.ep_g2 = _f(ep["x"]), _f(ep.get("g2"))
+        a.ep_x, a.ep_g2 = _f(ep.get("x")), _f(ep.get("g2"))
+        if ep.get("gen") is not None:
+            assert ep.get("x") is None
+            set_gen(ep["gen"], Lout)
+            a.gen_ep = 1
         a.ep_s1, a.ep_t1 = _f(ep.get("s1")), _f(ep.get("t1"))
         a.ep_mean, a.ep_rstd = _f(ep.get("mean")), _f(ep.get("rstd"))
         if ep.get("g2k") is not None:
@@ -242,18 +260,20 @@
             f"sa_conv_gemm({cin},{cout},{sa},{u})")
     if e0 is not None:
         ntap = sum(len(p) for p in phases)
-        esz = x.element_size()
+        esz = y.element_size()
         extra = (a_out.numel() * 2 if a_out is not None else 0)
         if ep:
-            extra += y.numel() * esz * (2 if ep.get("g2") is not None else 1)
+            extra += y.numel() * esz * ((ep.get("g2") is not None) + (ep.get("gen") is None))
         if nb:
             extra += x.numel() * esz
-        io = (x.numel() + y.numel()) * esz
+        io = ((B * Lin * 4 if gen is not None else x.numel() * esz) + y.numel() * esz)
         route = lib.sa_conv_gemm_route(kc, cin, cout, sa, u, C.byref(a))
         tname = {L.F32: "float", L.BF16: "bf16_t", L.BF16X3: "bf16x3_t", L.BF16X1F: "bf16x1f_t", L.FP8: "fp8_t"}[kc]
         ws_mode = (5 if s2 is not None else 0) if s1 is None else 3 if want_pro_stats else 4 if s2 is not None else 1
         kind = (f"sa_conv_wsd_kernel ({tname}, {cin}->{cout}; 5 instances)" if route == 3 else
                 f"sa_conv_ws_kernel<{ws_mode},{ntap}> ({tname}, {cin}->{cout})" if route == 2 else
+                f"sa_conv_gemm_gen_kernel<{tname},{cin},{cout},{sa},{u}{',nb prologue' if nb else ''}>"
+                if gen is not None or (ep and ep.get("gen") is not None) else
                 f"sa_conv_gemm_kernel<{tname},{cin},{cout},{sa},{u}{',nb prologue' if nb else ''}>")
         PROFILE.stop(e0, io + ntap * cin * cout * esz + extra,
                      2 * B * (-(-Lout // u)) * ntap * cin * cout,
```

Result: no change. 3.976 million frames/s (median of 6 runs) (+0.5%).
